# nv-tlabs/LION

Hardware: AMD Instinct MI355X
Metric: shapes/sec @1000-step DDIM, Bx2048pts (higher is better)
Workload: dtype f32 (operands of the 3x3x3 voxel convolutions and of the long 1x1 convolutions cut into fp16 hi/lo pairs on the 16-bi...

## Files before the change

include/lion_hip.h:

```cpp
#ifndef LION_HIP_H_
#define LION_HIP_H_

#include <stddef.h>
#include <stdint.h>

#ifdef __cplusplus
extern "C" {
#endif

typedef void *lionStream_t;

#define LION_OK 0
#define LION_EINVAL (-1)
#define LION_EUNSUPPORTED (-2)
#define LION_EWORKSPACE (-3)

int lion_abi_version(void);

size_t lion_avg_voxelize_workspace_bytes(int B, int C, int N, int r);
int lion_avg_voxelize_forward(const float *feat, const int32_t *coords, int B, int C, int N,
                              int r, float *out, int32_t *ind, int32_t *cnt, void *ws,
                              size_t ws_bytes, lionStream_t stream);

int lion_voxelize_points_forward(const float *feat, const float *coords, int B, int C, int N,
// ... 48 lines not shown
int lion_three_nn_interpolate_cat_forward(const float *points, const float *centers, const float *cfeat, const float *temb,
                                          int ld_t, const float *skip, int B, int C1, int C2, int C3, int N, int M,
                                          float *out, int32_t *idx, float *wgt, lionStream_t stream);
int lion_three_nn_interpolate_backward(const float *gy, const int32_t *idx, const float *wgt,
                                       int B, int C, int N, int M, float *gx,
                                       lionStream_t stream);

int lion_chamfer_forward(const float *xyz1, const float *xyz2, int B, int N, int M,
                         float *dist1, float *dist2, int32_t *idx1, int32_t *idx2,
                         lionStream_t stream);
int lion_chamfer_backward(const float *xyz1, const float *xyz2, const float *gdist1,
                          const float *gdist2, const int32_t *idx1, const int32_t *idx2, int B,
                          int N, int M, float *gxyz1, float *gxyz2, lionStream_t stream);
int lion_chamfer_loss_reduce(const float *dist1, const float *dist2, int B, int N, int M, float s1,
                             float s2, float *loss, lionStream_t stream);
int lion_chamfer_loss_backward(const float *xyz1, const float *xyz2, const int32_t *idx1,
                               const int32_t *idx2, const float *gloss, int B, int N, int M, float s1,
                               float s2, float *gxyz1, float *gxyz2, lionStream_t stream);

size_t lion_emd_workspace_bytes(int B, int N, int M);
int lion_emd_approxmatch(const float *xyz1, const float *xyz2, int B, int N, int M,
                         float *match, void *ws, size_t ws_bytes, lionStream_t stream);
int lion_emd_cost(const float *xyz1, const float *xyz2, int B, int N, int M, float *cost, void *ws,
                  size_t ws_bytes, lionStream_t stream);
int lion_emd_matchcost(const float *xyz1, const float *xyz2, const float *match, int B, int N,
                       int M, float *cost, void *ws, size_t ws_bytes, lionStream_t stream);
int lion_emd_matchcost_backward(const float *grad_cost, const float *xyz1, const float *xyz2,
                                const float *match, int B, int N, int M, float *grad1,
                                float *grad2, lionStream_t stream);
int lion_emd_loss_forward(const float *xyz1, const float *xyz2, int B, int N, int M, float *loss,
                          float *g1u, float *g2u, void *ws, size_t ws_bytes, lionStream_t stream);
int lion_emd_loss_backward(const float *gloss, const float *g1u, const float *g2u, int B, int N, int M,
                           float *gxyz1, float *gxyz2, lionStream_t stream);

int lion_ddim_update(const float *x, const float *eps, const float *z, size_t numel, float s,
                     float c, float sigma, float *out, lionStream_t stream);
int lion_ddpm_update(const float *x, const float *eps, const float *z, size_t numel,
                     int t_is_zero, float k_outer, float k_a, float k_b, float scale,
                     float temp, float *out, lionStream_t stream);
int lion_chain_begin_step(const float *table, int n_steps, int32_t *counter, float *t_out, int B, float *cur,
                          lionStream_t stream);
int lion_chain_update_noise(int mode, const float *x, const float *eps, size_t numel, const float *cur,
                            const uint32_t *seed , uint32_t stream_id, float *out,
                            float *z_out, lionStream_t stream);
int lion_chain_begin_step_temb(const float *table, int n_steps, int32_t *counter, float *t_out, int B, float *cur,
                               const float *temb_table, int temb_width, float *temb_out, lionStream_t stream);
int lion_chain_update_noise_cm(int mode, const float *x, const float *eps_cm, int B, int N, const float *cur,
                               const uint32_t *seed, uint32_t stream_id, float *out, float *z_out, lionStream_t stream);
int lion_dpmpp_update(const float *x, const float *eps, const float *hist, size_t numel, float a0, float a1, float a2,
                      float a3, float a4, float a5, float *out, float *hist_out, lionStream_t stream);
int lion_chain_update_multistep(const float *x, const float *eps, const float *hist, size_t numel, const float *cur,
                                float *out, float *hist_out, lionStream_t stream);
int lion_chain_update_multistep_cm(const float *x, const float *eps_cm, const float *hist, int B, int N, const float *cur,
                                   float *out, float *hist_out, lionStream_t stream);
int lion_sde_dpmpp_update(const float *x, const float *eps, const float *hist, const float *z_in, size_t numel, float a0,
                          float a1, float a2, float a3, float a4, float a5, float a6,
                          const uint32_t *seed , uint32_t step_word, uint32_t stream_id, float *out,
                          float *hist_out, float *z_out, lionStream_t stream);
int lion_chain_update_multistep_noise(const float *x, const float *eps, const float *hist, size_t numel, const float *cur,
                                      const float *table, const uint32_t *seed, uint32_t stream_id, float *out,
                                      float *hist_out, float *z_out, lionStream_t stream);
int lion_chain_update_multistep_noise_cm(const float *x, const float *eps_cm, const float *hist, int B, int N, const float *cur,
                                         const float *table, const uint32_t *seed, uint32_t stream_id, float *out,
                                         float *hist_out, float *z_out, lionStream_t stream);
int lion_ddim_encode_update(const float *base, const float *eps, size_t numel, float a0, float a1, float a2, float *out,
                            float *base_out, lionStream_t stream);
int lion_chain_update_encode(const float *base, const float *eps, size_t numel, const float *cur, float *out, float *base_out,
                             lionStream_t stream);
int lion_chain_update_encode_cm(const float *base, const float *eps_cm, int B, int N, const float *cur, float *out,
                                float *base_out, lionStream_t stream);
#define LION_DIFFUSE_STEP_WORD 0xFFFFFFFFu
int lion_chain_diffuse(const float *x0, const float *z_in, size_t numel, float m, float s,
                       const uint32_t *seed , uint32_t stream_id,
                       float *out, float *z_out, lionStream_t stream);
#define LION_START_STEP_WORD 0xFFFFFFFEu
int lion_philox_normal_keyed(const uint32_t *keys , int B, int n, uint32_t step_word, uint32_t stream_id,
                             float *out, lionStream_t stream);
int lion_chain_update_noise_keyed(int mode, const float *x, const float *eps, int B, int n, const float *cur,
                                  const uint32_t *keys, uint32_t stream_id, float *out, float *z_out, lionStream_t stream);
int lion_chain_update_noise_cm_keyed(int mode, const float *x, const float *eps_cm, int B, int N, const float *cur,
                                     const uint32_t *keys, uint32_t stream_id, float *out, float *z_out, lionStream_t stream);
int lion_chain_update_multistep_noise_keyed(const float *x, const float *eps, const float *hist, int B, int n, const float *cur,
                                            const float *table, const uint32_t *keys, uint32_t stream_id, float *out,
                                            float *hist_out, float *z_out, lionStream_t stream);
int lion_chain_update_multistep_noise_cm_keyed(const float *x, const float *eps_cm, const float *hist, int B, int N,
                                               const float *cur, const float *table, const uint32_t *keys, uint32_t stream_id,
                                               float *out, float *hist_out, float *z_out, lionStream_t stream);
int lion_chain_diffuse_keyed(const float *x0, int B, int n, float m, float s, const uint32_t *keys, uint32_t stream_id,
                             float *out, float *z_out, lionStream_t stream);
int lion_chain_update_noise_keyed_from(int mode, const float *x, const float *eps, int B, int n, const float *cur,
                                       const int32_t *first_row , const uint32_t *keys, uint32_t stream_id,
                                       float *out, float *z_out, lionStream_t stream);
int lion_chain_update_noise_cm_keyed_from(int mode, const float *x, const float *eps_cm, int B, int N, const float *cur,
                                          const int32_t *first_row, const uint32_t *keys, uint32_t stream_id, float *out,
                                          float *z_out, lionStream_t stream);
int lion_chain_diffuse_keyed_at(const float *x0, int B, int n, const float *ms , const uint32_t *keys,
                                uint32_t stream_id, float *out, float *z_out, lionStream_t stream);
int lion_chain_update_noise_keyed_known(int mode, const float *x, const float *eps, int B, int n, const float *cur,
                                        const int32_t *first_row , const uint32_t *keys,
                                        uint32_t stream_id, const float *known_x0, const uint8_t *keep ,
                                        const float *known_ms , uint32_t known_stream_id, float *out,
                                        float *z_out, lionStream_t stream);
int lion_chain_update_noise_cm_keyed_known(int mode, const float *x, const float *eps_cm, int B, int N, const float *cur,
                                           const int32_t *first_row, const uint32_t *keys, uint32_t stream_id,
                                           const float *known_x0, const uint8_t *keep, const float *known_ms,
                                           uint32_t known_stream_id, float *out, float *z_out, lionStream_t stream);
#define LION_VOXEL_STEP_WORD 0xFFFFFFFDu
#define LION_PERTURB_STEP_WORD 0xFFFFFFFCu
size_t lion_voxel_surface_workspace_bytes(int B, int N, int r, int K);
int lion_voxel_surface_points_keyed(const float *x, int B, int N, int r, const uint32_t *keys ,
                                    uint32_t stream_id, int K, float *out, int32_t *faces_out ,
                                    void *ws, size_t ws_bytes, lionStream_t stream);
int lion_perturb_points_keyed(int mode, const float *x, int B, int N, float p0, const uint32_t *keys, uint32_t stream_id,
                              float *out, lionStream_t stream);
int lion_voxel_occupancy(const float *x, int B, int N, int r, const float *frame_in ,
                         uint8_t *grid, float *frame_out , int32_t *clamped_out ,
                         lionStream_t stream);
int lion_voxel_surface_points_grid_keyed(const uint8_t *grid, const float *frame, int B, int r, const uint32_t *keys,
                                         uint32_t stream_id, int K, float *out, int32_t *faces_out ,
                                         lionStream_t stream);
int lion_voxel_iou(const uint8_t *a, const uint8_t *b, int B, int r, int32_t *counts ,
                   float *iou , lionStream_t stream);
int lion_latent_unpack(const float *x, int B, int N, int D, float *all, float *coords, float *rest, lionStream_t stream);
int lion_concat_broadcast(const float *a, const float *t, int B, int Ca, int Ct, int N, int ld_t, float *out,
                          lionStream_t stream);

size_t lion_conv3d_packed_floats(int Cout, int Cin);
int lion_conv3d_pack_weights(const float *w, int Cout, int Cin, float *wp, lionStream_t stream);
int lion_conv3d_k3_forward(const float *x, const float *wp, const float *bias, int B, int Cin,
                           int Cout, int r, float *y, lionStream_t stream);
size_t lion_conv3d_wgrad_workspace_floats(int B, int Cin, int Cout, int r);
int lion_conv3d_k3_wgrad(const float *x, const float *gy, int B, int Cin, int Cout, int r, float *gw, float *ws,
                         size_t ws_floats, lionStream_t stream);
int lion_conv3d_k3_wgrad_split(const float *x, const float *gy, int B, int Cin, int Cout, int r, float *gw, float *ws,
                               size_t ws_floats, lionStream_t stream);
size_t lion_conv3d_wgrad_sparse_workspace_floats(int B, int Cin, int Cout, int r);
int lion_conv3d_k3_wgrad_split_sparse(const float *x, const float *gy, const int32_t *cnt, int B, int Cin, int Cout, int r,
                                      float *gw, float *ws, size_t ws_floats, lionStream_t stream);

int lion_conv3d_stat_tiles(int r, int Cout, int B, int sparse);
int lion_conv3d_k3_fused_forward(const float *x, const float *wp, const float *bias, int B, int Cin,
                                 int Cout, int r, const float *pro_a, const float *pro_b, const float *pro_bias,
                                 const float *tconst, float *y, float *stats, int32_t *occ, lionStream_t stream);
size_t lion_conv3d_occupancy_ints(int r, int Cout, int B);
int lion_conv3d_const_response(const float *wsum, const float *bias2, const float *bias1, const float *pro_a,
                               const float *pro_b, int B, int Cin, int Cout, float *tconst, lionStream_t stream);
int lion_conv3d_tile_occupancy(const int32_t *cnt, int B, int r, int Cout, int32_t *occ_m1, int32_t *occ_m2,
                               lionStream_t stream);
int lion_conv3d_tile_occupancy_aware(const int32_t *cnt, int B, int r, int Cout, int32_t *occ_m1, int32_t *occ_m2,
                                     int consumer_aware, lionStream_t stream);
int lion_groupnorm_fold(const float *stats, int B, int C, int T, int G, int voxels, const float *gamma,
                        const float *beta, const float *fac, const float *gbias, int ld_fg, float eps,
                        float *A, float *Bs, float *chmean, lionStream_t stream);
size_t lion_conv3d_split_packed_halfs(int Cout, int Cin);
int lion_conv3d_split_pack_weights(const float *w, int Cout, int Cin, uint16_t *wp, lionStream_t stream);
int lion_conv3d_split_stat_tiles(int r, int Cout);
int lion_conv3d_k3_split_forward(const float *x, const uint16_t *wp, const float *bias, int B, int Cin, int Cout,
                                 int r, const float *pro_a, const float *pro_b, const float *pro_bias,
                                 const float *tconst, float *y, float *stats, int32_t *occ, lionStream_t stream);
int lion_conv3d_k3_half_forward(const float *x, const uint16_t *wp, const float *bias, int B, int Cin, int Cout,
                                int r, const float *pro_a, const float *pro_b, const float *pro_bias,
                                const float *tconst, float *y, float *stats, int32_t *occ, lionStream_t stream);
size_t lion_skinny_packed_floats(int Cout, int Cin);
int lion_skinny_pack_weights(const float *w, int Cout, int Cin, float *wp, lionStream_t stream);
int lion_skinny_splits(int Cin, int Cout);
int lion_skinny_gemm(const float *pin, int ks_in, const float *bias_in, int act_in, const float *addT,
                     const float *wp, int nb, int Cin, int Cout, float *pout, lionStream_t stream);
int lion_skinny_finish(const float *A, int ks_a, const float *bias_a, const float *Bp, int ks_b, const float *resid,
                       int nb, int C, int mode, float *y, lionStream_t stream);
int lion_skinny_gemm_se_finish(const float *pin, int ks_in, const float *bias_in, int act_in, const float *wp, int nb, int Cin,
                               int Cout, const float *A, int ks_a, const float *bias_a, const float *resid, float *y,
                               lionStream_t stream);
int lion_internal_skinny_gemm_plain(const float *pin, int ks_in, const float *bias_in, int act_in, const float *addT,
                                    const float *wp, int nb, int Cin, int Cout, float *pout, lionStream_t stream);
int lion_internal_skinny_gemm_se_finish_plain(const float *pin, int ks_in, const float *bias_in, int act_in, const float *wp,
                                              int nb, int Cin, int Cout, const float *A, int ks_a, const float *bias_a,
                                              const float *resid, float *y, lionStream_t stream);
int lion_to_channel_major(const float *a, int lda, int Ca, float *oa, const float *b, int ldb, int Cb, float *ob, int B,
                          lionStream_t stream);
int lion_from_channel_major(const float *x, int B, int C, float *y, lionStream_t stream);
int lion_groupnorm_fold_se(const float *stats, int B, int C, int T, int G, int voxels, const float *gamma,
                           const float *beta, const float *fac, const float *gbias, int ld_fg, float eps, const float *w1,
                           const float *w2, int H, float *A, float *Bs, lionStream_t stream);
int lion_internal_groupnorm_fold_se_plain(const float *stats, int B, int C, int T, int G, int voxels, const float *gamma,
                                          const float *beta, const float *fac, const float *gbias, int ld_fg, float eps,
                                          const float *w1, const float *w2, int H, float *A, float *Bs, lionStream_t stream);
int lion_se_gate(const float *chmean, const float *w1, const float *w2, int B, int C, int H, float *A,
                 float *Bs, lionStream_t stream);
int lion_trilinear_devoxelize_affine_forward(const float *coords, const float *feat, const float *scale,
                                             const float *shift, int B, int C, int N, int r, float *out,
                                             lionStream_t stream);
size_t lion_devoxelize_plan_bytes(int B, int N, int r);
int lion_trilinear_devoxelize_plan(const float *coords, int B, int N, int r, void *plan, size_t plan_bytes,
                                   lionStream_t stream);
int lion_trilinear_devoxelize_planned_forward(const void *plan, size_t plan_bytes, const float *coords, const float *feat,
                                              const float *scale, const float *shift, int B, int C, int N, int r,
                                              float *out, lionStream_t stream);

int lion_row_stats(const float *x, int rows, int L, float *stats, lionStream_t stream);
size_t lion_pwconv_packed_floats(int Cout, int Cin);
int lion_pwconv_pack_weights(const float *w, int Cout, int Cin, float *wp, lionStream_t stream);
int lion_pwconv_stat_tiles(int Cout, int Cin, int L);
int lion_pwconv_forward(const float *x, const float *wp, const float *bias, int B, int Cin, int Cout, int L,
                        const float *pro_a, const float *pro_b, float *y, float *stats, lionStream_t stream);
int lion_pwconv_forward_max(const float *x, const float *wp, const float *bias, int B, int Cin, int Cout, int L,
                            const float *pro_a, const float *pro_b, const float *out_a, const float *out_b,
                            float *stats, float *ymax, lionStream_t stream);
size_t lion_pwconv_split_packed_halfs(int Cout, int Cin);
int lion_pwconv_split_pack_weights(const float *w, int Cout, int Cin, uint16_t *wp, lionStream_t stream);
int lion_pwconv_split_pack_weights_t(const float *w, int Cout, int Cin, const uint16_t *wp, uint16_t *wpt, lionStream_t stream);
int lion_pwconv_split_stat_tiles(int Cout, int Cin, int L);
int lion_pwconv_split_forward(const float *x, const uint16_t *wp, const float *bias, int B, int Cin, int Cout, int L,
                              const float *pro_a, const float *pro_b, float *y, float *stats, lionStream_t stream);
int lion_pwconv_grouped_forward(const float *coords, const float *centers, const float *feat, const int32_t *idx,
                                const float *wp, const float *bias, int B, int C, int N, int M, int U, int Cout, float *y,
                                float *stats, lionStream_t stream);
int lion_pwconv_split_grouped_forward(const float *coords, const float *centers, const float *feat, const int32_t *idx,
                                      const uint16_t *wp, const float *bias, int B, int C, int N, int M, int U, int Cout,
                                      float *y, float *stats, lionStream_t stream);
int lion_internal_pwconv_walk(const float *x, const float *wp, const float *bias, int B, int Cin, int Cout, int L,
                              const float *pro_a, const float *pro_b, const float *out_a, const float *out_b,
                              const float *coords, const float *centers, const float *feat, const int32_t *idx, int N, int U,
                              float *y, float *stats, int max_wg, int lds_weights, lionStream_t stream);
int lion_internal_pwconv_small_plain(const float *x, const float *wp, const float *bias, int B, int Cin, int Cout, int L,
                                     const float *pro_a, const float *pro_b, const float *coords, const float *centers,
                                     const float *feat, const int32_t *idx, int N, int U, float *y, float *stats,
                                     lionStream_t stream);
int lion_linear_attention_core(const float *qkv, int B, int H, int D, int N, float *out, lionStream_t stream);
int lion_internal_linear_attention_path(int N, int aligned);
int lion_internal_linear_attention_core_plain(const float *qkv, int B, int H, int D, int N, float *out, lionStream_t stream);
int lion_linear_attention_core_backward(const float *qkv, const float *gout, int B, int H, int D, int N, float *gqkv,
                                        lionStream_t stream);
int lion_linear_forward(const float *x, const float *wp, const float *bias, int B, int K, int O, int act, float slope,
                        float *y, lionStream_t stream);
int lion_affine_swish(const float *x, const float *A, const float *Bs, int rows, int L, float *y,
                      lionStream_t stream);
int lion_affine_swish_max(const float *x, const float *A, const float *Bs, int rows, int M, int U,
                          float *y, lionStream_t stream);
int lion_timestep_embedding(const float *t, const float *row, float scale, int B, int half, int D, float *emb,
                            lionStream_t stream);
int lion_affine_swish_add(const float *x, const float *A, const float *Bs, const float *addend, int rows, int L, float *y,
                          lionStream_t stream);

size_t lion_scatter_csr_workspace_bytes(int B, int E, int bins);
int lion_scatter_csr(const float *gy, const int32_t *idx, const float *w, int B, int C, int S, int E, int bins, void *ws,
                     size_t ws_bytes, float *gx, lionStream_t stream);

size_t lion_pwconv_wgrad_workspace_bytes(int B, int Cin, int Cout, int L);
int lion_pwconv_wgrad(const float *x, const float *gy, int B, int Cin, int Cout, int L, void *ws, size_t ws_bytes,
                      float *gw, float *gb, lionStream_t stream);

int lion_gn_train_fold(const float *stats, const float *gw, const float *gb, const float *fac, int fac_stride,
                       const float *bias, int bias_stride, int B, int C, int G, int L, float eps, float *A, float *Bs,
                       float *mean, float *rstd, lionStream_t stream);
int lion_row_stats64(const float *x, int rows, int L, double *stats, lionStream_t stream);
int lion_gn_train_fold64(const double *stats, const float *gw, const float *gb, const float *fac, int fac_stride,
                         const float *bias, int bias_stride, int B, int C, int G, int L, float eps, float *A,
                         float *Bs, float *mean, float *rstd, lionStream_t stream);
int lion_gn_train_bwd_fold(const float *S, const float *mean, const float *rstd, const float *gw, const float *gb,
                           const float *fac, int fac_stride, int B, int C, int G, int L, float *Q, float *R, float *dfac,
                           float *dbias, int d_stride, float *pw, const float *A, const double *xstats, const float *gate,
                           const float *qse, float *Aout, lionStream_t stream);
int lion_gn_train_param_grads(const float *pw, int B, int C, float *dgw, float *dgb, float *dxs, lionStream_t stream);
int lion_se_gate_fwd(const float *stats, const float *w1, const float *w2, int B, int C, int Cr, int L, float *mean, float *h,
                     float *g, float *zero, lionStream_t stream);
int lion_se_gate_bwd(const float *S, const float *g, const float *h, const float *mean, const float *w1, const float *w2, int B,
                     int C, int Cr, int L, float *dpre2, float *dpre1, float *Q, float *dw1, float *dw2, lionStream_t stream);
int lion_rows_dot2(const float *g, const float *v, const float *ws, int B, int C, int N, float *S, lionStream_t stream);
int lion_trilinear_devoxelize_backward_affine(const float *gy, const int32_t *inds, const float *wgts, const float *x,
                                              const float *Ap, const float *Q, const float *R, int B, int C, int N, int r3,
                                              float *dx, lionStream_t stream);
int lion_gn_se_gate_fwd(const double *xstats, const float *A, const float *Bs, const float *w1, const float *w2, int B, int C, int Cr,
                        int L, float *mean, float *h, float *g, float *A2, float *B2, lionStream_t stream);
int lion_gn_se_gate_bwd(const float *S, const double *xstats, const float *A, const float *Bs, const float *g, const float *h,
                        const float *mean, const float *w1, const float *w2, int B, int C, int Cr, int L, float *Sp, float *dpre2,
                        float *dpre1, float *Qse, float *dw1, float *dw2, lionStream_t stream);
int lion_affine_act(const float *x, const float *A, const float *Bs, int rows, int L, int act, float *y,
                    lionStream_t stream);
int lion_affine_act_bwd_stats(const float *x, const float *gy, const float *A, const float *Bs, int rows, int L, int act,
                              float *S, lionStream_t stream);
int lion_affine_act_bwd_apply(const float *x, const float *gy, const float *A, const float *Bs, const float *Q,
                              const float *R, int rows, int L, int act, float *dx, lionStream_t stream);
int lion_affine_act_dropout(const float *x, const float *A, const float *Bs, int rows, int L, int act, const uint64_t *seed,
                            float keep, float *y, lionStream_t stream);
int lion_affine_act_dropout_bwd_stats(const float *x, const float *gy, const float *A, const float *Bs, int rows, int L, int act,
                                      const uint64_t *seed, float keep, float *S, lionStream_t stream);
int lion_affine_act_dropout_bwd_apply(const float *x, const float *gy, const float *A, const float *Bs, const float *Q,
                                      const float *R, int rows, int L, int act, const uint64_t *seed, float keep, float *dx,
                                      lionStream_t stream);
int lion_affine_act_max(const float *x, const float *A, const float *Bs, int rows, int M, int U, int act, float *y,
                        lionStream_t stream);
int lion_affine_act_max_bwd_stats(const float *x, const float *gy, const float *A, const float *Bs, int rows, int M, int U,
                                  int act, float *S, lionStream_t stream);
int lion_affine_act_max_bwd_apply(const float *x, const float *gy, const float *A, const float *Bs, const float *Q,
                                  const float *R, int rows, int M, int U, int act, float *dx, lionStream_t stream);

int lion_adam_chunk(void);
int lion_adam_row(void);
int lion_adam_step(const uint64_t *table, const int32_t *numel, const int32_t *blockmap, int blocks, int tensors, const float *lr,
                   float beta1, float beta2, float eps, float weight_decay, float ema_decay, lionStream_t stream);

int lion_grad_sqnorm_partials(const uint64_t *table, const int32_t *numel, const int32_t *blockmap, int blocks, float *partials,
                              lionStream_t stream);
int lion_grad_clip_coef(const float *partials, int n, float max_norm, float *out2, lionStream_t stream);
int lion_adam_step_scaled(const uint64_t *table, const int32_t *numel, const int32_t *blockmap, int blocks, int tensors,
                          const float *lr, float beta1, float beta2, float eps, float weight_decay, float ema_decay,
                          const float *grad_scale, lionStream_t stream);

#define LION_ODE_RUNNING 0
#define LION_ODE_FINISHED 1
#define LION_ODE_TOO_SMALL_STEP (-1)
typedef struct lion_ode_ctrl {
  double t, h_abs, t_bound, direction, rtol, atol;
  double h, t_new, err_norm, h0, d1, sign;
  int32_t stage, cur, status, step_rejected;
  int32_t yslot, fslot, nfe, n_accepted;
  int32_t n_rejected, accepted, pad0, pad1;
} lion_ode_ctrl;
size_t lion_ode_partials_bytes(size_t n);
int lion_ode_stage(double *Y, const double *K, size_t n, lion_ode_ctrl *ctrl, float *x32, float *t_model, int B,
                   lionStream_t stream);
int lion_ode_drift(const float *eps, int cm_points, const float *x32, size_t n, const float *t_model, float beta_start,
                   float beta_delta, float neg_beta_start, float half_beta_delta, float one_minus_sigma2_0,
                   const float *mix_a, const float *mix_b, int mix_len, double *K, lion_ode_ctrl *ctrl,
                   lionStream_t stream);
int lion_ode_error_partials(const double *Y, const double *K, size_t n, const lion_ode_ctrl *ctrl, double *partials,
                            lionStream_t stream);
int lion_ode_control(const double *partials, size_t n, lion_ode_ctrl *ctrl, lionStream_t stream);

#ifdef __cplusplus
}
#endif
#endif
```

lion_amd/_lib.py:

```python
from __future__ import annotations

import ctypes as C
import os

_HERE = os.path.dirname(os.path.abspath(__file__))
SO_PATH = os.environ.get("LION_HIP_SO") or os.path.join(_HERE, "csrc", "liblion_hip.so")

_vp, _i, _f, _sz = C.c_void_p, C.c_int, C.c_float, C.c_size_t

SIGNATURES = {
    "lion_abi_version": (_i, []),
    "lion_avg_voxelize_workspace_bytes": (_sz, [_i, _i, _i, _i]),
    "lion_avg_voxelize_forward": (_i, [_vp, _vp, _i, _i, _i, _i, _vp, _vp, _vp, _vp, _sz, _vp]),
    "lion_voxelize_points_forward": (_i, [_vp, _vp, _i, _i, _i, _i, _i, _f, _vp, _vp, _vp, _vp,
                                          _vp, _sz, _vp]),
    "lion_voxel_plan_bytes": (_sz, [_i, _i, _i]),
    "lion_voxel_index": (_i, [_vp, _i, _i, _i, _i, _f, _vp, _vp, _vp, _vp, _sz, _vp]),
    "lion_voxel_scatter": (_i, [_vp, _vp, _sz, _i, _i, _i, _i, _vp, _vp]),
    "lion_voxel_scatter_read": (_i, [_vp, _vp, _sz, _i, _i, _i, _i, _vp, _vp, _vp]),
    "lion_internal_voxelize_plan": (_i, [_i, _i, _i, _i, _i, _vp, _vp]),
    "lion_internal_devoxelize_path": (_i, [_i, _i, _i, _i, _i, _vp, _vp]),
    "lion_avg_voxelize_backward": (_i, [_vp, _vp, _vp, _i, _i, _i, _i, _vp, _vp]),
    "lion_trilinear_devoxelize_forward": (_i, [_vp, _vp, _i, _i, _i, _i, _i, _vp, _vp, _vp, _vp]),
    "lion_trilinear_devoxelize_backward": (_i, [_vp, _vp, _vp, _i, _i, _i, _i, _vp, _vp]),
    "lion_ball_query": (_i, [_vp, _vp, _i, _i, _i, _f, _i, _vp, _vp]),
    "lion_grouping_forward": (_i, [_vp, _vp, _i, _i, _i, _i, _i, _vp, _vp]),
    "lion_group_points_forward": (_i, [_vp, _vp, _vp, _vp, _i, _i, _i, _i, _i, _vp, _vp]),
    "lion_grouping_backward": (_i, [_vp, _vp, _i, _i, _i, _i, _i, _vp, _vp]),
    "lion_furthest_point_sampling": (_i, [_vp, _i, _i, _i, _vp, _vp]),
    "lion_gather_features_forward": (_i, [_vp, _vp, _i, _i, _i, _i, _vp, _vp]),
    "lion_gather_features_backward": (_i, [_vp, _vp, _i, _i, _i, _i, _vp, _vp]),
    "lion_three_nn_interpolate_forward": (_i, [_vp, _vp, _vp, _i, _i, _i, _i, _vp, _vp, _vp, _vp]),
    "lion_three_nn_interpolate_backward": (_i, [_vp, _vp, _vp, _i, _i, _i, _i, _vp, _vp]),
    "lion_chamfer_forward": (_i, [_vp, _vp, _i, _i, _i, _vp, _vp, _vp, _vp, _vp]),
    "lion_chamfer_backward": (_i, [_vp, _vp, _vp, _vp, _vp, _vp, _i, _i, _i, _vp, _vp, _vp]),
    "lion_chamfer_loss_reduce": (_i, [_vp, _vp, _i, _i, _i, _f, _f, _vp, _vp]),
    "lion_chamfer_loss_backward": (_i, [_vp, _vp, _vp, _vp, _vp, _i, _i, _i, _f, _f, _vp, _vp, _vp]),
    "lion_emd_workspace_bytes": (_sz, [_i, _i, _i]),
    "lion_emd_approxmatch": (_i, [_vp, _vp, _i, _i, _i, _vp, _vp, _sz, _vp]),
    "lion_emd_cost": (_i, [_vp, _vp, _i, _i, _i, _vp, _vp, _sz, _vp]),
    "lion_emd_matchcost": (_i, [_vp, _vp, _vp, _i, _i, _i, _vp, _vp, _sz, _vp]),
    "lion_emd_matchcost_backward": (_i, [_vp, _vp, _vp, _vp, _i, _i, _i, _vp, _vp, _vp]),
    "lion_emd_loss_forward": (_i, [_vp, _vp, _i, _i, _i, _vp, _vp, _vp, _vp, _sz, _vp]),
    "lion_emd_loss_backward": (_i, [_vp, _vp, _vp, _i, _i, _i, _vp, _vp, _vp]),
    "lion_conv3d_packed_floats": (_sz, [_i, _i]),
    "lion_conv3d_pack_weights": (_i, [_vp, _i, _i, _vp, _vp]),
    "lion_conv3d_k3_forward": (_i, [_vp, _vp, _vp, _i, _i, _i, _i, _vp, _vp]),
    "lion_conv3d_wgrad_workspace_floats": (_sz, [_i, _i, _i, _i]),
    "lion_conv3d_k3_wgrad": (_i, [_vp, _vp, _i, _i, _i, _i, _vp, _vp, _sz, _vp]),
    "lion_conv3d_k3_wgrad_split": (_i, [_vp, _vp, _i, _i, _i, _i, _vp, _vp, _sz, _vp]),
    "lion_conv3d_wgrad_sparse_workspace_floats": (_sz, [_i, _i, _i, _i]),
    "lion_conv3d_k3_wgrad_split_sparse": (_i, [_vp, _vp, _vp, _i, _i, _i, _i, _vp, _vp, _sz, _vp]),
    "lion_conv3d_stat_tiles": (_i, [_i, _i, _i, _i]),
    "lion_conv3d_k3_fused_forward": (_i, [_vp, _vp, _vp, _i, _i, _i, _i, _vp, _vp, _vp, _vp, _vp, _vp, _vp, _vp]),
    "lion_conv3d_const_response": (_i, [_vp, _vp, _vp, _vp, _vp, _i, _i, _i, _vp, _vp]),
    "lion_conv3d_occupancy_ints": (_sz, [_i, _i, _i]),
    "lion_conv3d_tile_occupancy": (_i, [_vp, _i, _i, _i, _vp, _vp, _vp]),
    "lion_conv3d_tile_occupancy_aware": (_i, [_vp, _i, _i, _i, _vp, _vp, _i, _vp]),
    "lion_conv3d_split_packed_halfs": (_sz, [_i, _i]),
    "lion_conv3d_split_pack_weights": (_i, [_vp, _i, _i, _vp, _vp]),
    "lion_conv3d_split_stat_tiles": (_i, [_i, _i]),
    "lion_conv3d_k3_split_forward": (_i, [_vp, _vp, _vp, _i, _i, _i, _i, _vp, _vp, _vp, _vp, _vp, _vp, _vp, _vp]),
    "lion_conv3d_k3_half_forward": (_i, [_vp, _vp, _vp, _i, _i, _i, _i, _vp, _vp, _vp, _vp, _vp, _vp, _vp, _vp]),
    "lion_groupnorm_fold": (_i, [_vp, _i, _i, _i, _i, _i, _vp, _vp, _vp, _vp, _i, _f, _vp, _vp, _vp, _vp]),
    "lion_groupnorm_fold_se": (_i, [_vp, _i, _i, _i, _i, _i, _vp, _vp, _vp, _vp, _i, _f, _vp, _vp, _i, _vp, _vp, _vp]),
    "lion_internal_groupnorm_fold_se_plain": (_i, [_vp, _i, _i, _i, _i, _i, _vp, _vp, _vp, _vp, _i, _f, _vp, _vp, _i, _vp, _vp, _vp]),
    "lion_skinny_packed_floats": (_sz, [_i, _i]),
    "lion_skinny_pack_weights": (_i, [_vp, _i, _i, _vp, _vp]),
    "lion_skinny_splits": (_i, [_i, _i]),
    "lion_skinny_gemm": (_i, [_vp, _i, _vp, _i, _vp, _vp, _i, _i, _i, _vp, _vp]),
    "lion_skinny_gemm_se_finish": (_i, [_vp, _i, _vp, _i, _vp, _i, _i, _i, _vp, _i, _vp, _vp, _vp, _vp]),
    "lion_internal_skinny_gemm_plain": (_i, [_vp, _i, _vp, _i, _vp, _vp, _i, _i, _i, _vp, _vp]),
    "lion_internal_skinny_gemm_se_finish_plain": (_i, [_vp, _i, _vp, _i, _vp, _i, _i, _i, _vp, _i, _vp, _vp, _vp, _vp]),
    "lion_skinny_finish": (_i, [_vp, _i, _vp, _vp, _i, _vp, _i, _i, _i, _vp, _vp]),
    "lion_to_channel_major": (_i, [_vp, _i, _i, _vp, _vp, _i, _i, _vp, _i, _vp]),
    "lion_from_channel_major": (_i, [_vp, _i, _i, _vp, _vp]),
    "lion_se_gate": (_i, [_vp, _vp, _vp, _i, _i, _i, _vp, _vp, _vp]),
    "lion_trilinear_devoxelize_affine_forward": (_i, [_vp, _vp, _vp, _vp, _i, _i, _i, _i, _vp, _vp]),
    "lion_devoxelize_plan_bytes": (_sz, [_i, _i, _i]),
    "lion_trilinear_devoxelize_plan": (_i, [_vp, _i, _i, _i, _vp, _sz, _vp]),
    "lion_trilinear_devoxelize_planned_forward": (_i, [_vp, _sz, _vp, _vp, _vp, _vp, _i, _i, _i, _i, _vp, _vp]),
    "lion_row_stats": (_i, [_vp, _i, _i, _vp, _vp]),
    "lion_pwconv_packed_floats": (_sz, [_i, _i]),
    "lion_pwconv_pack_weights": (_i, [_vp, _i, _i, _vp, _vp]),
    "lion_pwconv_stat_tiles": (_i, [_i, _i, _i]),
    "lion_pwconv_forward": (_i, [_vp, _vp, _vp, _i, _i, _i, _i, _vp, _vp, _vp, _vp, _vp]),
    "lion_pwconv_forward_max": (_i, [_vp, _vp, _vp, _i, _i, _i, _i, _vp, _vp, _vp, _vp, _vp, _vp, _vp]),
    "lion_pwconv_split_packed_halfs": (_sz, [_i, _i]),
    "lion_pwconv_split_pack_weights": (_i, [_vp, _i, _i, _vp, _vp]),
    "lion_pwconv_split_pack_weights_t": (_i, [_vp, _i, _i, _vp, _vp, _vp]),
    "lion_pwconv_split_stat_tiles": (_i, [_i, _i, _i]),
    "lion_pwconv_split_forward": (_i, [_vp, _vp, _vp, _i, _i, _i, _i, _vp, _vp, _vp, _vp, _vp]),
    "lion_pwconv_grouped_forward": (_i, [_vp, _vp, _vp, _vp, _vp, _vp, _i, _i, _i, _i, _i, _i, _vp, _vp, _vp]),
    "lion_pwconv_split_grouped_forward": (_i, [_vp, _vp, _vp, _vp, _vp, _vp, _i, _i, _i, _i, _i, _i, _vp, _vp, _vp]),
    "lion_internal_pwconv_walk": (_i, [_vp, _vp, _vp, _i, _i, _i, _i, _vp, _vp, _vp, _vp, _vp, _vp, _vp, _vp, _i, _i, _vp, _vp, _i, _i, _vp]),
    "lion_internal_pwconv_small_plain": (_i, [_vp, _vp, _vp, _i, _i, _i, _i, _vp, _vp, _vp, _vp, _vp, _vp, _i, _i, _vp, _vp, _vp]),
    "lion_linear_attention_core": (_i, [_vp, _i, _i, _i, _i, _vp, _vp]),
    "lion_internal_linear_attention_path": (_i, [_i, _i]),
    "lion_internal_linear_attention_core_plain": (_i, [_vp, _i, _i, _i, _i, _vp, _vp]),
    "lion_linear_attention_core_backward": (_i, [_vp, _vp, _i, _i, _i, _i, _vp, _vp]),
    "lion_linear_forward": (_i, [_vp, _vp, _vp, _i, _i, _i, _i, _f, _vp, _vp]),
    "lion_affine_swish": (_i, [_vp, _vp, _vp, _i, _i, _vp, _vp]),
    "lion_affine_swish_max": (_i, [_vp, _vp, _vp, _i, _i, _i, _vp, _vp]),
    "lion_timestep_embedding": (_i, [_vp, _vp, _f, _i, _i, _i, _vp, _vp]),
    "lion_affine_swish_add": (_i, [_vp, _vp, _vp, _vp, _i, _i, _vp, _vp]),
    "lion_scatter_csr_workspace_bytes": (_sz, [_i, _i, _i]),
    "lion_scatter_csr": (_i, [_vp, _vp, _vp, _i, _i, _i, _i, _i, _vp, _sz, _vp, _vp]),
    "lion_pwconv_wgrad_workspace_bytes": (_sz, [_i, _i, _i, _i]),
    "lion_pwconv_wgrad": (_i, [_vp, _vp, _i, _i, _i, _i, _vp, _sz, _vp, _vp, _vp]),
    "lion_gn_train_fold": (_i, [_vp, _vp, _vp, _vp, _i, _vp, _i, _i, _i, _i, _i, _f, _vp, _vp, _vp, _vp, _vp]),
    "lion_row_stats64": (_i, [_vp, _i, _i, _vp, _vp]),
    "lion_gn_train_fold64": (_i, [_vp, _vp, _vp, _vp, _i, _vp, _i, _i, _i, _i, _i, _f, _vp, _vp, _vp, _vp, _vp]),
    "lion_gn_train_bwd_fold": (_i, [_vp, _vp, _vp, _vp, _vp, _vp, _i, _i, _i, _i, _i, _vp, _vp, _vp, _vp, _i, _vp, _vp, _vp, _vp, _vp,
                                    _vp, _vp]),
    "lion_gn_train_param_grads": (_i, [_vp, _i, _i, _vp, _vp, _vp, _vp]),
    "lion_adam_chunk": (_i, []),
    "lion_adam_row": (_i, []),
    "lion_adam_step": (_i, [_vp, _vp, _vp, _i, _i, _vp, _f, _f, _f, _f, _f, _vp]),
    "lion_grad_sqnorm_partials": (_i, [_vp, _vp, _vp, _i, _vp, _vp]),
    "lion_grad_clip_coef": (_i, [_vp, _i, _f, _vp, _vp]),
    "lion_adam_step_scaled": (_i, [_vp, _vp, _vp, _i, _i, _vp, _f, _f, _f, _f, _f, _vp, _vp]),
    "lion_se_gate_fwd": (_i, [_vp, _vp, _vp, _i, _i, _i, _i, _vp, _vp, _vp, _vp, _vp]),
    "lion_se_gate_bwd": (_i, [_vp, _vp, _vp, _vp, _vp, _vp, _i, _i, _i, _i, _vp, _vp, _vp, _vp, _vp, _vp]),
    "lion_rows_dot2": (_i, [_vp, _vp, _vp, _i, _i, _i, _vp, _vp]),
    "lion_trilinear_devoxelize_backward_affine": (_i, [_vp, _vp, _vp, _vp, _vp, _vp, _vp, _i, _i, _i, _i, _vp, _vp]),
    "lion_gn_se_gate_fwd": (_i, [_vp, _vp, _vp, _vp, _vp, _i, _i, _i, _i, _vp, _vp, _vp, _vp, _vp, _vp]),
    "lion_gn_se_gate_bwd": (_i, [_vp, _vp, _vp, _vp, _vp, _vp, _vp, _vp, _vp, _i, _i, _i, _i, _vp, _vp, _vp, _vp, _vp, _vp, _vp]),
    "lion_affine_act": (_i, [_vp, _vp, _vp, _i, _i, _i, _vp, _vp]),
    "lion_affine_act_bwd_stats": (_i, [_vp, _vp, _vp, _vp, _i, _i, _i, _vp, _vp]),
    "lion_affine_act_bwd_apply": (_i, [_vp, _vp, _vp, _vp, _vp, _vp, _i, _i, _i, _vp, _vp]),
    "lion_affine_act_dropout": (_i, [_vp, _vp, _vp, _i, _i, _i, _vp, _f, _vp, _vp]),
    "lion_affine_act_dropout_bwd_stats": (_i, [_vp, _vp, _vp, _vp, _i, _i, _i, _vp, _f, _vp, _vp]),
    "lion_affine_act_dropout_bwd_apply": (_i, [_vp, _vp, _vp, _vp, _vp, _vp, _i, _i, _i, _vp, _f, _vp, _vp]),
    "lion_affine_act_max": (_i, [_vp, _vp, _vp, _i, _i, _i, _i, _vp, _vp]),
    "lion_affine_act_max_bwd_stats": (_i, [_vp, _vp, _vp, _vp, _i, _i, _i, _i, _vp, _vp]),
    "lion_affine_act_max_bwd_apply": (_i, [_vp, _vp, _vp, _vp, _vp, _vp, _i, _i, _i, _i, _vp, _vp]),
    "lion_ddim_update": (_i, [_vp, _vp, _vp, _sz, _f, _f, _f, _vp, _vp]),
    "lion_ddpm_update": (_i, [_vp, _vp, _vp, _sz, _i, _f, _f, _f, _f, _f, _vp, _vp]),
    "lion_chain_begin_step": (_i, [_vp, _i, _vp, _vp, _i, _vp, _vp]),
    "lion_chain_update_noise": (_i, [_i, _vp, _vp, _sz, _vp, _vp, C.c_uint32, _vp, _vp, _vp]),
    "lion_chain_begin_step_temb": (_i, [_vp, _i, _vp, _vp, _i, _vp, _vp, _i, _vp, _vp]),
    "lion_chain_update_noise_cm": (_i, [_i, _vp, _vp, _i, _i, _vp, _vp, C.c_uint32, _vp, _vp, _vp]),
    "lion_chain_diffuse": (_i, [_vp, _vp, _sz, _f, _f, _vp, C.c_uint32, _vp, _vp, _vp]),
    "lion_dpmpp_update": (_i, [_vp, _vp, _vp, _sz, _f, _f, _f, _f, _f, _f, _vp, _vp, _vp]),
    "lion_chain_update_multistep": (_i, [_vp, _vp, _vp, _sz, _vp, _vp, _vp, _vp]),
    "lion_chain_update_multistep_cm": (_i, [_vp, _vp, _vp, _i, _i, _vp, _vp, _vp, _vp]),
    "lion_sde_dpmpp_update": (_i, [_vp, _vp, _vp, _vp, _sz, _f, _f, _f, _f, _f, _f, _f, _vp, C.c_uint32, C.c_uint32, _vp, _vp,
                                   _vp, _vp]),
    "lion_chain_update_multistep_noise": (_i, [_vp, _vp, _vp, _sz, _vp, _vp, _vp, C.c_uint32, _vp, _vp, _vp, _vp]),
    "lion_chain_update_multistep_noise_cm": (_i, [_vp, _vp, _vp, _i, _i, _vp, _vp, _vp, C.c_uint32, _vp, _vp, _vp, _vp]),
    "lion_ddim_encode_update": (_i, [_vp, _vp, _sz, _f, _f, _f, _vp, _vp, _vp]),
    "lion_chain_update_encode": (_i, [_vp, _vp, _sz, _vp, _vp, _vp, _vp]),
    "lion_chain_update_encode_cm": (_i, [_vp, _vp, _i, _i, _vp, _vp, _vp, _vp]),
    "lion_philox_normal_keyed": (_i, [_vp, _i, _i, C.c_uint32, C.c_uint32, _vp, _vp]),
    "lion_chain_update_noise_keyed": (_i, [_i, _vp, _vp, _i, _i, _vp, _vp, C.c_uint32, _vp, _vp, _vp]),
    "lion_chain_update_noise_cm_keyed": (_i, [_i, _vp, _vp, _i, _i, _vp, _vp, C.c_uint32, _vp, _vp, _vp]),
    "lion_chain_update_multistep_noise_keyed": (_i, [_vp, _vp, _vp, _i, _i, _vp, _vp, _vp, C.c_uint32, _vp, _vp, _vp, _vp]),
    "lion_chain_update_multistep_noise_cm_keyed": (_i, [_vp, _vp, _vp, _i, _i, _vp, _vp, _vp, C.c_uint32, _vp, _vp, _vp, _vp]),
    "lion_chain_diffuse_keyed": (_i, [_vp, _i, _i, _f, _f, _vp, C.c_uint32, _vp, _vp, _vp]),
    "lion_chain_update_noise_keyed_from": (_i, [_i, _vp, _vp, _i, _i, _vp, _vp, _vp, C.c_uint32, _vp, _vp, _vp]),
    "lion_chain_update_noise_cm_keyed_from": (_i, [_i, _vp, _vp, _i, _i, _vp, _vp, _vp, C.c_uint32, _vp, _vp, _vp]),
    "lion_chain_update_noise_keyed_known": (_i, [_i, _vp, _vp, _i, _i, _vp, _vp, _vp, C.c_uint32, _vp, _vp, _vp, C.c_uint32, _vp,
                                                 _vp, _vp]),
    "lion_chain_update_noise_cm_keyed_known": (_i, [_i, _vp, _vp, _i, _i, _vp, _vp, _vp, C.c_uint32, _vp, _vp, _vp, C.c_uint32,
                                                    _vp, _vp, _vp]),
    "lion_chain_diffuse_keyed_at": (_i, [_vp, _i, _i, _vp, _vp, C.c_uint32, _vp, _vp, _vp]),
    "lion_voxel_surface_workspace_bytes": (_sz, [_i, _i, _i, _i]),
    "lion_voxel_surface_points_keyed": (_i, [_vp, _i, _i, _i, _vp, C.c_uint32, _i, _vp, _vp, _vp, _sz, _vp]),
    "lion_perturb_points_keyed": (_i, [_i, _vp, _i, _i, _f, _vp, C.c_uint32, _vp, _vp]),
    "lion_voxel_occupancy": (_i, [_vp, _i, _i, _i, _vp, _vp, _vp, _vp, _vp]),
    "lion_voxel_surface_points_grid_keyed": (_i, [_vp, _vp, _i, _i, _vp, C.c_uint32, _i, _vp, _vp, _vp]),
    "lion_voxel_iou": (_i, [_vp, _vp, _i, _i, _vp, _vp, _vp]),
    "lion_latent_unpack": (_i, [_vp, _i, _i, _i, _vp, _vp, _vp, _vp]),
    "lion_concat_broadcast": (_i, [_vp, _vp, _i, _i, _i, _i, _i, _vp, _vp]),
    "lion_three_nn_interpolate_cat_forward": (_i, [_vp, _vp, _vp, _vp, _i, _vp, _i, _i, _i, _i, _i, _i, _vp, _vp, _vp, _vp]),
    "lion_ode_partials_bytes": (_sz, [_sz]),
    "lion_ode_stage": (_i, [_vp, _vp, _sz, _vp, _vp, _vp, _i, _vp]),
    "lion_ode_drift": (_i, [_vp, _i, _vp, _sz, _vp, _f, _f, _f, _f, _f, _vp, _vp, _i, _vp, _vp, _vp]),
    "lion_ode_error_partials": (_i, [_vp, _vp, _sz, _vp, _vp, _vp]),
    "lion_ode_control": (_i, [_vp, _sz, _vp, _vp]),
}



_ERR = {-1: "LION_EINVAL (bad shape / null pointer)",
        -2: "LION_EUNSUPPORTED (shape outside what the kernels implement)",
        -3: "LION_EWORKSPACE (workspace too small)"}

_lib = None


def load() -> C.CDLL:
    global _lib
    if _lib is not None:
        return _lib
    if not os.path.exists(SO_PATH):
        raise RuntimeError(
            f"lion_amd: HIP extension not built: {SO_PATH} is missing. Run "
            f"`python -c 'import __graft_entry__ as g; g.build()'` or lion_amd/csrc/build.sh. "
            f"There is no CPU fallback.")
    lib = C.CDLL(SO_PATH)
    for name, (res, args) in SIGNATURES.items():
        try:
            fn = getattr(lib, name)
        except AttributeError as e:
            raise RuntimeError(f"lion_amd: {SO_PATH} does not export {name}") from e
        fn.restype = res
        fn.argtypes = args
    _lib = lib
    return lib


def check(code: int, what: str) -> None:
    if code != 0:
        msg = _ERR.get(code, f"hipError {code}" if code > 0 else f"error {code}")
        raise RuntimeError(f"lion_amd: {what} failed: {msg}")


def call(name: str, *args, unsupported_ok: bool = False) -> bool:
    import torch
    if len(args) + 1 != len(SIGNATURES[name][1]):
        raise TypeError(f"lion_amd: {name} takes {len(SIGNATURES[name][1]) - 1} arguments before the stream, got {len(args)}")
    dev, argv = None, list(args)
    for i, a in enumerate(args):
        if isinstance(a, torch.Tensor):
            d = a.get_device()
            if d != dev:
                if d < 0:
                    raise RuntimeError("lion_amd: expected a CUDA(HIP) tensor; there is no CPU path")
                if dev is not None:
                    raise RuntimeError(f"lion_amd: {name}: operands on different devices (cuda:{dev} and cuda:{d})")
# ... 27 lines not shown
```

lion_amd/chain.py:

```python
from __future__ import annotations

from collections import OrderedDict

import numpy as np
import torch

from . import _lib, _wcache

DDIM, DDPM, DPMPP, SDE_DPMPP, ENCODE = range(5)
UPDATE = {
    DDIM: ("lion_chain_update_noise", (DDIM, "x", "eps", "size", "cur", "seed", 0, "x", "z")),
    DDPM: ("lion_chain_update_noise", (DDPM, "x", "eps", "size", "cur", "seed", 0, "x", "z")),
    DPMPP: ("lion_chain_update_multistep", ("x", "eps", "hist", "size", "cur", "x", "hist")),
    SDE_DPMPP: ("lion_chain_update_multistep_noise", ("x", "eps", "hist", "size", "cur", "table", "seed", 0, "x", "hist", "z")),
    ENCODE: ("lion_chain_update_encode", ("base", "eps", "size", "cur", "x", "base")),
}
KEYED_MODES = (DDIM, DDPM, SDE_DPMPP)
FROM_ROWS_MODES = (DDPM,)
KNOWN_STREAM = 2
START_STEP_WORD, DIFFUSE_STEP_WORD = 0xFFFFFFFE, 0xFFFFFFFF
_MASK64 = 0xFFFFFFFFFFFFFFFF


def split_seed(seed: int, n: int):
    out, state = [], seed & _MASK64
    for _ in range(n):
        state = (state + 0x9E3779B97F4A7C15) & _MASK64
        z = state
        z = ((z ^ (z >> 30)) * 0xBF58476D1CE4E5B9) & _MASK64
        z = ((z ^ (z >> 27)) * 0x94D049BB133111EB) & _MASK64
        out.append(z ^ (z >> 31))
    return out


def sample_keys(seeds, num_samples, who="seeds") -> list:
    if isinstance(seeds, torch.Tensor):
        seeds = seeds.detach().cpu().reshape(-1).tolist()
    elif isinstance(seeds, np.ndarray):
        seeds = seeds.reshape(-1).tolist()
    try:
        keys = [int(s) & _MASK64 for s in seeds]
    except TypeError as e:
        raise ValueError(f"{who}: a sequence or tensor of {num_samples} ints, got {seeds!r}") from e
    if len(keys) != int(num_samples):
        raise ValueError(f"{who}: {len(keys)} seeds for {num_samples} samples")
    return keys


def first_rows(first_row, num_samples) -> list:
    rows = [int(r) for r in first_row]
    if len(rows) != int(num_samples) or any(not 0 <= r < 2 ** 31 for r in rows):
        raise ValueError(f"GraphedChain: first_row = {rows!r}: {num_samples} ints in [0, 2^31)")
    return rows


def key_words(keys, device=None):
    k = np.array([[s & 0xFFFFFFFF, (s >> 32) & 0xFFFFFFFF] for s in keys], dtype=np.uint32).view(np.int32)
    t = torch.from_numpy(k)
    return t if device is None else t.to(device)


RECORD = None
TEMB_TABLE = __import__("os").environ.get("LION_TEMB_TABLE", "1") != "0"
CHANNEL_MAJOR_EPS = __import__("os").environ.get("LION_CHAIN_CM_EPS", "1") != "0"

def policy_key() -> tuple:
    from . import conv_ops, fused_ops, geometry
    from .models import pvcnn2_ada
    return (pvcnn2_ada.SPARSE_CONV1, pvcnn2_ada.FUSE_INFERENCE, pvcnn2_ada.OVERLAP_POINT_BRANCH, geometry.ENABLED,
            geometry.SPLIT_GRAPH, conv_ops.SPLIT, fused_ops.PW_SPLIT, pvcnn2_ada.VOX_PLAN, TEMB_TABLE, fused_ops.MAX_RECOMPUTE,
            pvcnn2_ada.SKIP_UNREAD, pvcnn2_ada.SKIP_UNREAD_LEVEL2, CHANNEL_MAJOR_EPS, pvcnn2_ada.SA_GATHER, conv_ops.PRECISION)


def channel_major(model, shape) -> bool:
    n_pts, n_cls = getattr(model, "num_points", 0), getattr(model, "num_classes", 0)
    return CHANNEL_MAJOR_EPS and hasattr(model, "geometry_source") and n_cls == 4 and int(np.prod(shape)) == n_pts * n_cls


def same_conditioning(owner, condition_input, clip_feat) -> bool:
    same = lambda buf, new: (buf is None) == (new is None) and (buf is None or buf.shape == new.shape)
    return same(owner.cond, condition_input) and same(owner.clip, clip_feat)


class LRU:

    def __init__(self, capacity=4):
        self._entries, self._capacity = OrderedDict(), capacity

    def lookup(self, key, usable, build):
        hit = self._entries.get(key)
        if hit is not None and usable(hit):
            self._entries.move_to_end(key)
            return hit
        self._entries.pop(key, None)
        hit = self._entries[key] = build()
        while len(self._entries) > self._capacity:
            self._entries.popitem(last=False)
        return hit

    def clear(self):
        self._entries.clear()


class CapturedStep:

    def __init__(self, model, step, x, *, warmup=2, split=None):
        self.model, self.x = model, x
        self.fingerprint, self.policy = _wcache.fingerprint(model), policy_key()
        self.pinned = []
        dev = x.device
        from . import geometry
        src = getattr(model, "geometry_source", None)
        self.geo_graphs = self.graph_b = self.graphs = self.waits = self.geo_plan = None
        if split is None:
            split = geometry.SPLIT_GRAPH and src is not None and not geometry.ENABLED
        main = torch.cuda.current_stream(dev)
        side = torch.cuda.Stream(device=dev)
        side.wait_stream(main)
        with _wcache.pinning(self.pinned):
            with torch.no_grad(), torch.cuda.stream(side):
                for _ in range(warmup):
                    step()
            main.wait_stream(side)
            if split:
                self.geo_stream = torch.cuda.Stream(device=dev)
                self.ev_step = torch.cuda.Event()

                def geo(boundary=None):
                    mods, coords = src(x)
                    return geometry.compute_chain(mods, coords, boundary=boundary)
                self.geo_stream.wait_stream(main)
                with torch.no_grad(), torch.cuda.stream(self.geo_stream):
                    geo()
                main.wait_stream(self.geo_stream)
                torch.cuda.synchronize(dev)
                self.geo_graphs = [torch.cuda.CUDAGraph()]
                gs = torch.cuda.Stream(device=dev)
                gs.wait_stream(main)

                def geo_cut(i):
                    if i == 1:
                        self.geo_graphs[-1].capture_end()
                        self.geo_graphs.append(torch.cuda.CUDAGraph())
                        self.geo_graphs[-1].capture_begin(pool=self.geo_graphs[0].pool())
                with torch.no_grad(), torch.cuda.stream(gs):
                    self.geo_graphs[0].capture_begin()
                    try:
                        self.geo_plan = geo(geo_cut)
                    finally:
                        self.geo_graphs[-1].capture_end()
                main.wait_stream(gs)
                torch.cuda.synchronize(dev)
                self.geo_stage_of_graph = [0, self.geo_plan["stages"] - 1][:len(self.geo_graphs)]
                self.ev_geo = [torch.cuda.Event() for _ in self.geo_graphs]
                graphs, waits = [torch.cuda.CUDAGraph()], []

                def on_use(first, last):
                    need = [g for g, st_ in enumerate(self.geo_stage_of_graph)
                            if st_ >= first and (g == 0 or self.geo_stage_of_graph[g - 1] < last)]
                    need = [g for g in need if not any(g in w for w in waits)]
                    if not need:
                        return
                    graphs[-1].capture_end()
                    waits.append(need)
                    graphs.append(torch.cuda.CUDAGraph())
                    graphs[-1].capture_begin(pool=graphs[0].pool())
                cap = torch.cuda.Stream(device=dev)
                cap.wait_stream(main)
                with torch.no_grad(), torch.cuda.stream(cap), geometry.external(self.geo_plan, on_use):
                    graphs[0].capture_begin()
                    try:
                        step()
                    finally:
                        graphs[-1].capture_end()
                main.wait_stream(cap)
                self.graph = graphs[0]
                if waits:
                    self.graphs, self.waits = graphs, waits
                    self.graph_b = graphs[1]
                else:
                    self.geo_graphs = self.geo_plan = None
            else:
                self.graph = torch.cuda.CUDAGraph()
                with torch.no_grad(), torch.cuda.graph(self.graph):
                    step()
        self.pinned = list({id(v): v for v in self.pinned}.values())

    def replay(self):
        if self.graph_b is None:
            self.graph.replay()
            return
        main = torch.cuda.current_stream(self.x.device)
        self.ev_step.record(main)
        self.geo_stream.wait_event(self.ev_step)
        with torch.cuda.stream(self.geo_stream):
            for g, ev in zip(self.geo_graphs, self.ev_geo):
                g.replay()
                ev.record(self.geo_stream)
        self.graphs[0].replay()
        for k, need in enumerate(self.waits):
            for g in need:
                main.wait_event(self.ev_geo[g])
            self.graphs[k + 1].replay()

    def valid(self):
        return self.fingerprint == _wcache.fingerprint(self.model) and self.policy == policy_key()


class GraphedChain:
    def __init__(self, model, num_samples, shape, condition_input, clip_feat, device, mode, capacity, warmup=2,
                 record_noise=False, keyed=False, from_rows=False, known=False):
        self.model, self.mode, self.capacity, self.keyed = model, mode, int(capacity), bool(keyed)
        self.from_rows, self.known = bool(from_rows), bool(known)
        dev = torch.device(device)
        size = [num_samples] + list(shape)
        per_sample = int(np.prod(shape))
        if self.from_rows and not (keyed and mode in FROM_ROWS_MODES):
            raise ValueError(f"GraphedChain: from_rows needs a keyed DDPM chain, got mode {mode}, keyed={bool(keyed)}")
        if self.known and not (keyed and self.from_rows):
            raise ValueError(f"GraphedChain: known needs keyed=True and from_rows=True, got keyed={bool(keyed)}, "
                             f"from_rows={self.from_rows}")
        if keyed and mode not in KEYED_MODES:
            raise ValueError(f"GraphedChain: mode {mode} draws nothing and has no keyed form")
        if keyed and per_sample % 4 != 0:
# ... 153 lines not shown
```

lion_amd/csrc/common.h:

```cpp
#pragma once
#include <hip/hip_runtime.h>
#include <stdint.h>
#include <stddef.h>
#include <type_traits>

#include "lion_hip.h"

#define LION_WAVE 64

#define LION_LAUNCH_CHECK()                         \
  do {                                              \
    hipError_t e__ = hipGetLastError();             \
    if (e__ != hipSuccess) return (int)e__;         \
  } while (0)

static inline int lion_cdiv(int a, int b) { return (a + b - 1) / b; }

#define LION_MAX_DEVICES 32
struct LionLdsLimit {
  size_t bytes[LION_MAX_DEVICES];
};
static inline int lion_current_device(int *dev) {
  if (hipGetDevice(dev) != hipSuccess || *dev < 0 || *dev >= LION_MAX_DEVICES) return LION_EINVAL;
  return 0;
}
static inline int lion_cu_count(int *n) {
  static int cu_count[LION_MAX_DEVICES] = {0};
  int dev = 0;
  if (int e = lion_current_device(&dev)) return e;
  if (!cu_count[dev]) {
    hipDeviceProp_t prop;
    if (hipGetDeviceProperties(&prop, dev) != hipSuccess) return LION_EINVAL;
    cu_count[dev] = prop.multiProcessorCount;
  }
  *n = cu_count[dev];
  return 0;
}
template <typename K>
static inline int lion_dynamic_lds(K kernel, size_t bytes, LionLdsLimit &limit) {
  int dev = 0;
  if (int e = lion_current_device(&dev)) return e;
  if (bytes > limit.bytes[dev]) {
    hipError_t e = hipFuncSetAttribute(reinterpret_cast<const void *>(kernel),
                                       hipFuncAttributeMaxDynamicSharedMemorySize, (int)bytes);
    if (e != hipSuccess) return (int)e;
    limit.bytes[dev] = bytes;
  }
  return 0;
}

template <auto Kernel> struct LionLaunch;
template <typename... P, void (*Kernel)(P...)> struct LionLaunch<Kernel> {
  int operator()(dim3 grid, dim3 block, size_t lds, hipStream_t st, P... args) const {
    if (lds > 0) {
      static LionLdsLimit limit = {};
      if (int e = lion_dynamic_lds(Kernel, lds, limit)) return e;
    }
    Kernel<<<grid, block, lds, st>>>(args...);
    return (int)hipGetLastError();
  }
};
template <auto Kernel> static constexpr LionLaunch<Kernel> lion_launch{};

template <bool V> using BoolC = std::bool_constant<V>;
template <int V> using IntC = std::integral_constant<int, V>;
template <typename F> static inline int lion_with_flags(bool a, F f) { return a ? f(BoolC<true>{}) : f(BoolC<false>{}); }
template <typename F> static inline int lion_with_flags(bool a, bool b, F f) {
  return lion_with_flags(a, [&](auto A) { return lion_with_flags(b, [&](auto B) { return f(A, B); }); });
}

struct PwGather {
  const float *coords, *centers, *feat;
  const int32_t *idx;
  int C, N, U;
};

__device__ __forceinline__ float mul_rn(float a, float b) { return __fmul_rn(a, b); }
__device__ __forceinline__ float add_rn(float a, float b) { return __fadd_rn(a, b); }
__device__ __forceinline__ float sub_rn(float a, float b) { return __fsub_rn(a, b); }
__device__ __forceinline__ float div_rn(float a, float b) { return __fdiv_rn(a, b); }
__device__ __forceinline__ float sqrt_rn(float a) { return sqrtf(a); }
__device__ __forceinline__ void philox4x32_10(uint32_t c0, uint32_t c1, uint32_t c2, uint32_t c3, uint32_t k0,
                                              uint32_t k1, uint32_t out[4]) {
#pragma unroll
  for (int r = 0; r < 10; ++r) {
    const uint64_t p0 = (uint64_t)0xD2511F53u * c0, p1 = (uint64_t)0xCD9E8D57u * c2;
    const uint32_t n0 = (uint32_t)(p1 >> 32) ^ c1 ^ k0, n2 = (uint32_t)(p0 >> 32) ^ c3 ^ k1;
    c1 = (uint32_t)p1; c3 = (uint32_t)p0; c0 = n0; c2 = n2;
    k0 += 0x9E3779B9u; k1 += 0xBB67AE85u;
  }
  out[0] = c0; out[1] = c1; out[2] = c2; out[3] = c3;
}

__device__ __forceinline__ float swish_fast(float t) { return t * __builtin_amdgcn_rcpf(1.0f + __expf(-t)); }

__device__ __forceinline__ float sqdist3(float ax, float ay, float az, float bx, float by,
                                         float bz) {
  const float dx = sub_rn(ax, bx), dy = sub_rn(ay, by), dz = sub_rn(az, bz);
  return add_rn(add_rn(mul_rn(dx, dx), mul_rn(dy, dy)), mul_rn(dz, dz));
}

#define LION_DPP_F32(v, ctrl) __builtin_bit_cast(float, __builtin_amdgcn_update_dpp(0, __builtin_bit_cast(int, (v)), (ctrl), 0xf, 0xf, true))
__device__ __forceinline__ float row16_sum_rn(float v) {
  v = __fadd_rn(v, LION_DPP_F32(v, 0xB1));
  v = __fadd_rn(v, LION_DPP_F32(v, 0x4E));
  v = __fadd_rn(v, LION_DPP_F32(v, 0x141));
  v = __fadd_rn(v, LION_DPP_F32(v, 0x140));
  return v;
}
__device__ __forceinline__ unsigned wave_max_u32_lane63(unsigned v) {
#define LION_DPP_U32(x, ctrl, rmask) ((unsigned)__builtin_amdgcn_update_dpp(0, (int)(x), (ctrl), (rmask), 0xf, true))
  unsigned o;
  o = LION_DPP_U32(v, 0xB1, 0xf); v = o > v ? o : v;
  o = LION_DPP_U32(v, 0x4E, 0xf); v = o > v ? o : v;
  o = LION_DPP_U32(v, 0x141, 0xf); v = o > v ? o : v;
  o = LION_DPP_U32(v, 0x140, 0xf); v = o > v ? o : v;
  o = LION_DPP_U32(v, 0x142, 0xa); v = o > v ? o : v;
  o = LION_DPP_U32(v, 0x143, 0xc); v = o > v ? o : v;
#undef LION_DPP_U32
  return v;
}
__device__ __forceinline__ float row_pair_sum_odd_rows(float v) {
  return __fadd_rn(v, __builtin_bit_cast(float, __builtin_amdgcn_update_dpp(0, __builtin_bit_cast(int, v), 0x142, 0xa, 0xf, true)));
}
#define LION_DPP_F32_ROWS(x, ctrl, rmask) \
  __builtin_bit_cast(float, __builtin_amdgcn_update_dpp(0, __builtin_bit_cast(int, (x)), (ctrl), (rmask), 0xf, true))
__device__ __forceinline__ float row16_max(float v) {
  float o;
  o = LION_DPP_F32(v, 0xB1); v = o > v ? o : v;
  o = LION_DPP_F32(v, 0x4E); v = o > v ? o : v;
  o = LION_DPP_F32(v, 0x141); v = o > v ? o : v;
  o = LION_DPP_F32(v, 0x140); v = o > v ? o : v;
  return v;
}

__device__ __forceinline__ int wave_incl_scan(int v, int lane) {
#pragma unroll
  for (int d = 1; d < LION_WAVE; d <<= 1) {
    const int t = __shfl_up(v, d, LION_WAVE);
    if (lane >= d) v += t;
  }
  return v;
}
```

lion_amd/csrc/conv3d.hip:

```cpp
#include "conv3d_tiles.h"

namespace {

typedef float f32x16 __attribute__((ext_vector_type(16)));
#ifndef LION_CONV_KC
#define LION_CONV_KC 4
#endif
#ifndef LION_CONV_WAVES
#define LION_CONV_WAVES 2
#endif
constexpr int KC = LION_CONV_KC;

__device__ __forceinline__ float pro_act(float v, float pa, float pb) {
  const float t = v * pa + pb;
  return swish_fast(t);
}

template <int TD, int TH, int TW, int COT, int VB, bool PRO, bool STATS>
__global__ __launch_bounds__(256, LION_CONV_WAVES) void conv3d_k3_kernel(const float *__restrict__ x,
                                                                const float *__restrict__ wp,
                                                                const float *__restrict__ bias,
                                                                float *__restrict__ y, int Cin,
                                                                int Cout, int r,
                                                                const float *__restrict__ pro_a,
// ... 341 lines not shown
    const int4 v = c4[i];
    if (v.x | v.y | v.z | v.w) {
      const unsigned m4 = (v.x ? 1u : 0u) | (v.y ? 2u : 0u) | (v.z ? 4u : 0u) | (v.w ? 8u : 0u);
      atomicOr(&col[(i << 2) / r], m4 << ((i << 2) % r));
    }
  }
  __syncthreads();
  const int RW = 64 / r;
  for (int e = tid; e < 2 * ntiles; e += 1024) {
    const int t = e % ntiles, margin = 1 + e / ntiles;
    const int dt = (t / nth) * TD, ht = (t % nth) * TH;
    int mask = 0;
    for (int w = 0; w < 4; ++w) {
      const int dl = dt + (w * RW) / TH, hl = ht + (w * RW) % TH;
      unsigned any = 0u;
      for (int d = max(dl - margin, 0); d <= min(dl + margin, r - 1); ++d)
        for (int h = max(hl - margin, 0); h <= min(hl + RW - 1 + margin, r - 1); ++h) any |= col[d * r + h];
      mask |= (any ? 1 : 0) << w;
    }
    flag[margin - 1][t] = mask;
  }
  __syncthreads();
  __shared__ unsigned long long bal[2][4];
  const int m = tid >> 8, t = tid & 255, lane = tid & 63, w = (tid >> 6) & 3;
  const bool live = tid < 512 && t < ntiles;
  const int f = live ? flag[m][t] : 0;
  const unsigned long long bl = __ballot(f != 0);
  if (tid < 512 && lane == 0) bal[m][w] = bl;
  __syncthreads();
  if (live) {
    int32_t *occ = m == 0 ? occ1 : occ2;
    if (occ) {
      int before = __popcll(bal[m][w] & ((1ull << lane) - 1ull)), occupied = 0;
      for (int ww = 0; ww < 4; ++ww) {
        const int c = __popcll(bal[m][ww]);
        if (ww < w) before += c;
        occupied += c;
      }
      int32_t *fl = occ + (size_t)b * ntiles, *list = occ + total + (size_t)b * ntiles;
      int need = flag[1][t] != 0;
      if (m == 0) {
        if (aware == 2) {
          need = 0;
        } else {
          const int td = t / nth, th = t % nth;
          for (int dd = max(td - 1, 0); dd <= min(td + 1, r / TD - 1); ++dd)
            for (int hh = max(th - 1, 0); hh <= min(th + 1, nth - 1); ++hh) need |= flag[1][dd * nth + hh] != 0;
        }
      }
      fl[t] = f | (need << 8) | ((m == 1 && flag[0][t] != 0) ? (1 << 9) : 0);
      list[f ? before : occupied + (t - before)] = t;
      if (b == 0 && t == 0) { occ[2 * total] = 0; occ[2 * total + 1] = 0; occ[2 * total + 2] = aware; }
    }
  }
}

__global__ __launch_bounds__(256) void conv_tconst_kernel(const float *__restrict__ wsum, const float *__restrict__ bias2,
                                                          const float *__restrict__ bias1, const float *__restrict__ pro_a,
                                                          const float *__restrict__ pro_b, int Cin, int Cout,
                                                          float *__restrict__ tconst) {
  __shared__ float sc[256];
  const int cfg = blockIdx.x, b = blockIdx.y, tid = threadIdx.x;
  for (int c = tid; c < Cin; c += 256)
    sc[c] = pro_act(bias1 ? bias1[c] : 0.f, pro_a[(size_t)b * Cin + c], pro_b[(size_t)b * Cin + c]);
  __syncthreads();
  for (int co = tid; co < Cout; co += 256) {
    double acc = bias2 ? (double)bias2[co] : 0.0;
    const float *w = wsum + (size_t)cfg * Cin * Cout + co;
    for (int c = 0; c < Cin; ++c) acc += (double)w[(size_t)c * Cout] * (double)sc[c];
    tconst[((size_t)b * 27 + cfg) * Cout + co] = (float)acc;
  }
}

template <int HV, int CC>
__global__ __launch_bounds__(256) void gn_fold_se_ahead_kernel(const float *__restrict__ stats, int C, int T, int G, float count,
                                                               const float *__restrict__ gamma, const float *__restrict__ beta,
                                                               const float *__restrict__ fac, const float *__restrict__ gbias,
                                                               int ld_fg, float eps, const float *__restrict__ w1,
                                                               const float *__restrict__ w2, float *__restrict__ A,
                                                               float *__restrict__ Bs) {
  constexpr int H = 4 * HV;
  __shared__ double cs[256][2];
  __shared__ float sA[256], sB[256], sm[256], sh[128];
  const int b = blockIdx.x, tid = threadIdx.x, lane = tid & 63, wave = tid >> 6, cpg = C / G;
  const int tc = min(tid, C - 1);
  const float p_f = fac[(size_t)b * ld_fg + tc], p_gb = gbias[(size_t)b * ld_fg + tc], p_gam = gamma[tc], p_bet = beta[tc];
  float w1r[HV][CC];
  float4 w2r[HV];
#pragma unroll
  for (int jj = 0; jj < HV; ++jj)
#pragma unroll
    for (int q = 0; q < CC; ++q) w1r[jj][q] = w1[(size_t)(wave + 4 * jj) * C + min(lane + 64 * q, C - 1)];
#pragma unroll
  for (int j = 0; j < HV; ++j) w2r[j] = reinterpret_cast<const float4 *>(w2 + (size_t)tc * H)[j];
  int cp2 = 1;
  while (cp2 < C) cp2 <<= 1;
  const int LPC = 256 / cp2, ch = tid / LPC, sub = tid % LPC;
  double s1 = 0.0, s2 = 0.0;
  if (ch < C) {
    const float2 *p = reinterpret_cast<const float2 *>(stats + (((size_t)b * C + ch) * T) * 2);
    for (int t0 = sub; t0 < T; t0 += 8 * LPC) {
      float2 v[8];
#pragma unroll
      for (int u = 0; u < 8; ++u) v[u] = p[min(t0 + u * LPC, T - 1)];
#pragma unroll
      for (int u = 0; u < 8; ++u)
        if (t0 + u * LPC < T) { s1 += (double)v[u].x; s2 += (double)v[u].y; }
    }
  }
  for (int m = 1; m < LPC; m <<= 1) { s1 += __shfl_xor(s1, m, 64); s2 += __shfl_xor(s2, m, 64); }
  if (ch < C && sub == 0) { cs[ch][0] = s1; cs[ch][1] = s2; }
  __syncthreads();
  if (tid < C) {
    const int g0 = (tid / cpg) * cpg;
    double g1 = 0.0, g2 = 0.0;
    for (int k = 0; k < cpg; ++k) { g1 += cs[g0 + k][0]; g2 += cs[g0 + k][1]; }
    const double n = (double)count * cpg, mean = g1 / n;
    double var = g2 / n - mean * mean;
    var = var > 0.0 ? var : 0.0;
    const float rstd = (float)(1.0 / sqrt(var + (double)eps));
    const float a0 = rstd * p_gam;
    const float a = a0 * p_f, bb = (p_bet - (float)mean * a0) * p_f + p_gb;
    sA[tid] = a;
    sB[tid] = bb;
    sm[tid] = a * (float)(cs[tid][0] / count) + bb;
  }
  __syncthreads();
#pragma unroll
  for (int jj = 0; jj < HV; ++jj) {
    float acc = 0.f;
#pragma unroll
    for (int q = 0; q < CC; ++q)
      if (lane + 64 * q < C) acc += w1r[jj][q] * sm[lane + 64 * q];
#pragma unroll
    for (int m = 32; m >= 1; m >>= 1) acc += __shfl_xor(acc, m, 64);
    if (lane == 0) sh[wave + 4 * jj] = acc > 0.f ? acc : 0.f;
  }
  __syncthreads();
  if (tid < C) {
    float acc = 0.f;
#pragma unroll
    for (int j = 0; j < HV; ++j) {
      acc += w2r[j].x * sh[4 * j];
      acc += w2r[j].y * sh[4 * j + 1];
      acc += w2r[j].z * sh[4 * j + 2];
      acc += w2r[j].w * sh[4 * j + 3];
    }
    const float g = 1.0f / (1.0f + expf(-acc));
    A[(size_t)b * C + tid] = sA[tid] * g;
    Bs[(size_t)b * C + tid] = sB[tid] * g;
  }
}

__global__ void conv3d_pack_kernel(const float *__restrict__ w, int Cout, int Cin, int Cin_pad,
                                   float *__restrict__ wp) {
  const int i = blockIdx.x * blockDim.x + threadIdx.x;
  const int total = Cin_pad * 27 * Cout;
  if (i >= total) return;
  const int co = i % Cout, t = (i / Cout) % 27, ci = i / (Cout * 27);
  wp[i] = ci < Cin ? w[((size_t)co * Cin + ci) * 27 + t] : 0.f;
}

template <int COT, int TD, int TH, int TW>
static int launch_conv(IntC<TD>, IntC<TH>, IntC<TW>, const float *x, const float *wp, const float *bias, float *y, int B,
                       int Cin, int Cout, int r, const float *pa, const float *pb, const float *pbias, const float *tconst,
                       float *stats, int32_t *occ, hipStream_t st) {
  constexpr int VB = TD * TH * TW / 128;
  const int tiles = conv_tile_count(r, VB);
  dim3 grid;
  if (int e = conv_grid(occ != nullptr, B, tiles, Cout / COT, 2, &grid)) return e;
  constexpr int NT = 256, HALO = (TD + 2) * (TH + 2) * (TW + 2);
  constexpr int SWS = ((KC * 27 * COT + 255) / 256) * 256 + 256;
  static_assert(KC * HALO >= 27 * COT, "the response table must fit the input tile buffer");
  const size_t LDS = (size_t)(((KC * HALO + 3) & ~3) + 2 * SWS + COT + (pa ? 3 * ((Cin + 63) & ~63) : 0) +
                              (NT / 64) * COT * 2) * 4;
  return lion_with_flags(pa != nullptr, stats != nullptr, [&](auto PRO, auto ST) {
    return lion_launch<conv3d_k3_kernel<TD, TH, TW, COT, VB, decltype(PRO)::value, decltype(ST)::value>>(
        grid, NT, LDS, st, x, wp, bias, y, Cin, Cout, r, pa, pb, pbias, tconst, stats, occ, B, tiles);
  });
}

struct ConvPlan { int vb, cot, tiles; };
constexpr ConvPlan conv_plan(int r, int Cout, int B, bool sparse) {
  const int t4 = conv_tile_count(r, 4), t2 = conv_tile_count(r, 2);
  if (!sparse && Cout % 64 == 0 && r >= 16 && (long)t4 * (Cout / 64) * B >= 512) return {4, 64, t4};
  if (Cout % 64 == 0 && (long)t2 * (Cout / 64) * B >= 512) return {2, 64, t2};
  if (Cout % 32 == 0 && r >= 16) return sparse ? ConvPlan{2, 32, t2} : ConvPlan{4, 32, t4};
  if (Cout % 32 == 0) return {1, 32, conv_tile_count(r, 1)};
  return {0, 0, 0};
}
constexpr bool sparse256(int r, int B) { return conv_plan(r, 32, B, true).vb == 2 && conv_plan(r, 64, B, true).vb == 2; }
static_assert(sparse256(16, 1) && sparse256(16, 32) && sparse256(32, 1) && sparse256(32, 32), "a sparse plan left conv_tile256");

}

extern "C" {

size_t lion_conv3d_packed_floats(int Cout, int Cin) {
  return (size_t)((Cin + KC - 1) / KC * KC) * 27 * Cout;
}

int lion_conv3d_pack_weights(const float *w, int Cout, int Cin, float *wp, lionStream_t stream) {
  if (!w || !wp || Cout <= 0 || Cin <= 0) return LION_EINVAL;
  const int Cin_pad = (Cin + KC - 1) / KC * KC;
  const int total = Cin_pad * 27 * Cout;
  return lion_launch<conv3d_pack_kernel>(lion_cdiv(total, 256), 256, 0, static_cast<hipStream_t>(stream), w, Cout, Cin,
                                         Cin_pad, wp);
}

int lion_conv3d_k3_fused_forward(const float *x, const float *wp, const float *bias, int B, int Cin,
                                 int Cout, int r, const float *pro_a, const float *pro_b, const float *pro_bias,
                                 const float *tconst, float *y, float *stats, int32_t *occ, lionStream_t stream) {
  if (int e = conv_forward_args(x, wp, y, B, Cin, Cout, pro_a, pro_b, tconst, occ)) return e;
  if (Cin % KC != 0 || (pro_a && Cin > 256) || (r != 8 && r != 16 && r != 32)) return LION_EUNSUPPORTED;
  hipStream_t st = static_cast<hipStream_t>(stream);
  const ConvPlan p = conv_plan(r, Cout, B, occ != nullptr);
  return conv_tile_dispatch(r, p.vb, [&](auto TD, auto TH, auto TW) {
    auto go = [&](auto COT) {
      return launch_conv<decltype(COT)::value>(TD, TH, TW, x, wp, bias, y, B, Cin, Cout, r, pro_a, pro_b, pro_bias, tconst,
                                               stats, occ, st);
    };
    constexpr int vb = decltype(TD)::value * decltype(TH)::value * decltype(TW)::value / 128;
    if constexpr (decltype(TW)::value == 8) return p.cot == 32 * vb ? go(IntC<32 * vb>{}) : (int)LION_EUNSUPPORTED;
    else return p.cot == 64 ? go(IntC<64>{}) : go(IntC<32>{});
  });
}

int lion_conv3d_k3_forward(const float *x, const float *wp, const float *bias, int B, int Cin,
                           int Cout, int r, float *y, lionStream_t stream) {
  return lion_conv3d_k3_fused_forward(x, wp, bias, B, Cin, Cout, r, nullptr, nullptr, nullptr, nullptr, y, nullptr,
                                      nullptr, stream);
}

int lion_conv3d_const_response(const float *wsum, const float *bias2, const float *bias1, const float *pro_a,
                               const float *pro_b, int B, int Cin, int Cout, float *tconst, lionStream_t stream) {
  if (!wsum || !pro_a || !pro_b || !tconst || B <= 0 || Cin <= 0 || Cout <= 0) return LION_EINVAL;
  if (Cin > 256) return LION_EUNSUPPORTED;
  return lion_launch<conv_tconst_kernel>(dim3(27, B), 256, 0, static_cast<hipStream_t>(stream), wsum, bias2, bias1,
                                         pro_a, pro_b, Cin, Cout, tconst);
}

size_t lion_conv3d_occupancy_ints(int r, int Cout, int B) {
  if (r != 16 && r != 32) return 0;
  return (size_t)2 * B * conv_plan(r, Cout, B, true).tiles + 4;
}

int lion_conv3d_tile_occupancy(const int32_t *cnt, int B, int r, int Cout, int32_t *occ_m1, int32_t *occ_m2,
                               lionStream_t stream) {
  return lion_conv3d_tile_occupancy_aware(cnt, B, r, Cout, occ_m1, occ_m2, 0, stream);
}

int lion_conv3d_tile_occupancy_aware(const int32_t *cnt, int B, int r, int Cout, int32_t *occ_m1, int32_t *occ_m2,
                                     int consumer_aware, lionStream_t stream) {
  if (!cnt || (!occ_m1 && !occ_m2) || B <= 0 || Cout <= 0) return LION_EINVAL;
  if (r != 16 && r != 32) return LION_EUNSUPPORTED;
  const ConvPlan p = conv_plan(r, Cout, B, true);
  if (!p.vb || p.tiles > 256 || (((uintptr_t)cnt) & 15) != 0) return LION_EUNSUPPORTED;
  const ConvTileDims t = conv_tile_dims(r, p.vb);
  return lion_launch<conv_tile_occ_kernel>(B, 1024, 0, static_cast<hipStream_t>(stream), cnt, r, t.td, t.th, occ_m1, occ_m2,
                                           consumer_aware == 2 ? 2 : consumer_aware ? 1 : 0);
}

int lion_conv3d_stat_tiles(int r, int Cout, int B, int sparse) {
  if (r != 8 && r != 16 && r != 32) return 0;
  return conv_plan(r, Cout, B, sparse != 0).tiles;
}

static int gn_fold_se_args(const float *stats, int B, int C, int T, int G, const float *gamma, const float *beta,
                           const float *fac, const float *gbias, int ld_fg, const float *w1, const float *w2, int H,
                           float *A, float *Bs) {
  if (!stats || !gamma || !beta || !fac || !gbias || !w1 || !w2 || !A || !Bs) return LION_EINVAL;
  if (B <= 0 || C <= 0 || T <= 0 || G <= 0 || C % G != 0 || ld_fg < C || H <= 0) return LION_EINVAL;
  if (C > 256 || C < 4 || H > 128) return LION_EUNSUPPORTED;
  return 0;
}

int lion_groupnorm_fold_se(const float *stats, int B, int C, int T, int G, int voxels, const float *gamma,
                           const float *beta, const float *fac, const float *gbias, int ld_fg, float eps, const float *w1,
                           const float *w2, int H, float *A, float *Bs, lionStream_t stream) {
  if (int e = gn_fold_se_args(stats, B, C, T, G, gamma, beta, fac, gbias, ld_fg, w1, w2, H, A, Bs)) return e;
  hipStream_t st = static_cast<hipStream_t>(stream);
  if (H % 4 != 0 || H > 32 || (H & (H - 1)) != 0 || (((uintptr_t)w2) & 15) != 0)
    return lion_launch<gn_fold_se_kernel>(B, 256, 0, st, stats, C, T, G, (float)voxels, gamma, beta, fac, gbias, ld_fg, eps, w1, w2,
                                          H, A, Bs);
  auto go = [&](auto HV, auto CC) {
    return lion_launch<gn_fold_se_ahead_kernel<decltype(HV)::value, decltype(CC)::value>>(
        B, 256, 0, st, stats, C, T, G, (float)voxels, gamma, beta, fac, gbias, ld_fg, eps, w1, w2, A, Bs);
  };
  auto rows = [&](auto CC) {
    return H == 4 ? go(IntC<1>{}, CC) : H == 8 ? go(IntC<2>{}, CC) : H == 16 ? go(IntC<4>{}, CC) : go(IntC<8>{}, CC);
  };
  return C <= 64 ? rows(IntC<1>{}) : C <= 128 ? rows(IntC<2>{}) : rows(IntC<4>{});
}

int lion_internal_groupnorm_fold_se_plain(const float *stats, int B, int C, int T, int G, int voxels, const float *gamma,
                                          const float *beta, const float *fac, const float *gbias, int ld_fg, float eps,
                                          const float *w1, const float *w2, int H, float *A, float *Bs, lionStream_t stream) {
  if (int e = gn_fold_se_args(stats, B, C, T, G, gamma, beta, fac, gbias, ld_fg, w1, w2, H, A, Bs)) return e;
  return lion_launch<gn_fold_se_kernel>(B, 256, 0, static_cast<hipStream_t>(stream), stats, C, T, G, (float)voxels,
                                        gamma, beta, fac, gbias, ld_fg, eps, w1, w2, H, A, Bs);
}

int lion_groupnorm_fold(const float *stats, int B, int C, int T, int G, int voxels, const float *gamma,
                        const float *beta, const float *fac, const float *gbias, int ld_fg, float eps,
                        float *A, float *Bs, float *chmean, lionStream_t stream) {
  if (!stats || !gamma || !beta || !fac || !gbias || !A || !Bs || !chmean) return LION_EINVAL;
  if (B <= 0 || C <= 0 || T <= 0 || G <= 0 || C % G != 0 || C / G > 64 || ld_fg < C) return LION_EINVAL;
  return lion_launch<gn_fold_kernel>(dim3(G, B), 256, 0, static_cast<hipStream_t>(stream), stats, C, T, G,
                                     (float)voxels, gamma, beta, fac, gbias, ld_fg, eps, A, Bs, chmean);
}

}
```

lion_amd/csrc/devoxelize.hip:

```cpp
#include "common.h"

namespace {

struct Corners {
  int ix[8];
  float w[8];
};

__device__ __forceinline__ Corners corners_of(float x, float y, float z, int r, int r2) {
  Corners k;
  const float xl = floorf(x), yl = floorf(y), zl = floorf(z);
  const float xd1 = sub_rn(x, xl), yd1 = sub_rn(y, yl), zd1 = sub_rn(z, zl);
  const float xd0 = sub_rn(1.0f, xd1), yd0 = sub_rn(1.0f, yd1), zd0 = sub_rn(1.0f, zd1);
  k.w[0] = mul_rn(mul_rn(xd0, yd0), zd0);
  k.w[1] = mul_rn(mul_rn(xd0, yd0), zd1);
  k.w[2] = mul_rn(mul_rn(xd0, yd1), zd0);
  k.w[3] = mul_rn(mul_rn(xd0, yd1), zd1);
  k.w[4] = mul_rn(mul_rn(xd1, yd0), zd0);
  k.w[5] = mul_rn(mul_rn(xd1, yd0), zd1);
  k.w[6] = mul_rn(mul_rn(xd1, yd1), zd0);
  k.w[7] = mul_rn(mul_rn(xd1, yd1), zd1);
  const int xlo = (int)xl, ylo = (int)yl, zlo = (int)zl;
  const int xs = (xd1 > 0.0f) ? r2 : 0;
  const int ys = (yd1 > 0.0f) ? r : 0;
  const int zs = (zd1 > 0.0f) ? 1 : 0;
  k.ix[0] = xlo * r2 + ylo * r + zlo;
  k.ix[1] = k.ix[0] + zs;
  k.ix[2] = k.ix[0] + ys;
  k.ix[3] = k.ix[2] + zs;
  k.ix[4] = k.ix[0] + xs;
  k.ix[5] = k.ix[4] + zs;
  k.ix[6] = k.ix[4] + ys;
  k.ix[7] = k.ix[6] + zs;
  return k;
}

template <int CT, bool AFF>
__global__ __launch_bounds__(256) void devox_fwd_kernel(const float *__restrict__ coords,
                                                        const float *__restrict__ feat, int C,
                                                        int N, int r, int training,
                                                        float *__restrict__ out,
                                                        int32_t *__restrict__ inds,
                                                        float *__restrict__ wgts,
                                                        const float *__restrict__ scale,
                                                        const float *__restrict__ shift) {
  const int b = blockIdx.z, i = blockIdx.x * blockDim.x + threadIdx.x;
  if (i >= N) return;
  const int r2 = r * r, r3 = r2 * r;
  const float *co = coords + (size_t)b * 3 * N;
  Corners k = corners_of(co[i], co[i + N], co[i + 2 * N], r, r2);
  if (training && blockIdx.y == 0) {
#pragma unroll
    for (int q = 0; q < 8; ++q) {
      wgts[((size_t)b * 8 + q) * N + i] = k.w[q];
      inds[((size_t)b * 8 + q) * N + i] = k.ix[q];
    }
  }
#pragma unroll
  for (int q = 0; q < 8; ++q) k.ix[q] = min(max(k.ix[q], 0), r3 - 1);
  const int c0 = blockIdx.y * CT, c1 = min(C, c0 + CT);
  const float *f = feat + ((size_t)b * C + c0) * r3;
  float *o = out + ((size_t)b * C + c0) * N + i;
  float wsum = 0.f;
  if (AFF) {
    wsum = k.w[0];
#pragma unroll
    for (int q = 1; q < 8; ++q) wsum += k.w[q];
  }
#pragma unroll 4
  for (int c = c0; c < c1; ++c, f += r3, o += N) {
    float v[8];
#pragma unroll
    for (int q = 0; q < 8; ++q) v[q] = f[k.ix[q]];
    float acc = mul_rn(k.w[0], v[0]);
#pragma unroll
    for (int q = 1; q < 8; ++q) acc = add_rn(acc, mul_rn(k.w[q], v[q]));
    if (AFF) acc = acc * scale[(size_t)b * C + c] + shift[(size_t)b * C + c] * wsum;
    *o = acc;
  }
}


template <int LD, bool AFF, bool SPLIT, bool ONE>
__global__ __launch_bounds__(256) void devox_slab_kernel(
    const float *__restrict__ coords, const float *__restrict__ feat, int C, int N, int r, int PX,
    int XS_rt, int CT, int CI, int slab_floats, int training, float *__restrict__ out,
    int32_t *__restrict__ inds, float *__restrict__ wgts, const float *__restrict__ scale,
    const float *__restrict__ shift) {
  static_assert(!(ONE && SPLIT), "the single-slab form fetches whole grids: there is no row-end rule to apply");
  constexpr bool FILT = !ONE;
  extern __shared__ __attribute__((aligned(16))) unsigned char smem[];
  float *lds = reinterpret_cast<float *>(smem);
  constexpr int PP = 8;
  const int XS = ONE ? 1 : XS_rt;
  const int tid = threadIdx.x, b = blockIdx.y, c0 = blockIdx.x * CT;
  const int nch = min(CT, C - c0);
  const int r2 = r * r, r3 = r2 * r;
  const float *co = coords + (size_t)b * 3 * N;
  uint16_t *sorted = reinterpret_cast<uint16_t *>(lds + 2 * slab_floats);
  int *scnt = reinterpret_cast<int *>(sorted + ((N + 1) & ~1));
  unsigned *need = reinterpret_cast<unsigned *>(scnt + XS);

  const int ngrp = (nch + CI - 1) / CI;
  const int nit = ngrp * XS;
  auto slab_count4 = [&](int g, int xs) {
    return XS == 1 ? (min(CI, nch - g * CI) * r3) >> 2 : ((min(r, xs * PX + PX + 1) - xs * PX) * r2) >> 2;
  };
  typedef __attribute__((address_space(3))) float lds_float;
  const uint32_t lds_base = (uint32_t)(uintptr_t)(lds_float *)lds;
  const int wave = __builtin_amdgcn_readfirstlane(tid >> 6);
  auto issue = [&](int it) {
    const int g = it / XS, xs = it - g * XS;
    const float4 *src = reinterpret_cast<const float4 *>(feat + ((size_t)b * C + c0 + g * CI) * r3 + (size_t)xs * PX * r2);
    const int n4 = slab_count4(g, xs);
    const uint32_t dst0 = lds_base + (uint32_t)((it & 1) * slab_floats * 4 + wave * 1024);
    const int row0 = XS == 1 ? 0 : xs * PX * r;
#pragma unroll
    for (int j = 0; j < LD; ++j) {
      const int f = tid + j * 256;
      const float4 *gp = src + f;
      const uint32_t dst = __builtin_amdgcn_readfirstlane(dst0 + j * 4096);
      bool want;
      if (FILT) {
        int row = (4 * f) / r;
        if (XS == 1) row %= r2;
        else row += row0;
        want = f < n4 && ((need[row >> 5] >> (row & 31)) & 1u);
        if (SPLIT && !want && f < n4) {
          int rowh = (4 * f + 3) / r;
          if (XS == 1) rowh %= r2;
          else rowh += row0;
          want = (need[rowh >> 5] >> (rowh & 31)) & 1u;
        }
      } else {
        want = f < n4;
      }
      if (want) {
        unsigned keep;
        asm volatile("s_mov_b32 %0, m0\n\ts_mov_b32 m0, %2\n\ts_nop 0\n\tglobal_load_lds_dwordx4 %1, off\n\ts_mov_b32 m0, %0"
                     : "=&s"(keep) : "v"(gp), "s"(dst) : "memory");
      }
    }
  };
  float cx[PP], cy[PP], cz[PP];
  if constexpr (ONE) {
#pragma unroll
    for (int p = 0; p < PP; ++p) {
      const int i = tid + p * 256;
      cx[p] = cy[p] = cz[p] = 0.f;
      if (i < N) { cx[p] = co[i]; cy[p] = co[i + N]; cz[p] = co[i + 2 * N]; }
    }
    issue(0);
  } else {
    const int nwords = (r2 + 31) >> 5;
    for (int w = tid; w < nwords; w += 256) need[w] = 0u;
    __syncthreads();
    for (int i = tid; i < N; i += 256) {
      const float x = co[i], y = co[i + N];
      const float xl = floorf(x), yl = floorf(y);
      if (xl >= 0.f && yl >= 0.f && xl < (float)r && yl < (float)r) {
        const int x0 = (int)xl, y0 = (int)yl;
        const int x1 = min(x0 + (sub_rn(x, xl) > 0.0f ? 1 : 0), r - 1), y1 = min(y0 + (sub_rn(y, yl) > 0.0f ? 1 : 0), r - 1);
        const int ra = x0 * r + y0, rb = x0 * r + y1, rc = x1 * r + y0, rd = x1 * r + y1;
        atomicOr(&need[ra >> 5], 1u << (ra & 31));
        atomicOr(&need[rb >> 5], 1u << (rb & 31));
        atomicOr(&need[rc >> 5], 1u << (rc & 31));
        atomicOr(&need[rd >> 5], 1u << (rd & 31));
      }
    }
    __syncthreads();
    issue(0);

    for (int s2 = tid; s2 < XS; s2 += 256) scnt[s2] = 0;
    __syncthreads();
    int sl0[PP];
#pragma unroll
    for (int p = 0; p < PP; ++p) {
      const int i = tid + p * 256;
      sl0[p] = -1;
      if (i < N) {
        sl0[p] = min(max((int)floorf(co[i]) / PX, 0), XS - 1);
        if (XS > 1) atomicAdd(&scnt[sl0[p]], 1);
      }
    }
    __syncthreads();
    if (tid == 0) {
      int run = 0;
      for (int s2 = 0; s2 < XS; ++s2) { const int c = scnt[s2]; scnt[s2] = run; run += c; }
    }
    __syncthreads();
#pragma unroll
    for (int p = 0; p < PP; ++p) {
      const int i = tid + p * 256;
      if (i < N) sorted[XS > 1 ? atomicAdd(&scnt[sl0[p]], 1) : i] = (uint16_t)i;
    }
    __syncthreads();
  }

  int ix0[PP], xsl[PP], pid[PP];
  float xd1[PP], yd1[PP], zd1[PP];
#pragma unroll
  for (int p = 0; p < PP; ++p) {
    const int k = tid + p * 256;
    xsl[p] = -1;
    ix0[p] = 0;
    pid[p] = 0;
    xd1[p] = yd1[p] = zd1[p] = 0.f;
    if (k < N) {
      const int i = ONE ? k : (int)sorted[k];
      pid[p] = i;
      const float x = ONE ? cx[p] : co[i], y = ONE ? cy[p] : co[i + N], z = ONE ? cz[p] : co[i + 2 * N];
      const Corners kk = corners_of(x, y, z, r, r2);
      if (training && blockIdx.x == 0) {
#pragma unroll
        for (int q = 0; q < 8; ++q) {
          wgts[((size_t)b * 8 + q) * N + i] = kk.w[q];
          inds[((size_t)b * 8 + q) * N + i] = kk.ix[q];
        }
      }
      const float xl = floorf(x), yl = floorf(y), zl = floorf(z);
      xd1[p] = sub_rn(x, xl);
      yd1[p] = sub_rn(y, yl);
      zd1[p] = sub_rn(z, zl);
      ix0[p] = kk.ix[0];
      xsl[p] = min(max((int)xl / PX, 0), XS - 1);
      const int xin = (int)xl - xsl[p] * PX;
      const bool ok = xl >= 0.f && yl >= 0.f && zl >= 0.f && xl < (float)r && yl < (float)r && zl < (float)r &&
                      kk.ix[7] < r3 && xin >= 0 && xin < PX;
      if (!ok) xsl[p] = -2;
    }
  }

  for (int it = 0; it < nit; ++it) {
    const int g = it / XS, xs = it - g * XS;
    const int cg = c0 + g * CI, cin = min(CI, nch - g * CI);
    float *buf = lds + (it & 1) * slab_floats;
    asm volatile("s_waitcnt vmcnt(0)" ::: "memory");
    __syncthreads();
    if (it + 1 < nit) issue(it + 1);
    const int base = xs * PX * r2;
    float *o = out + ((size_t)b * C + cg) * N;
#pragma unroll
    for (int p = 0; p < PP; ++p) {
      if (xsl[p] == xs) {
        const float xd0 = sub_rn(1.0f, xd1[p]), yd0 = sub_rn(1.0f, yd1[p]), zd0 = sub_rn(1.0f, zd1[p]);
        const int xo = (xd1[p] > 0.0f) ? r2 : 0, yo = (yd1[p] > 0.0f) ? r : 0, zo = (zd1[p] > 0.0f) ? 1 : 0;
        const float w0 = mul_rn(mul_rn(xd0, yd0), zd0), w1 = mul_rn(mul_rn(xd0, yd0), zd1[p]);
        const float w2 = mul_rn(mul_rn(xd0, yd1[p]), zd0), w3 = mul_rn(mul_rn(xd0, yd1[p]), zd1[p]);
        const float w4 = mul_rn(mul_rn(xd1[p], yd0), zd0), w5 = mul_rn(mul_rn(xd1[p], yd0), zd1[p]);
        const float w6 = mul_rn(mul_rn(xd1[p], yd1[p]), zd0), w7 = mul_rn(mul_rn(xd1[p], yd1[p]), zd1[p]);
        float wsum = w0;
        if (AFF) { wsum += w1; wsum += w2; wsum += w3; wsum += w4; wsum += w5; wsum += w6; wsum += w7; }
        const float *f0 = buf + (ix0[p] - base);
        for (int ci = 0; ci < cin; ++ci, f0 += r3) {
          const float *f1 = f0 + xo;
          const float v0 = f0[0], v1 = f0[zo], v2 = f0[yo], v3 = f0[yo + zo];
          const float v4 = f1[0], v5 = f1[zo], v6 = f1[yo], v7 = f1[yo + zo];
          float a = mul_rn(w0, v0);
          a = add_rn(a, mul_rn(w1, v1));
          a = add_rn(a, mul_rn(w2, v2));
          a = add_rn(a, mul_rn(w3, v3));
          a = add_rn(a, mul_rn(w4, v4));
          a = add_rn(a, mul_rn(w5, v5));
          a = add_rn(a, mul_rn(w6, v6));
          a = add_rn(a, mul_rn(w7, v7));
          if (AFF) a = a * scale[(size_t)b * C + cg + ci] + shift[(size_t)b * C + cg + ci] * wsum;
          o[(size_t)ci * N + pid[p]] = a;
        }
      } else if (xsl[p] == -2 && xs == 0) {
        for (int ci = 0; ci < cin; ++ci) o[(size_t)ci * N + pid[p]] = 0.f;
      }
    }
  }
}

constexpr int DVR_R = 32, DVR_NT = 512, DVR_PP = 2048 / DVR_NT;
constexpr int DVR_RING_BYTES = 144 * 1024;
constexpr int DVR_NJ = 9;

__device__ __forceinline__ void wait_vm_uniform(int n) {
  n = __builtin_amdgcn_readfirstlane(n);
#define LION_WVM(k) case k: asm volatile("s_waitcnt vmcnt(" #k ")" ::: "memory"); break;
  switch (n < 0 ? 0 : n) {
    LION_WVM(0) LION_WVM(1) LION_WVM(2) LION_WVM(3) LION_WVM(4) LION_WVM(5) LION_WVM(6) LION_WVM(7) LION_WVM(8) LION_WVM(9)
    LION_WVM(10) LION_WVM(11) LION_WVM(12) LION_WVM(13) LION_WVM(14) LION_WVM(15) LION_WVM(16) LION_WVM(17) LION_WVM(18)
    LION_WVM(19) LION_WVM(20) LION_WVM(21) LION_WVM(22) LION_WVM(23) LION_WVM(24) LION_WVM(25) LION_WVM(26) LION_WVM(27)
    LION_WVM(28) LION_WVM(29) LION_WVM(30) LION_WVM(31) LION_WVM(32) LION_WVM(33) LION_WVM(34) LION_WVM(35) LION_WVM(36)
    LION_WVM(37) LION_WVM(38) LION_WVM(39)
  default: asm volatile("s_waitcnt vmcnt(40)" ::: "memory"); break;
  }
#undef LION_WVM
}

template <int G> constexpr int devox_plan_stride() { return 16 + (DVR_NJ * DVR_NT / (G / 4)) * 2 + 2048 * 16 + 2048; }

template <bool AFF, int G, int MODE>
__global__ __launch_bounds__(DVR_NT) void devox_ring_kernel(const float *__restrict__ coords,
                                                            const float *__restrict__ feat, int C, int N, int CT,
                                                            int training, float *__restrict__ out,
                                                            int32_t *__restrict__ inds, float *__restrict__ wgts,
                                                            const float *__restrict__ scale,
                                                            const float *__restrict__ shift, int dmax,
                                                            unsigned char *__restrict__ plan) {
  extern __shared__ __attribute__((aligned(16))) unsigned char smem[];
  constexpr int PP = DVR_PP, r = DVR_R, r2 = r * r, r3 = r2 * r, NT = DVR_NT;
  constexpr int PPR = r / G, NP = r2 * PPR, nwords = NP / 32, LP = G / 4;
  constexpr int NPMAX = DVR_NJ * NT / LP;
  static_assert(nwords <= 128, "two bitmap words per lane of the ranking wave");
  float *lds = reinterpret_cast<float *>(smem);
  const int tid = threadIdx.x, b = blockIdx.y, c0 = blockIdx.x * CT;
  const int nch = min(CT, C - c0);
  unsigned *need = reinterpret_cast<unsigned *>(smem + DVR_RING_BYTES);
  unsigned *base = need + nwords;
  uint16_t *plist = reinterpret_cast<uint16_t *>(base + nwords);
  float *s_sc = reinterpret_cast<float *>(plist + NPMAX);
  int *s_np = reinterpret_cast<int *>(s_sc + 32);
  const float *co = coords + (size_t)b * 3 * N;
  unsigned char *pl_b = (MODE != 0) ? plan + (size_t)b * devox_plan_stride<G>() : nullptr;
  const uint16_t *pl_list = reinterpret_cast<const uint16_t *>(pl_b + 16);
  uint16_t *pl_off = reinterpret_cast<uint16_t *>(pl_b + 16 + NPMAX * 2);
  signed char *pl_st = reinterpret_cast<signed char *>(pl_b + 16 + NPMAX * 2 + 2048 * 16);

  if (tid < nwords) need[tid] = 0u;
  if (AFF && tid < 2 * 16) {
    const int ci = tid & 15;
    s_sc[tid] = ci < nch ? (tid < 16 ? scale : shift)[(size_t)b * C + c0 + ci] : 0.f;
  }
  __syncthreads();
  int np = 0, nj = 0, buf_bytes = 0, D = 2;
  bool fits = false;
  int goff[DVR_NJ];
  typedef __attribute__((address_space(3))) float lds_float;
  const uint32_t lds_base = (uint32_t)(uintptr_t)(lds_float *)lds;
  const int wave = __builtin_amdgcn_readfirstlane(tid >> 6);
  int ops = 0;
  int mark[4] = {0, 0, 0, 0};
  auto ring_shape = [&]() {
    nj = (np * LP + NT - 1) / NT;
    buf_bytes = nj * NT * 16;
    D = nj == 0 ? 2 : min(min(dmax, 4), DVR_RING_BYTES / (nj ? buf_bytes : 1));
    fits = nj <= DVR_NJ && D >= 2;
  };
  auto issue = [&](int ci) {
    const float *src = feat + ((size_t)b * C + c0 + ci) * r3;
    const uint32_t dst0 = lds_base + (uint32_t)((ci % D) * buf_bytes + wave * 1024);
#pragma unroll
    for (int j = 0; j < DVR_NJ; ++j) {
      if (j < nj) {
        const uint32_t dst = __builtin_amdgcn_readfirstlane(dst0 + j * (NT * 16));
        const float *gp = src + goff[j];
        unsigned keep;
        asm volatile("s_mov_b32 %0, m0\n\ts_mov_b32 m0, %2\n\ts_nop 0\n\tglobal_load_lds_dwordx4 %1, off nt\n\ts_mov_b32 m0, %0"
                     : "=&s"(keep) : "v"(gp), "s"(dst) : "memory");
      }
    }
    ops += nj;
    mark[ci % D] = ops;
  };
  if (MODE == 1) {
    const int *hdr = reinterpret_cast<const int *>(pl_b);
    unsigned pl[DVR_NJ];
#pragma unroll
    for (int j = 0; j < DVR_NJ; ++j) pl[j] = pl_list[(tid + j * NT) / LP];
    np = __builtin_amdgcn_readfirstlane(hdr[0]);
    ring_shape();
    fits = fits && hdr[1] != 0;
    const int n4 = fits ? np * LP : 0;
#pragma unroll
    for (int j = 0; j < DVR_NJ; ++j) {
      const int f = tid + j * NT;
      goff[j] = f < n4 ? (int)pl[j] * G + (f % LP) * 4 : 0;
    }
    if (fits)
      for (int k = 0; k < D - 1 && k < nch; ++k) issue(k);
  }
  float xd1[PP], yd1[PP], zd1[PP];
  int row4[PP][4], zl_[PP], st[PP];
#pragma unroll
  for (int p = 0; p < PP; ++p) {
    const int i = tid + p * NT;
    st[p] = 0;
    xd1[p] = yd1[p] = zd1[p] = 0.f;
    row4[p][0] = row4[p][1] = row4[p][2] = row4[p][3] = zl_[p] = 0;
    if (i < N) {
      const float x = co[i], y = co[i + N], z = co[i + 2 * N];
      const Corners kk = corners_of(x, y, z, r, r2);
      if (training && blockIdx.x == 0) {
#pragma unroll
        for (int q = 0; q < 8; ++q) {
          wgts[((size_t)b * 8 + q) * N + i] = kk.w[q];
          inds[((size_t)b * 8 + q) * N + i] = kk.ix[q];
        }
      }
      const float xl = floorf(x), yl = floorf(y), zl = floorf(z);
      xd1[p] = sub_rn(x, xl);
      yd1[p] = sub_rn(y, yl);
      zd1[p] = sub_rn(z, zl);
      const bool ok = xl >= 0.f && yl >= 0.f && zl >= 0.f && xl < (float)r && yl < (float)r && zl < (float)r &&
                      kk.ix[7] < r3;
      st[p] = ok ? 1 : -2;
      if (ok) {
        const int x0 = (int)xl, y0 = (int)yl;
        const int x1 = x0 + (xd1[p] > 0.0f ? 1 : 0), y1 = y0 + (yd1[p] > 0.0f ? 1 : 0);
        zl_[p] = (int)zl;
        row4[p][0] = x0 * r + y0; row4[p][1] = x0 * r + y1; row4[p][2] = x1 * r + y0; row4[p][3] = x1 * r + y1;
        if (zl_[p] == r - 1 && zd1[p] > 0.0f) st[p] = 2;
      }
      if (MODE != 1 && st[p] == 1) {
        const int zh = zl_[p] + (zd1[p] > 0.0f ? 1 : 0);
#pragma unroll
        for (int k = 0; k < 4; ++k) {
          const int pl = row4[p][k] * PPR + zl_[p] / G, ph = row4[p][k] * PPR + zh / G;
          atomicOr(&need[pl >> 5], 1u << (pl & 31));
          if (ph != pl) atomicOr(&need[ph >> 5], 1u << (ph & 31));
        }
      }
    }
  }
  auto slot_of = [&](int pc) { return (int)(base[pc >> 5] + __popc(need[pc >> 5] & ((1u << (pc & 31)) - 1u))); };
  if (MODE != 1) {
    __syncthreads();
    if (tid < 64) {
      const int w0 = 2 * tid, w1 = 2 * tid + 1;
      const int c0_ = w0 < nwords ? __popc(need[w0]) : 0, c1_ = w1 < nwords ? __popc(need[w1]) : 0;
// ... 171 lines not shown
  int ix[8];
  float w[8];
  for (int q = 0; q < 8; ++q) {
    ix[q] = min(max(inds[((size_t)b * 8 + q) * N + i], 0), r3 - 1);
    w[q] = wgts[((size_t)b * 8 + q) * N + i];
  }
  const int c0 = blockIdx.y * CT, c1 = min(C, c0 + CT);
  for (int c = c0; c < c1; ++c) {
    const float gv = gy[((size_t)b * C + c) * N + i];
    for (int q = 0; q < 8; ++q) atomicAdd(gx + ((size_t)b * C + c) * r3 + ix[q], mul_rn(w[q], gv));
  }
}

}

constexpr int DVR_G = 8;
constexpr size_t DVR_LDS = (size_t)DVR_RING_BYTES + (size_t)2 * (DVR_R * DVR_R * (DVR_R / DVR_G) / 32) * 4 +
                           (size_t)(DVR_NJ * DVR_NT / (DVR_G / 4)) * 2 + 32 * 4 + 16;
static int devox_ring_depth() {
  static const int d = getenv("LION_DEVOX_RING") ? atoi(getenv("LION_DEVOX_RING")) : 4;
  return d < 2 ? 2 : d;
}

static int devox_ring_ct(int B, int C) {
  int CT = 8;
  while (CT > 1 && (long)B * lion_cdiv(C, CT) < 256) CT >>= 1;
  return CT;
}

template <int MODE>
static int devox_ring_launch(const float *coords, const float *feat, int B, int C, int N, int training, float *out,
                             int32_t *inds, float *wgts, const float *scale, const float *shift, unsigned char *plan,
                             hipStream_t st) {
  const int CT = devox_ring_ct(B, C);
  return lion_with_flags(scale != nullptr, [&](auto AFFINE) {
    return lion_launch<devox_ring_kernel<decltype(AFFINE)::value, DVR_G, MODE>>(
        dim3(lion_cdiv(C, CT), B), DVR_NT, DVR_LDS, st, coords, feat, C, N, CT, training, out, inds, wgts, scale, shift,
        devox_ring_depth(), plan);
  });
}

enum DevoxKind { DEVOX_RING = 0, DEVOX_SLAB = 1, DEVOX_GATHER = 2 };
struct DevoxPlan {
  DevoxKind kind;
  int PX, XS, CI, ld, slab_floats;
  int ct;
  size_t lds;
  dim3 grid;
};

static DevoxPlan devox_plan(int B, int C, int N, int r, bool aligned) {
  DevoxPlan p = {DEVOX_GATHER, 0, 0, 0, 0, 0, 0, 0, dim3()};
  const int r2 = r * r;
  if (r == DVR_R && N <= 2048 && aligned) {
    p.kind = DEVOX_RING;
    p.ct = devox_ring_ct(B, C);
    p.lds = DVR_LDS;
    p.grid = dim3(lion_cdiv(C, p.ct), B);
  } else if ((r2 % 4) == 0 && N <= 2048 && r2 <= 4608 && aligned) {
    p.kind = DEVOX_SLAB;
    const int planes_max = 9216 / r2;
    p.PX = planes_max >= r ? r : planes_max - 1;
    p.XS = lion_cdiv(r, p.PX);
    p.CI = p.XS == 1 ? (9216 / (r2 * r) < 16 ? 9216 / (r2 * r) : 16) : 1;
    const int ld0 = lion_cdiv((p.XS == 1 ? p.CI * r2 * r : (p.PX + 1) * r2) / 4, 256);
    p.ld = ld0 <= 1 ? 1 : ld0 <= 2 ? 2 : ld0 <= 4 ? 4 : 9;
    p.slab_floats = p.ld * 1024;
    p.lds = (size_t)2 * p.slab_floats * 4 + (size_t)((N + 1) & ~1) * 2 + (size_t)p.XS * 4 + (size_t)((r2 + 31) / 32) * 4;
    p.ct = 4 * p.CI;
    while (p.ct > p.CI && (long)B * lion_cdiv(C, p.ct) < 512) p.ct >>= 1;
    p.grid = dim3(lion_cdiv(C, p.ct), B);
  } else {
    const int pt = lion_cdiv(N, 256);
    p.ct = 16;
    while (p.ct > 2 && (long)B * pt * lion_cdiv(C, p.ct) < 2048) p.ct >>= 1;
    p.grid = dim3(pt, lion_cdiv(C, p.ct), B);
  }
  return p;
}

template <typename F> static int devox_ld_dispatch(int ld, F f) {
  switch (ld) {
  case 1: return f(IntC<1>{});
  case 2: return f(IntC<2>{});
  case 4: return f(IntC<4>{});
  default: return f(IntC<9>{});
  }
}
template <typename F> static int devox_ct_dispatch(int ct, F f) {
  switch (ct) {
  case 16: return f(IntC<16>{});
  case 8: return f(IntC<8>{});
  case 4: return f(IntC<4>{});
  default: return f(IntC<2>{});
  }
}

extern "C" {

static int devox_launch(const float *coords, const float *feat, int B, int C, int N, int r,
                        int training, float *out, int32_t *inds, float *wgts, const float *scale,
                        const float *shift, hipStream_t st) {
  const DevoxPlan p = devox_plan(B, C, N, r, (((uintptr_t)feat) & 15) == 0);
  if (p.kind == DEVOX_RING)
    return devox_ring_launch<0>(coords, feat, B, C, N, training, out, inds, wgts, scale, shift, nullptr, st);
  if (p.kind == DEVOX_SLAB) {
    auto slab = [&](auto LD, auto SPLIT, auto ONE) {
      return lion_with_flags(scale != nullptr, [&](auto AFFINE) {
        return lion_launch<devox_slab_kernel<decltype(LD)::value, decltype(AFFINE)::value, decltype(SPLIT)::value,
                                             decltype(ONE)::value>>(
            p.grid, 256, p.lds, st, coords, feat, C, N, r, p.PX, p.XS, p.ct, p.CI, p.slab_floats, training, out, inds, wgts,
            scale, shift);
      });
    };
    if (p.XS > 1) {
      if (p.ld != 9) return LION_EUNSUPPORTED;
      return lion_with_flags((r & 3) != 0, [&](auto SPLIT) { return slab(IntC<9>{}, SPLIT, BoolC<false>{}); });
    }
    return devox_ld_dispatch(p.ld, [&](auto LD) { return slab(LD, BoolC<false>{}, BoolC<true>{}); });
  }
  return devox_ct_dispatch(p.ct, [&](auto CT) {
    return lion_with_flags(scale != nullptr, [&](auto AFFINE) {
      return lion_launch<devox_fwd_kernel<decltype(CT)::value, decltype(AFFINE)::value>>(
          p.grid, 256, 0, st, coords, feat, C, N, r, training, out, inds, wgts, scale, shift);
    });
  });
}

int lion_internal_devoxelize_path(int B, int C, int N, int r, int aligned, int32_t *out, lionStream_t) {
  if (!out || B <= 0 || C <= 0 || N <= 0 || r <= 0) return LION_EINVAL;
  const DevoxPlan p = devox_plan(B, C, N, r, aligned != 0);
  const int32_t v[8] = {p.kind, p.PX, p.XS, p.CI, p.ld, p.ct, (int32_t)p.lds, (int32_t)p.grid.x};
  for (int k = 0; k < 8; ++k) out[k] = v[k];
  return LION_OK;
}

int lion_trilinear_devoxelize_forward(const float *coords, const float *feat, int B, int C, int N,
                                      int r, int training, float *out, int32_t *inds, float *wgts,
                                      lionStream_t stream) {
  if (!coords || !feat || !out || B <= 0 || C <= 0 || N <= 0 || r <= 0) return LION_EINVAL;
  if (training && (!inds || !wgts)) return LION_EINVAL;
  return devox_launch(coords, feat, B, C, N, r, training, out, inds, wgts, nullptr, nullptr,
                      static_cast<hipStream_t>(stream));
}

int lion_trilinear_devoxelize_affine_forward(const float *coords, const float *feat, const float *scale,
                                             const float *shift, int B, int C, int N, int r, float *out,
                                             lionStream_t stream) {
  if (!coords || !feat || !out || !scale || !shift || B <= 0 || C <= 0 || N <= 0 || r <= 0) return LION_EINVAL;
  return devox_launch(coords, feat, B, C, N, r, 0, out, nullptr, nullptr, scale, shift,
                      static_cast<hipStream_t>(stream));
}

size_t lion_devoxelize_plan_bytes(int B, int N, int r) {
  if (B <= 0 || N <= 0 || N > 2048 || r != DVR_R) return 0;
  return (size_t)B * devox_plan_stride<DVR_G>();
}

int lion_trilinear_devoxelize_plan(const float *coords, int B, int N, int r, void *plan, size_t plan_bytes,
                                   lionStream_t stream) {
  if (!coords || !plan || B <= 0 || N <= 0) return LION_EINVAL;
  const size_t need = lion_devoxelize_plan_bytes(B, N, r);
  if (!need || (((uintptr_t)plan) & 15) != 0) return LION_EUNSUPPORTED;
  if (plan_bytes < need) return LION_EWORKSPACE;
  return lion_launch<devox_ring_kernel<false, DVR_G, 2>>(dim3(1, B), DVR_NT, DVR_LDS, static_cast<hipStream_t>(stream),
                                                         coords, nullptr, 1, N, 1, 0, nullptr, nullptr, nullptr,
                                                         nullptr, nullptr, devox_ring_depth(),
                                                         static_cast<unsigned char *>(plan));
}

int lion_trilinear_devoxelize_planned_forward(const void *plan, size_t plan_bytes, const float *coords, const float *feat,
                                              const float *scale, const float *shift, int B, int C, int N, int r,
                                              float *out, lionStream_t stream) {
  if (!plan || !coords || !feat || !out || B <= 0 || C <= 0 || N <= 0) return LION_EINVAL;
  if ((scale == nullptr) != (shift == nullptr)) return LION_EINVAL;
  const size_t need = lion_devoxelize_plan_bytes(B, N, r);
  if (!need || (((uintptr_t)plan) & 15) != 0 || (((uintptr_t)feat) & 15) != 0) return LION_EUNSUPPORTED;
  if (plan_bytes < need) return LION_EWORKSPACE;
  hipStream_t st = static_cast<hipStream_t>(stream);
  unsigned char *pl = const_cast<unsigned char *>(static_cast<const unsigned char *>(plan));
  return devox_ring_launch<1>(coords, feat, B, C, N, 0, out, nullptr, nullptr, scale, shift, pl, st);
}

struct DevoxBwdPlan { int parts, nt; size_t lds; };
static DevoxBwdPlan devox_bwd_plan(int r3) {
  int parts = (size_t)r3 * 4 > 64 * 1024 ? 2 : 1;
  if (r3 % (4 * parts) != 0) parts = 1;
  return {parts, r3 >= 16384 ? 1024 : 256, (size_t)(r3 / parts) * 4};
}

int lion_trilinear_devoxelize_backward(const float *gy, const int32_t *inds, const float *wgts,
                                       int B, int C, int N, int r3, float *gx,
                                       lionStream_t stream) {
  if (!gy || !inds || !wgts || !gx || B <= 0 || C <= 0 || N <= 0 || r3 <= 0) return LION_EINVAL;
  hipStream_t st = static_cast<hipStream_t>(stream);
  if ((size_t)r3 * 4 <= 128 * 1024 && (r3 % 4) == 0) {
    const DevoxBwdPlan p = devox_bwd_plan(r3);
    return lion_launch<devox_bwd_lds_kernel<false>>(dim3(C, B, p.parts), p.nt, p.lds, st, gy, inds, wgts, nullptr, nullptr,
                                                    nullptr, nullptr, C, N, r3, gx);
  }
  hipError_t e = hipMemsetAsync(gx, 0, (size_t)B * C * r3 * 4, st);
  if (e != hipSuccess) return (int)e;
  const int CT = 8;
  return lion_launch<devox_bwd_atomic_kernel>(dim3(lion_cdiv(N, 256), lion_cdiv(C, CT), B), 256, 0, st, gy, inds, wgts,
                                              C, N, r3, CT, gx);
}

int lion_trilinear_devoxelize_backward_affine(const float *gy, const int32_t *inds, const float *wgts, const float *x,
                                              const float *Ap, const float *Q, const float *R, int B, int C, int N, int r3,
                                              float *dx, lionStream_t stream) {
  if (!gy || !inds || !wgts || !x || !Ap || !Q || !R || !dx || B <= 0 || C <= 0 || N <= 0 || r3 <= 0) return LION_EINVAL;
  if ((size_t)r3 * 4 > 128 * 1024 || (r3 % 8) != 0 || (((uintptr_t)x | (uintptr_t)dx) & 15) != 0) return LION_EUNSUPPORTED;
  const DevoxBwdPlan p = devox_bwd_plan(r3);
  return lion_launch<devox_bwd_lds_kernel<true>>(dim3(C, B, p.parts), p.nt, p.lds, static_cast<hipStream_t>(stream), gy, inds,
                                                 wgts, x, Ap, Q, R, C, N, r3, dx);
}

}
```

lion_amd/csrc/pointwise.hip:

```cpp
#include "common.h"

namespace {

__device__ __forceinline__ float swishf(float t) { return swish_fast(t); }

__global__ __launch_bounds__(256) void row_stats_kernel(const float *__restrict__ x, int L,
                                                        float *__restrict__ stats) {
  __shared__ float r1[4], r2[4];
  const int row = blockIdx.x, tid = threadIdx.x, lane = tid & 63, wave = tid >> 6;
  const float *p = x + (size_t)row * L;
  float s1 = 0.f, s2 = 0.f;
  if ((L & 3) == 0) {
    for (int i = tid * 4; i < L; i += 1024) {
      const float4 v = *reinterpret_cast<const float4 *>(p + i);
      s1 += (v.x + v.y) + (v.z + v.w);
      s2 += (v.x * v.x + v.y * v.y) + (v.z * v.z + v.w * v.w);
    }
  } else {
    for (int i = tid; i < L; i += 256) { const float v = p[i]; s1 += v; s2 += v * v; }
  }
  s1 = row16_sum_rn(s1); s2 = row16_sum_rn(s2);
#pragma unroll
  for (int m = 16; m < 64; m <<= 1) { s1 += __shfl_xor(s1, m, 64); s2 += __shfl_xor(s2, m, 64); }
  if (lane == 0) { r1[wave] = s1; r2[wave] = s2; }
  __syncthreads();
  if (tid == 0) {
    stats[(size_t)row * 2] = (r1[0] + r1[1]) + (r1[2] + r1[3]);
    stats[(size_t)row * 2 + 1] = (r2[0] + r2[1]) + (r2[2] + r2[3]);
  }
}

__global__ __launch_bounds__(256) void affine_swish_kernel(const float *__restrict__ x,
                                                           const float *__restrict__ A,
                                                           const float *__restrict__ Bs, int L,
                                                           float *__restrict__ y) {
  const int row = blockIdx.y;
  const float a = A[row], b = Bs[row];
  const float *p = x + (size_t)row * L;
  float *q = y + (size_t)row * L;
  const int i = (blockIdx.x * 256 + threadIdx.x) * 4;
  if (i + 3 < L && (L & 3) == 0) {
    const float4 v = *reinterpret_cast<const float4 *>(p + i);
    *reinterpret_cast<float4 *>(q + i) =
        make_float4(swishf(v.x * a + b), swishf(v.y * a + b), swishf(v.z * a + b), swishf(v.w * a + b));
  } else {
    for (int j = i; j < L && j < i + 4; ++j) q[j] = swishf(p[j] * a + b);
  }
}

__global__ __launch_bounds__(256) void affine_swish_add_kernel(const float *__restrict__ x, const float *__restrict__ A,
                                                               const float *__restrict__ Bs,
                                                               const float *__restrict__ addend, int L,
                                                               float *__restrict__ y) {
  const int row = blockIdx.y;
  const float a = A[row], b = Bs[row];
  const float *p = x + (size_t)row * L, *ad = addend + (size_t)row * L;
  float *q = y + (size_t)row * L;
  const int i = (blockIdx.x * 256 + threadIdx.x) * 4;
  if (i + 3 < L && (L & 3) == 0) {
    const float4 v = *reinterpret_cast<const float4 *>(p + i), w = *reinterpret_cast<const float4 *>(ad + i);
    *reinterpret_cast<float4 *>(q + i) = make_float4(swishf(v.x * a + b) + w.x, swishf(v.y * a + b) + w.y,
                                                     swishf(v.z * a + b) + w.z, swishf(v.w * a + b) + w.w);
  } else {
    for (int j = i; j < L && j < i + 4; ++j) q[j] = swishf(p[j] * a + b) + ad[j];
  }
}

__global__ void timestep_embedding_kernel(const float *__restrict__ t, const float *__restrict__ row, float scale, int B,
                                          int half, int D, float *__restrict__ emb) {
  const int e = blockIdx.x * blockDim.x + threadIdx.x;
  if (e >= B * D) return;
  const int b = e / D, i = e - b * D;
  float v = 0.f;
  if (i < 2 * half) {
    const float ang = mul_rn(mul_rn(t[b], scale), row[i < half ? i : i - half]);
    v = i < half ? sinf(ang) : cosf(ang);
  }
  emb[e] = v;
}

__global__ __launch_bounds__(256) void affine_swish_max_kernel(const float *__restrict__ x,
                                                               const float *__restrict__ A,
                                                               const float *__restrict__ Bs, int M,
                                                               int U, float *__restrict__ y) {
  const int row = blockIdx.y, m = blockIdx.x * 256 + threadIdx.x;
  if (m >= M) return;
  const float a = A[row], b = Bs[row];
  const float *p = x + ((size_t)row * M + m) * U;
  float best = -INFINITY;
  if ((U & 3) == 0) {
    for (int u = 0; u < U; u += 4) {
      const float4 v = *reinterpret_cast<const float4 *>(p + u);
      best = fmaxf(best, fmaxf(fmaxf(swishf(v.x * a + b), swishf(v.y * a + b)),
                               fmaxf(swishf(v.z * a + b), swishf(v.w * a + b))));
    }
  } else {
    for (int u = 0; u < U; ++u) best = fmaxf(best, swishf(p[u] * a + b));
  }
  y[(size_t)row * M + m] = best;
}

template <int LPM>
__global__ __launch_bounds__(256) void affine_swish_max_coop_kernel(const float *__restrict__ x,
                                                                    const float *__restrict__ A,
                                                                    const float *__restrict__ Bs, int M,
                                                                    float *__restrict__ y) {
  constexpr int MPW = 64 / LPM;
  constexpr int IT = 8;
  const int row = blockIdx.y, lane = threadIdx.x & 63, wave = threadIdx.x >> 6;
  const float a = A[row], b = Bs[row];
  const int m0 = (blockIdx.x * 4 + wave) * MPW * IT;
  const float4 *p = reinterpret_cast<const float4 *>(x + (size_t)row * M * (LPM * 4));
  float4 v[IT];
#pragma unroll
  for (int i = 0; i < IT; ++i) {
    const int m = min(m0 + i * MPW + lane / LPM, M - 1);
    v[i] = p[(size_t)m * LPM + (lane % LPM)];
  }
#pragma unroll
  for (int i = 0; i < IT; ++i) {
    float best = fmaxf(fmaxf(swishf(v[i].x * a + b), swishf(v[i].y * a + b)),
                       fmaxf(swishf(v[i].z * a + b), swishf(v[i].w * a + b)));
    if (LPM >= 2) best = fmaxf(best, LION_DPP_F32(best, 0xB1));
    if (LPM >= 4) best = fmaxf(best, LION_DPP_F32(best, 0x4E));
    if (LPM >= 8) best = fmaxf(best, LION_DPP_F32(best, 0x141));
    if (LPM >= 16) best = fmaxf(best, LION_DPP_F32(best, 0x140));
    const int m = m0 + i * MPW + lane / LPM;
    if ((lane % LPM) == 0 && m < M) y[(size_t)row * M + m] = best;
  }
}

__global__ __launch_bounds__(256) void se_gate_kernel(const float *__restrict__ chmean,
                                                      const float *__restrict__ w1,
                                                      const float *__restrict__ w2, int C, int H,
                                                      float *__restrict__ A, float *__restrict__ Bs) {
  __shared__ float sm[1024], sh[128];
  const int b = blockIdx.x, tid = threadIdx.x, lane = tid & 63, wave = tid >> 6;
  for (int c = tid; c < C; c += 256) sm[c] = A[(size_t)b * C + c] * chmean[(size_t)b * C + c] + Bs[(size_t)b * C + c];
  __syncthreads();
  for (int j = wave; j < H; j += 4) {
    float acc = 0.f;
    for (int c = lane; c < C; c += 64) acc += w1[(size_t)j * C + c] * sm[c];
#pragma unroll
    for (int m = 32; m >= 1; m >>= 1) acc += __shfl_xor(acc, m, 64);
    if (lane == 0) sh[j] = acc > 0.f ? acc : 0.f;
  }
  __syncthreads();
  for (int c = tid; c < C; c += 256) {
    float acc = 0.f;
    for (int j = 0; j < H; ++j) acc += w2[(size_t)c * H + j] * sh[j];
    const float g = 1.0f / (1.0f + expf(-acc));
    A[(size_t)b * C + c] *= g;
    Bs[(size_t)b * C + c] *= g;
  }
}


__global__ __launch_bounds__(256) void latent_unpack_kernel(const float *__restrict__ x, int N, int D,
                                                            float *__restrict__ all, float *__restrict__ coords,
                                                            float *__restrict__ rest) {
  __shared__ float tile[256 * 9];
  const int b = blockIdx.y, n0 = blockIdx.x * 256, tid = threadIdx.x;
  const int np = min(256, N - n0);
  const float *src = x + ((size_t)b * N + n0) * D;
  for (int i = tid; i < np * D; i += 256) tile[(i / D) * (D + 1) + i % D] = src[i];
  __syncthreads();
  if (tid >= np) return;
  for (int d = 0; d < D; ++d) {
    const float v = tile[tid * (D + 1) + d];
    if (all) all[((size_t)b * D + d) * N + n0 + tid] = v;
    if (coords && d < 3) coords[((size_t)b * 3 + d) * N + n0 + tid] = v;
    if (rest && d >= 3) rest[((size_t)b * (D - 3) + d - 3) * N + n0 + tid] = v;
  }
}

__global__ __launch_bounds__(256) void concat_broadcast_kernel(const float *__restrict__ a, const float *__restrict__ t,
                                                               int Ca, int Ct, int N4, int ld_t, float4 *__restrict__ out) {
  const int row = blockIdx.y, C = Ca + Ct, b = row / C, c = row % C;
  float4 *o = out + (size_t)row * N4;
  if (c < Ca) {
    const float4 *s = reinterpret_cast<const float4 *>(a) + ((size_t)b * Ca + c) * N4;
    for (int i = blockIdx.x * 256 + threadIdx.x; i < N4; i += gridDim.x * 256) o[i] = s[i];
  } else {
    const float v = t[(size_t)b * ld_t + c - Ca];
    for (int i = blockIdx.x * 256 + threadIdx.x; i < N4; i += gridDim.x * 256) o[i] = make_float4(v, v, v, v);
  }
}

}

constexpr int kMaxGridY = 65535;

extern "C" {

int lion_row_stats(const float *x, int rows, int L, float *stats, lionStream_t stream) {
  if (!x || !stats || rows <= 0 || L <= 0) return LION_EINVAL;
  return lion_launch<row_stats_kernel>(rows, 256, 0, static_cast<hipStream_t>(stream), x, L, stats);
}

int lion_affine_swish(const float *x, const float *A, const float *Bs, int rows, int L, float *y,
                      lionStream_t stream) {
  if (!x || !A || !Bs || !y || rows <= 0 || L <= 0) return LION_EINVAL;
  for (int r0 = 0; r0 < rows; r0 += kMaxGridY) {
    const int nr = rows - r0 < kMaxGridY ? rows - r0 : kMaxGridY;
    const size_t off = (size_t)r0 * L;
    if (int e = lion_launch<affine_swish_kernel>(dim3(lion_cdiv(lion_cdiv(L, 4), 256), nr), 256, 0,
                                                 static_cast<hipStream_t>(stream), x + off, A + r0, Bs + r0, L,
                                                 y + off))
      return e;
  }
  return 0;
}

int lion_timestep_embedding(const float *t, const float *row, float scale, int B, int half, int D, float *emb,
                            lionStream_t stream) {
  if (!t || !row || !emb || B <= 0 || half <= 0 || D < 2 * half) return LION_EINVAL;
  return lion_launch<timestep_embedding_kernel>(lion_cdiv(B * D, 256), 256, 0, static_cast<hipStream_t>(stream), t, row,
// ... 68 lines not shown
```

lion_amd/fused_ops.py:

```python
import collections
import os

import torch

from . import _lib
from ._wcache import WeightCache
from . import conv_ops
from .conv_ops import supported


def _border_sums(weight):
    m = torch.tensor([[0., 1., 1.], [1., 1., 1.], [1., 1., 0.]], dtype=torch.float64, device=weight.device)
    ws = torch.einsum("oidhw,ad,bh,cw->abcio", weight.detach().double(), m, m, m)
    return ws.reshape(27, weight.shape[1], weight.shape[0]).float().contiguous()


_WSUM_CACHE = WeightCache(_border_sums)


def border_weight_sums(weight):
    return _WSUM_CACHE.get(weight)


def conv3d_occupancy(counts, r, cout, b, consumer_aware=False):
    lib = _lib.load()
    n = lib.lion_conv3d_occupancy_ints(r, cout, b)
    buf = torch.empty((2, n), device=counts.device, dtype=torch.int32)
    _lib.call("lion_conv3d_tile_occupancy_aware", counts.contiguous(), b, r, cout, buf[0], buf[1], int(consumer_aware))
    return buf[0], buf[1]


class FoldSpec:

    def __init__(self, gn: torch.nn.GroupNorm, fac, gbias, count, se=None):
        self.gn, self.fac, self.gbias, self.count, self.se = gn, fac, gbias, int(count), se

    def apply(self, stats):
        if self.se is not None:
            merged = groupnorm_fold_se(stats, self.gn, self.fac, self.gbias, self.count, self.se)
            if merged is not None:
                return merged
            a, b_, m = groupnorm_fold(stats, self.gn, self.fac, self.gbias, self.count)
            return se_gate_(a, b_, m, self.se)
        a, b_, _ = groupnorm_fold(stats, self.gn, self.fac, self.gbias, self.count)
        return a, b_


def _pro_pair(pro):
    return (None, None) if pro is None else (pro[0].contiguous(), pro[1].contiguous())


def _bias(bias):
    return None if bias is None else bias.detach().contiguous()


def conv3d_fused(x, conv, pro=None, want_stats=True, occ=None, prev_conv=None, split=None, fold=None):
    lib = _lib.load()
    b, cin, r = x.shape[0], x.shape[1], x.shape[2]
    cout = conv.out_channels
    route = conv_ops.conv_route(cin, cout, r, split, x)
    assert pro is None or cin % 4 == 0
    x = conv_ops.pad_cin4(x)
    cin = x.shape[1]
    wp = route.packed(conv.weight)
    y = torch.empty((b, cout, r, r, r), device=x.device, dtype=torch.float32)
    pbias = tconst = None
    pa, pb = _pro_pair(pro)
    bias = _bias(conv.bias)
    sparse = occ is not None and r >= 16
    if sparse and pro is not None:
        if prev_conv is None or cin > 256:
            sparse = False
        else:
            ws = border_weight_sums(conv.weight)
            pbias = _bias(prev_conv.bias)
            tconst = torch.empty((b, 27, cout), device=x.device, dtype=torch.float32)
            _lib.call("lion_conv3d_const_response", ws, bias, pbias, pa, pb, b, cin, cout, tconst)
    stats = None
    if want_stats:
        query = getattr(lib, route.stat_tiles)
        tiles = query(r, cout, b, int(sparse)) if route.kind == "f32" else query(r, cout)
        stats = torch.empty((b, cout, tiles, 2), device=x.device, dtype=torch.float32)
    if not sparse:
        occ = None
    _lib.call(route.forward, x, wp, bias, b, cin, cout, r, pa, pb, pbias, tconst, y, stats, occ)
    if fold is not None:
        return y, fold.apply(stats)
    return y, stats


def groupnorm_fold(stats, gn: torch.nn.GroupNorm, fac, gbias, voxels):
    b, c, t, _ = stats.shape
    A = torch.empty((b, c), device=stats.device, dtype=torch.float32)
    Bs = torch.empty_like(A)
    cm = torch.empty_like(A)
    if not (fac.stride(1) == 1 and gbias.stride(1) == 1 and fac.stride(0) == gbias.stride(0) and fac.stride(0) >= c):
        fac, gbias = fac.contiguous(), gbias.contiguous()
    _lib.call("lion_groupnorm_fold", stats, b, c, t, gn.num_groups, int(voxels), gn.weight, gn.bias, fac, gbias,
              int(fac.stride(0)), float(gn.eps), A, Bs, cm)
    return A, Bs, cm


def groupnorm_fold_se(stats, gn: torch.nn.GroupNorm, fac, gbias, voxels, se):
    b, c, t, _ = stats.shape
    w1, w2 = se.fc[0].weight.detach(), se.fc[2].weight.detach()
    h = w1.shape[0]
    if c > 256 or c < 4 or h > 128 or not (w1.is_contiguous() and w2.is_contiguous()):
        return None
    A = torch.empty((b, c), device=stats.device, dtype=torch.float32)
    Bs = torch.empty_like(A)
    if not (fac.stride(1) == 1 and gbias.stride(1) == 1 and fac.stride(0) == gbias.stride(0) and fac.stride(0) >= c):
        fac, gbias = fac.contiguous(), gbias.contiguous()
    _lib.call("lion_groupnorm_fold_se", stats, b, c, t, gn.num_groups, int(voxels), gn.weight, gn.bias, fac, gbias,
              int(fac.stride(0)), float(gn.eps), w1, w2, h, A, Bs)
    return A, Bs


def se_gate_(A, Bs, chmean, se):
    w1, w2 = se.fc[0].weight.detach(), se.fc[2].weight.detach()
    h, c = w1.shape
    if c > 1024 or h > 128 or not (w1.is_contiguous() and w2.is_contiguous()):
        gate = se.fc(A * chmean + Bs)
        return A * gate, Bs * gate
    _lib.call("lion_se_gate", chmean, w1, w2, A.shape[0], c, h, A, Bs)
    return A, Bs


def devoxelize_plan(coords, r):
    lib = _lib.load()
    b, _, n = coords.shape
    nbytes = lib.lion_devoxelize_plan_bytes(b, n, int(r))
    if nbytes == 0 or not coords.is_contiguous() or coords.dtype != torch.float32:
        return None
    buf = torch.empty((nbytes,), device=coords.device, dtype=torch.uint8)
    _lib.call("lion_trilinear_devoxelize_plan", coords, b, n, int(r), buf, nbytes)
    return {"buf": buf, "coords": coords, "shape": (b, n, int(r))}


def devoxelize_affine(grid, coords, r, scale, shift, plan=None):
    b, c = grid.shape[:2]
    n = coords.shape[2]
    out = torch.empty((b, c, n), device=grid.device, dtype=torch.float32)
    co_c, gr_c, sc_c, sh_c = coords.contiguous(), grid.contiguous(), scale.contiguous(), shift.contiguous()
    if plan is not None and plan["shape"] == (b, n, int(r)) and plan["coords"].data_ptr() == co_c.data_ptr():
        buf = plan["buf"]
        _lib.call("lion_trilinear_devoxelize_planned_forward", buf, buf.numel(), co_c, gr_c, sc_c, sh_c, b, c, n, int(r), out)
        return out
    _lib.call("lion_trilinear_devoxelize_affine_forward", co_c, gr_c, sc_c, sh_c, b, c, n, int(r), out)
    return out


def fusable(conv1, conv2, r, x):
    return (x.is_cuda and x.dtype == torch.float32 and not torch.is_autocast_enabled()
            and supported(conv1.in_channels, conv1.out_channels, r)
            and supported(conv2.in_channels, conv2.out_channels, r)
            and conv2.in_channels % 4 == 0 and conv2.in_channels <= 256)


def _pw_pack(weight):
    return conv_ops.pack_with(weight, "lion_pwconv_packed_floats", "lion_pwconv_pack_weights", torch.float32, as_matrix=True)


_PW_CACHE = WeightCache(_pw_pack)
PW_ALL = os.environ.get("LION_PW_ALL", "1") != "0"


def pw_packed_weight(weight):
    return _PW_CACHE.get(weight)


def _pw_split_pack(weight):
    return conv_ops.pack_with(weight, "lion_pwconv_split_packed_halfs", "lion_pwconv_split_pack_weights", torch.int16,
                              as_matrix=True)


_PW_SPLIT_CACHE = WeightCache(_pw_split_pack)
PW_SPLIT = os.environ.get("LION_PW_SPLIT", "1") != "0"


def pw_use_split(split, b, cin, cout, L):
    can = cin * L < (1 << 29) and cin <= 4096
    if split is None:
        return PW_SPLIT and can and b * L >= 8192 and (L <= 4096 or cin * cout >= 8192)
    return bool(split) and can


PwRoute = collections.namedtuple("PwRoute", "split forward grouped stat_tiles cache pack")
_PW_ROUTES = {
    False: PwRoute(False, "lion_pwconv_forward", "lion_pwconv_grouped_forward", "lion_pwconv_stat_tiles", _PW_CACHE, _pw_pack),
    True: PwRoute(True, "lion_pwconv_split_forward", "lion_pwconv_split_grouped_forward", "lion_pwconv_split_stat_tiles",
                  _PW_SPLIT_CACHE, _pw_split_pack)}


def pw_route(b, cin, cout, L, split=None):
    return _PW_ROUTES[pw_use_split(split, b, cin, cout, L)]


def _pw_stats(route, b, cin, cout, L, like):
    tiles = getattr(_lib.load(), route.stat_tiles)(cout, cin, L)
    return torch.empty((b, cout, tiles, 2), device=like.device, dtype=torch.float32)


def is_plain_1x1(conv):
    return (conv.groups == 1 and all(k == 1 for k in conv.kernel_size) and all(s == 1 for s in conv.stride)
            and all(p == 0 for p in conv.padding))


def pw_supported(conv, x):
    if not PW_ALL:
        L = x[0, 0].numel()
        if not (conv.out_channels in (32, 64, 128, 256) and L >= 1024 and x.shape[0] * L * conv.out_channels >= (1 << 22)):
            return False
    return (is_plain_1x1(conv) and x.is_cuda and x.dtype == torch.float32 and x[0, 0].numel() > 0
            and _lib.load().lion_pwconv_stat_tiles(conv.out_channels, conv.in_channels, x[0, 0].numel()) > 0)


def pwconv_fused(x, conv, pro=None, want_stats=True, split=None):
    x = x.contiguous()
    b, cin = x.shape[:2]
    L = x[0, 0].numel()
    cout = conv.out_channels
    route = pw_route(b, cin, cout, L, split)
    y = torch.empty((b, cout) + tuple(x.shape[2:]), device=x.device, dtype=torch.float32)
    stats = _pw_stats(route, b, cin, cout, L, x) if want_stats else None
    pa, pb = _pro_pair(pro)
    _lib.call(route.forward, x, route.cache.get(conv.weight), _bias(conv.bias), b, cin, cout, L, pa, pb, y, stats)
    return y, stats


MAX_RECOMPUTE = os.environ.get("LION_PW_MAX_RECOMPUTE", "0") != "0"


def pwconv_max_recompute(x, conv, gn, style, pro):
    lib = _lib.load()
    x = x.contiguous()
    b, cin, m, u = x.shape
    L = m * u
    cout = conv.out_channels
    wp = pw_packed_weight(conv.weight)
    tiles = lib.lion_pwconv_stat_tiles(cout, cin, L)
    if tiles <= 0:
        return None
    stats = torch.empty((b, cout, tiles, 2), device=x.device, dtype=torch.float32)
    pa, pb = _pro_pair(pro)
    bias = _bias(conv.bias)
    if not _lib.call("lion_pwconv_forward_max", x, wp, bias, b, cin, cout, L, pa, pb, None, None, stats, None,
                     unsupported_ok=True):
        return None
    f, g = gn.affine(style)
    A, Bs, _ = groupnorm_fold(stats, gn.norm, f, g, L)
    y = torch.empty((b, cout, m), device=x.device, dtype=torch.float32)
    _lib.call("lion_pwconv_forward_max", x, wp, bias, b, cin, cout, L, pa, pb, A, Bs, None, y)
    return y


def pwconv_raw(x, w2d, bias=None, cached_param=None, transposed=False):
    lib = _lib.load()
    x = x.contiguous()
    b, cin = x.shape[:2]
    cout = w2d.shape[1] if transposed else w2d.shape[0]
    L = x[0, 0].numel()
    if not (x.is_cuda and x.dtype == torch.float32 and L > 0 and lib.lion_pwconv_stat_tiles(cout, cin, L) > 0):
        return None
    route = pw_route(b, cin, cout, L)
    if transposed and route.split and cached_param is not None:
        wf = route.cache.get(cached_param)
        wp = torch.empty((lib.lion_pwconv_split_packed_halfs(cout, cin),), device=x.device, dtype=torch.int16)
        _lib.call("lion_pwconv_split_pack_weights_t", w2d.detach().contiguous(), cin, cout, wf, wp)
    elif transposed:
        wp = route.pack(w2d.detach().t().contiguous())
    elif cached_param is not None:
        wp = route.cache.get(cached_param)
    else:
        wp = route.pack(w2d)
    y = torch.empty((b, cout) + tuple(x.shape[2:]), device=x.device, dtype=torch.float32)
    _lib.call(route.forward, x, wp, _bias(bias), b, cin, cout, L, None, None, y, None)
    return y


def pwconv_wgrad(x, gy, want_bias=False):
    lib = _lib.load()
    x, gy = x.contiguous(), gy.contiguous()
    b, cin = x.shape[:2]
    cout = gy.shape[1]
    L = x[0, 0].numel()
    wsb = lib.lion_pwconv_wgrad_workspace_bytes(b, cin, cout, L)
    ws = torch.empty((wsb,), device=x.device, dtype=torch.uint8)
    gw = torch.empty((cout, cin), device=x.device, dtype=torch.float32)
    gb = torch.empty((cout,), device=x.device, dtype=torch.float32) if want_bias else None
    _lib.call("lion_pwconv_wgrad", x, gy, b, cin, cout, L, ws, wsb, gw, gb)
    return (gw, gb) if want_bias else gw


def group_points(coords, centers, feat, idx):
    b, _, n = coords.shape
    m, u = idx.shape[1], idx.shape[2]
    c = 0 if feat is None else feat.shape[1]
    out = torch.empty((b, 3 + c, m, u), device=coords.device, dtype=torch.float32)
    _lib.call("lion_group_points_forward", coords.contiguous(), centers.contiguous(), None if feat is None else feat.contiguous(),
              idx.contiguous(), b, c, n, m, u, out)
    return out

# ... 250 lines not shown
```

lion_amd/models/pvcnn2_ada.py:

```python
import contextlib
import functools
import os

import torch
import torch.nn as nn
from einops import rearrange

from .. import functional as F
from ..functional import backend
from ..conv_ops import conv3d_module
from .. import fused_ops

FUSE_INFERENCE = True
SPARSE_CONV1 = True
OVERLAP_POINT_BRANCH = os.environ.get("LION_OVERLAP_POINT_BRANCH", "0") != "0"
_POINT_STREAMS = {}


_VOX_PLANS = None
VOX_PLAN = os.environ.get("LION_VOX_PLAN", "1") != "0"
OCC_PLAN = os.environ.get("LION_OCC_PLAN", "1") != "0"
SKIP_UNREAD = os.environ.get("LION_CONV_SKIP_UNREAD", "1") != "0"
SKIP_UNREAD_LEVEL2 = os.environ.get("LION_CONV_SKIP_UNREAD_LEVEL2", "1") != "0"
OCC_CLONE = os.environ.get("LION_OCC_CLONE", "0") != "0"
DEVOX_PLAN = os.environ.get("LION_DEVOX_PLAN", "1") != "0"
SA_GATHER = os.environ.get("LION_SA_GATHER", "1") != "0"


@contextlib.contextmanager
def voxel_plans():
    global _VOX_PLANS
    prev, _VOX_PLANS = _VOX_PLANS, ({} if VOX_PLAN else None)
    try:
        yield
    finally:
        _VOX_PLANS = prev


class VoxelGeometry:

    def __init__(self, coords, r, normalize, eps, plan, scoped):
        self.coords, self.r, self.normalize, self.eps, self.plan, self.scoped = coords, r, normalize, eps, plan, scoped
        self.norm, self.cnt = (plan["norm"], plan["cnt"]) if plan is not None else (None, None)
        self._occ, self._devox = {}, False

    def scatter(self, features, reader_level=0):
        b, c = features.shape[:2]
        if self.plan is None:
            out, self.norm, _, self.cnt = backend._backend.voxelize_points_forward(
                features.float().contiguous(), self.coords, self.r, self.normalize, self.eps)
        else:
            aware = reader_level and SKIP_UNREAD and SPARSE_CONV1 and self.r in (16, 32)
            occ_m1 = self.occupancy(reader_level, 64)[0] if aware else None
            out = backend._backend.voxel_scatter(features.float().contiguous(), self.plan, occ_m1)
        return out.view(b, c, self.r, self.r, self.r)

    def occupancy(self, level, cout):
        keep = self.scoped and OCC_PLAN
        occ = self._occ.get(level) if keep else None
        if occ is None:
            occ = fused_ops.conv3d_occupancy(self.cnt, self.r, cout, self.cnt.shape[0], consumer_aware=level)
            if keep:
                self._occ[level] = occ
        if keep and OCC_CLONE:
            return occ[0].clone(), occ[1].clone()
        return occ

    def devox_plan(self):
        if not (self.scoped and DEVOX_PLAN) or self.r != 32 or self.norm.shape[2] > 2048 or not self.norm.is_contiguous():
            return None
        if self._devox is False:
            self._devox = fused_ops.devoxelize_plan(self.norm, self.r)
        return self._devox


def _point_stream(device):
    key = (device.type, device.index)
    if key not in _POINT_STREAMS:
        _POINT_STREAMS[key] = torch.cuda.Stream(device=device)
    return _POINT_STREAMS[key]
from .adagn import AdaGN


class SE3d(nn.Module):

    def __init__(self, channel, reduction=8):
        super().__init__()
        self.fc = nn.Sequential(
            nn.Linear(channel, channel // reduction, bias=False),
            nn.ReLU(inplace=True),
            nn.Linear(channel // reduction, channel, bias=False),
            nn.Sigmoid())
        self.channel = channel

    def __repr__(self):
        return f"SE({self.channel}, {self.channel})"

    def gate(self, inputs):
        return self.fc(inputs.mean(-1).mean(-1).mean(-1))

    def forward(self, inputs):
        return inputs * self.gate(inputs).view(inputs.shape[0], inputs.shape[1], 1, 1, 1)


class LinearAttention(nn.Module):

    def __init__(self, dim, heads=4, dim_head=32, verbose=True):
        super().__init__()
        self.heads = heads
        hidden_dim = dim_head * heads
        self.to_qkv = nn.Conv2d(dim, hidden_dim * 3, 1, bias=False)
        self.to_out = nn.Conv2d(hidden_dim, dim, 1)

    def forward(self, x):
        if own_kernels(x) and self.to_qkv.out_channels == 3 * self.heads * 32 and fused_ops.pw_supported(self.to_qkv, x):
            qkv = fused_ops.pwconv_fused(x, self.to_qkv, None, want_stats=False)[0]
            core = fused_ops.linear_attention_core(qkv, self.heads, 32)
            return fused_ops.pwconv_fused(core, self.to_out, None, want_stats=False)[0]
        x = x.unsqueeze(-1)
        b, c, h, w = x.shape
        qkv = self.to_qkv(x)
        from .. import train_ops
        if w == 1 and self.to_qkv.out_channels == 3 * self.heads * 32 and train_ops.attention_trainable(qkv.squeeze(-1), self.heads, 32):
            out = train_ops.linear_attention_core(qkv.squeeze(-1), self.heads)
            return self.to_out(out.unsqueeze(-1)).squeeze(-1)
        q, k, v = rearrange(qkv, 'b (qkv heads c) h w -> qkv b heads c (h w)', heads=self.heads, qkv=3)
        k = k.softmax(dim=-1)
        context = torch.einsum('bhdn,bhen->bhde', k, v)
        out = torch.einsum('bhde,bhdn->bhen', context, q)
        out = rearrange(out, 'b heads c (h w) -> b (heads c) h w', heads=self.heads, h=h, w=w)
        return self.to_out(out).squeeze(-1)


def swish(input):
    return input * torch.sigmoid(input)


class Swish(nn.Module):
    def forward(self, input):
        return swish(input)


class BallQuery(nn.Module):

    def __init__(self, radius, num_neighbors, include_coordinates=True):
        super().__init__()
        self.radius = radius
        self.num_neighbors = num_neighbors
        self.include_coordinates = include_coordinates

    def forward(self, points_coords, centers_coords, points_features=None, grouped_view=False):
        with torch.autocast("cuda", enabled=False):
            points_coords = points_coords.float().contiguous()
            centers_coords = centers_coords.float().contiguous()
            neighbor_indices = F.ball_query(centers_coords, points_coords, self.radius, self.num_neighbors)
            if own_kernels(points_coords) and self.include_coordinates and points_coords.shape[1] == 3 \
                    and (points_features is None or points_features.dtype == torch.float32):
                if grouped_view and SA_GATHER:
                    return fused_ops.GroupedPoints(points_coords, centers_coords, points_features, neighbor_indices)
                return fused_ops.group_points(points_coords, centers_coords, points_features, neighbor_indices)
            neighbor_coordinates = F.grouping(points_coords, neighbor_indices)
            neighbor_coordinates = neighbor_coordinates - centers_coords.unsqueeze(-1)
            if points_features is None:
                assert self.include_coordinates, 'No Features For Grouping'
                return neighbor_coordinates
            neighbor_features = F.grouping(points_features.float(), neighbor_indices)
            if self.include_coordinates:
                neighbor_features = torch.cat([neighbor_coordinates, neighbor_features], dim=1)
# ... 56 lines not shown
    i, n = 0, len(layers)
    while i < n:
        layer = layers[i]
        norm = _group_norm(layer, adaptive)
        if norm is not None and train_ops.usable(x, need_grad):
            fused_act = i + 1 < n and isinstance(layers[i + 1], Swish)
            factor, bias = layer.affine(style) if adaptive else (None, None)
            if (not fused_act and i + 1 < n and isinstance(layers[i + 1], SE3d) and x.dim() == 5
                    and train_ops.se3d_trainable(layers[i + 1], x, need_grad)):
                x = train_ops.adagn_se(x, norm, factor, bias, layers[i + 1])
                i += 2
                continue
            if reduce_max and i + (2 if fused_act else 1) == n and train_ops.adagn_act_max_usable(x, need_grad):
                return train_ops.adagn_act_max(x, norm, factor, bias, act=fused_act)
            i += 2 if fused_act else 1
            drop_p, used = train_ops.fusable_dropout(layers, i) if fused_act else (0.0, 0)
            x = train_ops.adagn_act(x, norm, factor, bias, act=fused_act, dropout_p=drop_p)
            i += used
            continue
        if adaptive and isinstance(layer, AdaGN):
            x = layer(x, style)
        elif isinstance(layer, convs):
            x = conv(layer, x)
        elif isinstance(layer, SE3d) and train_ops.se3d_trainable(layer, x, need_grad):
            x = train_ops.se3d(layer, x)
        else:
            x = layer(x)
        i += 1
    return x.max(dim=-1).values if reduce_max else x


def run_layers(layers, x, style, conv, reduce_max=False):
    return walk(layers, x, style, conv, reduce_max, adaptive=True)


def voxel_tail(layers, grid, style, voxel_coords, resolution, training, adaptive):
    from .. import train_ops
    norm = _group_norm(layers[-2], adaptive) if training and len(layers) >= 2 and isinstance(layers[-1], SE3d) else None
    if norm is not None and train_ops.usable(grid) and train_ops.adagn_se_devox_usable(grid, layers[-1]):
        grid = walk(layers[:-2], grid, style, conv3d_module, False, adaptive)
        factor, bias = layers[-2].affine(style) if adaptive else (None, None)
        return train_ops.adagn_se_devox(grid, norm, factor, bias, layers[-1], voxel_coords, resolution), None
    grid = walk(layers, grid, style, conv3d_module, False, adaptive)
    return F.trilinear_devoxelize(grid, voxel_coords, resolution, training), grid


class SharedMLP(nn.Module):

    def __init__(self, in_channels, out_channels, dim=1, cfg={}):
        assert len(cfg) > 0, cfg
        super().__init__()
        conv = nn.Conv1d if dim == 1 else nn.Conv2d
        if not isinstance(out_channels, (list, tuple)):
            out_channels = [out_channels]
        layers = []
        for oc in out_channels:
            layers += [conv(in_channels, oc, 1), AdaGN(dim, cfg, oc), Swish()]
            in_channels = oc
        self.layers = nn.ModuleList(layers)

    def _fusable(self, x):
        return own_kernels(x) and not self.training

    def _run(self, x, style, reduce_max=False, add=None):
        if isinstance(x, fused_ops.GroupedPoints) and not self._fusable(x.coords):
            x = x.materialize()
        if self._fusable(x if torch.is_tensor(x) else x.coords):
            n = len(self.layers) // 3
            convs, gns = [self.layers[3 * i] for i in range(n)], [self.layers[3 * i + 1] for i in range(n)]
            return fused_ops.shared_mlp(x, convs, gns, style, reduce_max, add=add)
        x = run_layers(list(self.layers), x, style, conv1x1, reduce_max=reduce_max)
        return x if add is None else x + add

    def forward_max(self, x, style):
        return self._run(x, style, reduce_max=True)

    def forward(self, *inputs):
        if len(inputs) == 1 and len(inputs[0]) == 4:
            inputs = inputs[0]
        if len(inputs) == 4:
            x, _, _, style = inputs
            return (self._run(x, style), *inputs[1:])
        if len(inputs) == 2:
            return self._run(*inputs)
        raise NotImplementedError


class Voxelization(nn.Module):

    def __init__(self, resolution, normalize=True, eps=0):
        super().__init__()
        self.r = int(resolution)
        self.normalize = normalize
        self.eps = eps

    def geometry(self, coords):
        co = coords.detach()[:, :3].float().contiguous()
        if _VOX_PLANS is None:
            return VoxelGeometry(co, self.r, self.normalize, self.eps, None, False)
        key = (co.data_ptr(), tuple(co.shape), self.r, bool(self.normalize), float(self.eps))
        geo = _VOX_PLANS.get(key)
        if geo is None:
            geo = VoxelGeometry(co, self.r, self.normalize, self.eps, backend._backend.voxel_index(co, self.r, self.normalize, self.eps), True)
            if geo.plan is not None:
                _VOX_PLANS[key] = geo
        return geo

    def forward(self, features, coords):
        coords = coords.detach()
        if features is None:
            _, norm_coords, _, _ = backend._backend.voxelize_points_forward(
                None, coords[:, :3].float().contiguous(), self.r, self.normalize, self.eps)
            return features, norm_coords
        return F.voxelize_points(features, coords, self.r, self.normalize, self.eps)

    def extra_repr(self):
        return 'resolution={}{}'.format(
            self.r, ', normalized eps = {}'.format(self.eps) if self.normalize else '')


class PVConv(nn.Module):

    def __init__(self, in_channels, out_channels, kernel_size, resolution, normalize=1, eps=0,
                 with_se=False, add_point_feat=True, attention=False, dropout=0.1, verbose=True,
                 cfg={}):
        super().__init__()
        assert len(cfg) > 0, cfg
        self.resolution = resolution
        self.voxelization = Voxelization(resolution, normalize=normalize, eps=eps)
        norm = functools.partial(AdaGN, 3, cfg)
        voxel_layers = [
            nn.Conv3d(in_channels, out_channels, kernel_size, stride=1, padding=kernel_size // 2),
            norm(out_channels),
            Swish(),
            nn.Dropout(dropout),
            nn.Conv3d(out_channels, out_channels, kernel_size, stride=1, padding=kernel_size // 2),
            norm(out_channels),
        ]
        if with_se:
            voxel_layers.append(SE3d(out_channels))
        self.voxel_layers = nn.ModuleList(voxel_layers)
        self.attn = LinearAttention(out_channels, verbose=verbose) if attention else None
        if add_point_feat:
            self.point_features = SharedMLP(in_channels, out_channels, cfg=cfg)
        self.add_point_feat = add_point_feat

    def _aware_level(self):
        if not SKIP_UNREAD:
            return 0
        from .. import conv_ops
        conv2 = self.voxel_layers[4]
        return 2 if (SKIP_UNREAD_LEVEL2 and conv_ops.use_split(None, conv2.in_channels, conv2.out_channels, self.resolution)) else 1

    def _fused_voxel_branch(self, grid, geo, style, level):
        conv1, gn1, conv2, gn2 = self.voxel_layers[0], self.voxel_layers[1], self.voxel_layers[4], self.voxel_layers[5]
        se = self.voxel_layers[6] if len(self.voxel_layers) > 6 else None
        r = self.resolution
        occ1 = occ2 = None
        if SPARSE_CONV1 and r >= 16:
            occ1, occ2 = geo.occupancy(level, conv1.out_channels)
        f1, g1 = gn1.affine(style)
        y1, (a1, b1) = fused_ops.conv3d_fused(grid, conv1, None, True, occ1,
                                              fold=fused_ops.FoldSpec(gn1.norm, f1, g1, r ** 3))
        f2, g2 = gn2.affine(style)
        y2, (a2, b2) = fused_ops.conv3d_fused(y1, conv2, (a1, b1), True, occ2, prev_conv=conv1,
                                              fold=fused_ops.FoldSpec(gn2.norm, f2, g2, r ** 3, se))
        return fused_ops.devoxelize_affine(y2, geo.norm, r, a2, b2, plan=geo.devox_plan())

    def forward(self, inputs):
        features, coords_input, time_emb, style = inputs
        coords = coords_input[:, :3] if coords_input.shape[1] > 3 else coords_input
        assert features.shape[0] == coords.shape[0] and features.shape[2] == coords.shape[2], \
            f'get feat: {features.shape} and {coords.shape}'
        assert coords.shape[1] == 3, f'expect coords: B,3,Npoint, get: {coords.shape}'
        infer = (FUSE_INFERENCE and not self.training and not torch.is_grad_enabled() and features.is_cuda
                 and not torch.is_autocast_enabled())
        will_fuse = infer and fused_ops.fusable(self.voxel_layers[0], self.voxel_layers[4], self.resolution, features.float())
        if infer:
            level = self._aware_level() if will_fuse else 0
            geo = self.voxelization.geometry(coords)
            grid, voxel_coords = geo.scatter(features, level), geo.norm
        else:
            grid, voxel_coords = self.voxelization(features, coords)
        if will_fuse:
            pf = None
            if self.add_point_feat and OVERLAP_POINT_BRANCH:
                main, side = torch.cuda.current_stream(features.device), _point_stream(features.device)
                side.wait_stream(main)
                with torch.cuda.stream(side):
                    pf = self.point_features(features, style)
            fused = self._fused_voxel_branch(grid, geo, style, level)
            if pf is not None:
                main.wait_stream(side)
                pf.record_stream(main)
                fused = fused + pf
            elif self.add_point_feat:
                fused = self.point_features._run(features, style, add=fused)
            if self.attn is not None:
                fused = self.attn(fused)
            return fused, coords_input, time_emb, style
        fused, grid = voxel_tail(list(self.voxel_layers), grid, style, voxel_coords, self.resolution, self.training, adaptive=True)
        if self.add_point_feat:
            fused = fused + self.point_features(features, style)
        if self.attn is not None:
            fused = self.attn(fused)
        return fused, coords_input, time_emb, style


class PointNetAModule(nn.Module):

    def __init__(self, in_channels, out_channels, include_coordinates=True, cfg={}):
        super().__init__()
        if not isinstance(out_channels, (list, tuple)):
            out_channels = [[out_channels]]
        elif not isinstance(out_channels[0], (list, tuple)):
            out_channels = [out_channels]
        mlps, total = [], 0
        for oc in out_channels:
            mlps.append(SharedMLP(in_channels + (3 if include_coordinates else 0), oc, dim=1, cfg=cfg))
            total += oc[-1]
        self.include_coordinates = include_coordinates
        self.out_channels = total
        self.mlps = nn.ModuleList(mlps)

    def forward(self, inputs):
        features, coords, time_emb, style = inputs
        if self.include_coordinates:
            features = torch.cat([features, coords], dim=1)
        coords = torch.zeros((coords.size(0), 3, 1), device=coords.device)
        pooled = [mlp(features, style).max(dim=-1, keepdim=True).values for mlp in self.mlps]
        return (torch.cat(pooled, dim=1) if len(pooled) > 1 else pooled[0]), coords, time_emb

    def extra_repr(self):
        return f'out_channels={self.out_channels}, include_coordinates={self.include_coordinates}'


class PointNetSAModule(nn.Module):

    def __init__(self, num_centers, radius, num_neighbors, in_channels, out_channels,
                 include_coordinates=True, cfg={}):
        super().__init__()
        if not isinstance(radius, (list, tuple)):
            radius = [radius]
        if not isinstance(num_neighbors, (list, tuple)):
            num_neighbors = [num_neighbors] * len(radius)
        assert len(radius) == len(num_neighbors)
        if not isinstance(out_channels, (list, tuple)):
            out_channels = [[out_channels]] * len(radius)
        elif not isinstance(out_channels[0], (list, tuple)):
            out_channels = [out_channels] * len(radius)
        assert len(radius) == len(out_channels)
        groupers, mlps, total = [], [], 0
        for rad, oc, nn_ in zip(radius, out_channels, num_neighbors):
            groupers.append(BallQuery(radius=rad, num_neighbors=nn_, include_coordinates=include_coordinates))
            mlps.append(SharedMLP(in_channels + (3 if include_coordinates else 0), oc, dim=2, cfg=cfg))
            total += oc[-1]
        self.num_centers = num_centers
        self.out_channels = total
        self.groupers = nn.ModuleList(groupers)
        self.mlps = nn.ModuleList(mlps)

    def forward(self, inputs):
        features, coords, time_emb, style = inputs[0], inputs[1], inputs[2], inputs[3]
        if coords.shape[1] > 3:
            coords = coords[:, :3]
        centers_coords = F.furthest_point_sample(coords, self.num_centers)
        S = centers_coords.shape[-1]
        if time_emb is not None and type(time_emb) is not dict:
            time_emb = time_emb[:, :, :S]
        pooled = [mlp.forward_max(grouper(coords, centers_coords, features, grouped_view=True), style)
                  for grouper, mlp in zip(self.groupers, self.mlps)]
        out = torch.cat(pooled, dim=1) if len(pooled) > 1 else pooled[0]
        return out, centers_coords, time_emb, style

    def extra_repr(self):
        return f'num_centers={self.num_centers}, out_channels={self.out_channels}'


class PointNetFPModule(nn.Module):

    def __init__(self, in_channels, out_channels, cfg={}):
        super().__init__()
        self.mlp = SharedMLP(in_channels=in_channels, out_channels=out_channels, dim=1, cfg=cfg)

    def forward(self, inputs):
        if len(inputs) == 5:
            points_coords, centers_coords, centers_features, time_emb, style = inputs
            points_features = None
        elif len(inputs) == 6:
            points_coords, centers_coords, centers_features, points_features, time_emb, style = inputs
        else:
            raise NotImplementedError
        interpolated = None
        if isinstance(centers_features, tuple):
            cfeat, ctemb = centers_features
            interpolated = fused_ops.three_nn_interpolate_cat(points_coords, centers_coords, cfeat, ctemb, points_features)
            if interpolated is None:
                centers_features = torch.cat([cfeat, ctemb], dim=1)
        if interpolated is None:
            interpolated = F.nearest_neighbor_interpolate(points_coords, centers_coords, centers_features)
            if points_features is not None:
                interpolated = torch.cat([interpolated, points_features], dim=1)
        if time_emb is not None:
            time_emb = time_emb[:, :, 0:1].expand(-1, -1, points_coords.shape[-1])
        return self.mlp(interpolated, style), points_coords, time_emb, style


def _linear_gn_relu(in_channels, out_channels):
    return nn.Sequential(nn.Linear(in_channels, out_channels), nn.GroupNorm(8, out_channels), Swish())


def create_mlp_components(in_channels, out_channels, classifier=False, dim=2, width_multiplier=1, cfg={}):
    r = width_multiplier
    block = _linear_gn_relu if dim == 1 else SharedMLP
    if not isinstance(out_channels, (list, tuple)):
        out_channels = [out_channels]
    if len(out_channels) == 0 or (len(out_channels) == 1 and out_channels[0] is None):
        return nn.Sequential(), in_channels, in_channels
    layers = []
    for oc in out_channels[:-1]:
        if oc < 1:
            layers.append(nn.Dropout(oc))
        else:
            oc = int(r * oc)
            layers.append(block(in_channels, oc, cfg=cfg))
            in_channels = oc
    if dim == 1:
        layers.append(nn.Linear(in_channels, out_channels[-1]) if classifier
                      else _linear_gn_relu(in_channels, int(r * out_channels[-1])))
    else:
        layers.append(nn.Conv1d(in_channels, out_channels[-1], 1) if classifier
                      else SharedMLP(in_channels, int(r * out_channels[-1])))
    return layers, out_channels[-1] if classifier else int(r * out_channels[-1])


def create_pointnet2_sa_components(sa_blocks, extra_feature_channels, input_dim=3, embed_dim=64,
                                   use_att=False, force_att=0, dropout=0.1, with_se=False,
                                   normalize=True, eps=0, has_temb=1, width_multiplier=1,
                                   voxel_resolution_multiplier=1, verbose=True, cfg={}):
    assert len(cfg) > 0, cfg
    r, vr = width_multiplier, voxel_resolution_multiplier
    in_channels = extra_feature_channels + input_dim
    sa_layers, sa_in_channels = [], []
    num_centers = None
    for c, (conv_configs, sa_configs) in enumerate(sa_blocks):
# ... 69 lines not shown
```

Before: 5.915.

## Fuse point-branch GroupNorm fold with voxel fold and apply it after devoxelize

In the PVConv inference path, the point-branch 1x1 conv now runs before the voxel branch. Its GroupNorm statistics are folded in the same launch as the first voxel conv's fold, using a new paired fold kernel. The point branch's affine+swish+add is then applied either inside the devoxelize kernel (behind LION_DEVOX_TAIL, off by default) or in a separate affine_swish pass over the devoxelized output. This removes a separate fold launch and the point-MLP finish, but adds a large templated tail path to the devoxelize kernel with register-held prefetch and select trees.

```diff
diff --git a/include/lion_hip.h b/include/lion_hip.h
--- a/include/lion_hip.h
+++ b/include/lion_hip.h
@@ -224,6 +224,12 @@
 int lion_groupnorm_fold(const float *stats, int B, int C, int T, int G, int voxels, const float *gamma,
                         const float *beta, const float *fac, const float *gbias, int ld_fg, float eps,
                         float *A, float *Bs, float *chmean, lionStream_t stream);
+int lion_groupnorm_fold_pair(int B, const float *stats0, int C0, int T0, int G0, int voxels0, const float *gamma0,
+                             const float *beta0, const float *fac0, const float *gbias0, int ld_fg0, float eps0,
+                             float *A0, float *Bs0, float *chmean0, const float *stats1, int C1, int T1, int G1,
+                             int voxels1, const float *gamma1, const float *beta1, const float *fac1,
+                             const float *gbias1, int ld_fg1, float eps1, float *A1, float *Bs1, float *chmean1,
+                             lionStream_t stream);
 size_t lion_conv3d_split_packed_halfs(int Cout, int Cin);
 int lion_conv3d_split_pack_weights(const float *w, int Cout, int Cin, uint16_t *wp, lionStream_t stream);
 int lion_conv3d_split_stat_tiles(int r, int Cout);
@@ -262,6 +268,10 @@
 int lion_trilinear_devoxelize_affine_forward(const float *coords, const float *feat, const float *scale,
                                              const float *shift, int B, int C, int N, int r, float *out,
                                              lionStream_t stream);
+int lion_trilinear_devoxelize_affine_tail_forward(const float *coords, const float *feat, const float *scale,
+                                                  const float *shift, const float *pw, const float *pw_a,
+                                                  const float *pw_b, int B, int C, int N, int r, float *out,
+                                                  lionStream_t stream);
 size_t lion_devoxelize_plan_bytes(int B, int N, int r);
 int lion_trilinear_devoxelize_plan(const float *coords, int B, int N, int r, void *plan, size_t plan_bytes,
                                    lionStream_t stream);
diff --git a/lion_amd/_lib.py b/lion_amd/_lib.py
--- a/lion_amd/_lib.py
+++ b/lion_amd/_lib.py
@@ -63,6 +63,7 @@
     "lion_conv3d_k3_split_forward": (_i, [_vp, _vp, _vp, _i, _i, _i, _i, _vp, _vp, _vp, _vp, _vp, _vp, _vp, _vp]),
     "lion_conv3d_k3_half_forward": (_i, [_vp, _vp, _vp, _i, _i, _i, _i, _vp, _vp, _vp, _vp, _vp, _vp, _vp, _vp]),
     "lion_groupnorm_fold": (_i, [_vp, _i, _i, _i, _i, _i, _vp, _vp, _vp, _vp, _i, _f, _vp, _vp, _vp, _vp]),
+    "lion_groupnorm_fold_pair": (_i, [_i] + 2 * [_vp, _i, _i, _i, _i, _vp, _vp, _vp, _vp, _i, _f, _vp, _vp, _vp] + [_vp]),
     "lion_groupnorm_fold_se": (_i, [_vp, _i, _i, _i, _i, _i, _vp, _vp, _vp, _vp, _i, _f, _vp, _vp, _i, _vp, _vp, _vp]),
     "lion_internal_groupnorm_fold_se_plain": (_i, [_vp, _i, _i, _i, _i, _i, _vp, _vp, _vp, _vp, _i, _f, _vp, _vp, _i, _vp, _vp, _vp]),
     "lion_skinny_packed_floats": (_sz, [_i, _i]),
@@ -77,6 +78,7 @@
     "lion_from_channel_major": (_i, [_vp, _i, _i, _vp, _vp]),
     "lion_se_gate": (_i, [_vp, _vp, _vp, _i, _i, _i, _vp, _vp, _vp]),
     "lion_trilinear_devoxelize_affine_forward": (_i, [_vp, _vp, _vp, _vp, _i, _i, _i, _i, _vp, _vp]),
+    "lion_trilinear_devoxelize_affine_tail_forward": (_i, [_vp, _vp, _vp, _vp, _vp, _vp, _vp, _i, _i, _i, _i, _vp, _vp]),
     "lion_devoxelize_plan_bytes": (_sz, [_i, _i, _i]),
     "lion_trilinear_devoxelize_plan": (_i, [_vp, _i, _i, _i, _vp, _sz, _vp]),
     "lion_trilinear_devoxelize_planned_forward": (_i, [_vp, _sz, _vp, _vp, _vp, _vp, _i, _i, _i, _i, _vp, _vp]),
diff --git a/lion_amd/chain.py b/lion_amd/chain.py
--- a/lion_amd/chain.py
+++ b/lion_amd/chain.py
@@ -69,7 +69,8 @@
     from .models import pvcnn2_ada
     return (pvcnn2_ada.SPARSE_CONV1, pvcnn2_ada.FUSE_INFERENCE, pvcnn2_ada.OVERLAP_POINT_BRANCH, geometry.ENABLED,
             geometry.SPLIT_GRAPH, conv_ops.SPLIT, fused_ops.PW_SPLIT, pvcnn2_ada.VOX_PLAN, TEMB_TABLE, fused_ops.MAX_RECOMPUTE,
-            pvcnn2_ada.SKIP_UNREAD, pvcnn2_ada.SKIP_UNREAD_LEVEL2, CHANNEL_MAJOR_EPS, pvcnn2_ada.SA_GATHER, conv_ops.PRECISION)
+            pvcnn2_ada.SKIP_UNREAD, pvcnn2_ada.SKIP_UNREAD_LEVEL2, CHANNEL_MAJOR_EPS, pvcnn2_ada.SA_GATHER, conv_ops.PRECISION,
+            pvcnn2_ada.PVCONV_TAIL, fused_ops.DEVOX_TAIL)
 
 
 def channel_major(model, shape) -> bool:
diff --git a/lion_amd/csrc/common.h b/lion_amd/csrc/common.h
--- a/lion_amd/csrc/common.h
+++ b/lion_amd/csrc/common.h
@@ -93,6 +93,7 @@
 }
 
 __device__ __forceinline__ float swish_fast(float t) { return t * __builtin_amdgcn_rcpf(1.0f + __expf(-t)); }
+__device__ __forceinline__ float swish_affine_add(float x, float a, float b, float w) { return swish_fast(x * a + b) + w; }
 
 __device__ __forceinline__ float sqdist3(float ax, float ay, float az, float bx, float by,
                                          float bz) {
diff --git a/lion_amd/csrc/conv3d.hip b/lion_amd/csrc/conv3d.hip
--- a/lion_amd/csrc/conv3d.hip
+++ b/lion_amd/csrc/conv3d.hip
@@ -517,6 +517,80 @@
   }
 }
 
+struct GnFoldArgs {
+  const float *stats;
+  int C, T, G;
+  float count;
+  const float *gamma, *beta, *fac, *gbias;
+  int ld_fg;
+  float eps;
+  float *A, *Bs, *chmean;
+};
+
+__device__ __forceinline__ void gn_fold_ahead_body(const GnFoldArgs &a, int b, int g) {
+  __shared__ double cs[64][2];
+  __shared__ double gs[2];
+  __shared__ double ws[4][2];
+  const int C = a.C, T = a.T, cpg = C / a.G, tid = threadIdx.x;
+  const float count = a.count;
+  const int tc = g * cpg + min(tid, cpg - 1);
+  const float p_f = a.fac[(size_t)b * a.ld_fg + tc], p_gb = a.gbias[(size_t)b * a.ld_fg + tc];
+  const float p_gam = a.gamma[tc], p_bet = a.beta[tc];
+  int cp2 = 1;
+  while (cp2 < cpg) cp2 <<= 1;
+  const int LPC = 256 / cp2, ch = tid / LPC, sub = tid % LPC;
+  double s1 = 0.0, s2 = 0.0;
+  if (ch < cpg) {
+    const float2 *p = reinterpret_cast<const float2 *>(a.stats + (((size_t)b * C + g * cpg + ch) * T) * 2);
+    for (int t0 = sub; t0 < T; t0 += 8 * LPC) {
+      float2 v[8];
+#pragma unroll
+      for (int u = 0; u < 8; ++u) v[u] = p[min(t0 + u * LPC, T - 1)];
+#pragma unroll
+      for (int u = 0; u < 8; ++u)
+        if (t0 + u * LPC < T) { s1 += (double)v[u].x; s2 += (double)v[u].y; }
+    }
+  }
+  for (int m = 1; m < LPC && m < 64; m <<= 1) { s1 += __shfl_xor(s1, m, 64); s2 += __shfl_xor(s2, m, 64); }
+  if (LPC > 64) {
+    if ((tid & 63) == 0) { ws[tid >> 6][0] = s1; ws[tid >> 6][1] = s2; }
+    __syncthreads();
+    if (sub == 0) {
+      s1 = 0.0; s2 = 0.0;
+      for (int w = 0; w < LPC / 64; ++w) { s1 += ws[(tid >> 6) + w][0]; s2 += ws[(tid >> 6) + w][1]; }
+    }
+  }
+  if (ch < cpg && sub == 0) {
+    cs[ch][0] = s1;
+    cs[ch][1] = s2;
+    a.chmean[(size_t)b * C + g * cpg + ch] = (float)(s1 / count);
+  }
+  __syncthreads();
+  if (tid == 0) {
+    double g1 = 0.0, g2 = 0.0;
+    for (int c = 0; c < cpg; ++c) { g1 += cs[c][0]; g2 += cs[c][1]; }
+    gs[0] = g1;
+    gs[1] = g2;
+  }
+  __syncthreads();
+  if (tid < cpg) {
+    const double n = (double)count * cpg;
+    const double mean = gs[0] / n;
+    double var = gs[1] / n - mean * mean;
+    var = var > 0.0 ? var : 0.0;
+    const float rstd = (float)(1.0 / sqrt(var + (double)a.eps));
+    const int c = g * cpg + tid;
+    const float a0 = rstd * p_gam;
+    a.A[(size_t)b * C + c] = a0 * p_f;
+    a.Bs[(size_t)b * C + c] = (p_bet - (float)mean * a0) * p_f + p_gb;
+  }
+}
+
+__global__ __launch_bounds__(256) void gn_fold_pair_kernel(GnFoldArgs a0, GnFoldArgs a1) {
+  const bool second = (int)blockIdx.x >= a0.G;
+  gn_fold_ahead_body(second ? a1 : a0, blockIdx.y, second ? (int)blockIdx.x - a0.G : (int)blockIdx.x);
+}
+
 __global__ void conv3d_pack_kernel(const float *__restrict__ w, int Cout, int Cin, int Cin_pad,
                                    float *__restrict__ wp) {
   const int i = blockIdx.x * blockDim.x + threadIdx.x;
@@ -666,13 +740,36 @@
                                         gamma, beta, fac, gbias, ld_fg, eps, w1, w2, H, A, Bs);
 }
 
+static int gn_fold_args(const float *stats, int B, int C, int T, int G, int voxels, const float *gamma, const float *beta,
+                        const float *fac, const float *gbias, int ld_fg, float eps, float *A, float *Bs, float *chmean,
+                        GnFoldArgs *out) {
+  if (!stats || !gamma || !beta || !fac || !gbias || !A || !Bs || !chmean) return LION_EINVAL;
+  if (B <= 0 || C <= 0 || T <= 0 || G <= 0 || C % G != 0 || C / G > 64 || ld_fg < C) return LION_EINVAL;
+  *out = {stats, C, T, G, (float)voxels, gamma, beta, fac, gbias, ld_fg, eps, A, Bs, chmean};
+  return 0;
+}
+
 int lion_groupnorm_fold(const float *stats, int B, int C, int T, int G, int voxels, const float *gamma,
                         const float *beta, const float *fac, const float *gbias, int ld_fg, float eps,
                         float *A, float *Bs, float *chmean, lionStream_t stream) {
-  if (!stats || !gamma || !beta || !fac || !gbias || !A || !Bs || !chmean) return LION_EINVAL;
-  if (B <= 0 || C <= 0 || T <= 0 || G <= 0 || C % G != 0 || C / G > 64 || ld_fg < C) return LION_EINVAL;
+  GnFoldArgs a;
+  if (int e = gn_fold_args(stats, B, C, T, G, voxels, gamma, beta, fac, gbias, ld_fg, eps, A, Bs, chmean, &a)) return e;
   return lion_launch<gn_fold_kernel>(dim3(G, B), 256, 0, static_cast<hipStream_t>(stream), stats, C, T, G,
                                      (float)voxels, gamma, beta, fac, gbias, ld_fg, eps, A, Bs, chmean);
 }
 
-}
+int lion_groupnorm_fold_pair(int B, const float *stats0, int C0, int T0, int G0, int voxels0, const float *gamma0,
+                             const float *beta0, const float *fac0, const float *gbias0, int ld_fg0, float eps0,
+                             float *A0, float *Bs0, float *chmean0, const float *stats1, int C1, int T1, int G1,
+                             int voxels1, const float *gamma1, const float *beta1, const float *fac1,
+                             const float *gbias1, int ld_fg1, float eps1, float *A1, float *Bs1, float *chmean1,
+                             lionStream_t stream) {
+  GnFoldArgs a0, a1;
+  if (int e = gn_fold_args(stats0, B, C0, T0, G0, voxels0, gamma0, beta0, fac0, gbias0, ld_fg0, eps0, A0, Bs0, chmean0, &a0))
+    return e;
+  if (int e = gn_fold_args(stats1, B, C1, T1, G1, voxels1, gamma1, beta1, fac1, gbias1, ld_fg1, eps1, A1, Bs1, chmean1, &a1))
+    return e;
+  return lion_launch<gn_fold_pair_kernel>(dim3(G0 + G1, B), 256, 0, static_cast<hipStream_t>(stream), a0, a1);
+}
+
+}
diff --git a/lion_amd/csrc/devoxelize.hip b/lion_amd/csrc/devoxelize.hip
--- a/lion_amd/csrc/devoxelize.hip
+++ b/lion_amd/csrc/devoxelize.hip
@@ -81,13 +81,22 @@
 }
 
 
-template <int LD, bool AFF, bool SPLIT, bool ONE>
+using DevoxTailPtr = const float *__restrict__;
+struct DevoxTail { const float *pw, *pw_a, *pw_b; };
+__device__ __forceinline__ DevoxTail devox_tail() { return {nullptr, nullptr, nullptr}; }
+__device__ __forceinline__ DevoxTail devox_tail(DevoxTailPtr pw, DevoxTailPtr pw_a, DevoxTailPtr pw_b) { return {pw, pw_a, pw_b}; }
+
+template <int LD, bool AFF, bool SPLIT, bool ONE, typename... TailT>
 __global__ __launch_bounds__(256) void devox_slab_kernel(
     const float *__restrict__ coords, const float *__restrict__ feat, int C, int N, int r, int PX,
     int XS_rt, int CT, int CI, int slab_floats, int training, float *__restrict__ out,
     int32_t *__restrict__ inds, float *__restrict__ wgts, const float *__restrict__ scale,
-    const float *__restrict__ shift) {
+    const float *__restrict__ shift, TailT... tail_pack) {
+  constexpr bool TAIL = sizeof...(TailT) == 3;
+  static_assert(sizeof...(TailT) == 0 || sizeof...(TailT) == 3, "no tail, or pw, pw_a, pw_b");
+  const DevoxTail tail = devox_tail(tail_pack...);
   static_assert(!(ONE && SPLIT), "the single-slab form fetches whole grids: there is no row-end rule to apply");
+  static_assert(!TAIL || (ONE && AFF), "the tail exists for the single-slab affine form");
   constexpr bool FILT = !ONE;
   extern __shared__ __attribute__((aligned(16))) unsigned char smem[];
   float *lds = reinterpret_cast<float *>(smem);
@@ -142,6 +151,18 @@
       }
     }
   };
+  constexpr int TQ = TAIL ? 16 : 1;
+  const int tsh = N <= 256 ? 4 : N <= 512 ? 3 : N <= 1024 ? 2 : 1;
+  float tw[TQ];
+  auto tail_request = [&](int g) {
+    const int cin = min(CI, nch - g * CI);
+    if constexpr (TAIL) {
+      const float *__restrict__ src = tail.pw + ((size_t)b * C + c0 + g * CI) * N;
+#pragma unroll
+      for (int k = 0; k < TQ; ++k)
+        tw[k] = src[(unsigned)(min(k & ((1 << tsh) - 1), cin - 1) * N + min(tid + (k >> tsh) * 256, N - 1))];
+    }
+  };
   float cx[PP], cy[PP], cz[PP];
   if constexpr (ONE) {
 #pragma unroll
@@ -150,6 +171,7 @@
       cx[p] = cy[p] = cz[p] = 0.f;
       if (i < N) { cx[p] = co[i]; cy[p] = co[i + N]; cz[p] = co[i + 2 * N]; }
     }
+    if constexpr (TAIL) tail_request(0);
     issue(0);
   } else {
     const int nwords = (r2 + 31) >> 5;
@@ -237,9 +259,37 @@
     float *buf = lds + (it & 1) * slab_floats;
     asm volatile("s_waitcnt vmcnt(0)" ::: "memory");
     __syncthreads();
+    if constexpr (TAIL) {
+#pragma unroll
+      for (int k = 0; k < TQ; ++k) asm volatile("" : "+v"(tw[k]));
+    }
     if (it + 1 < nit) issue(it + 1);
     const int base = xs * PX * r2;
     float *o = out + ((size_t)b * C + cg) * N;
+    auto with_tail = [&](float a, int p, int ci, bool beyond_c) {
+      float t = a;
+      if constexpr (TAIL) {
+      const float *__restrict__ pw = tail.pw, *__restrict__ pw_a = tail.pw_a, *__restrict__ pw_b = tail.pw_b;
+      if (!beyond_c || ci < (1 << tsh)) {
+        const int idx = (p << tsh) + ci;
+        const bool b0 = idx & 1, b1 = idx & 2, b2 = idx & 4, b3 = idx & 8;
+        const float a0 = b0 ? tw[1] : tw[0], a1 = b0 ? tw[3] : tw[2], a2 = b0 ? tw[5] : tw[4], a3 = b0 ? tw[7] : tw[6];
+        const float a4 = b0 ? tw[9] : tw[8], a5 = b0 ? tw[11] : tw[10], a6 = b0 ? tw[13] : tw[12], a7 = b0 ? tw[15] : tw[14];
+        const float e0 = b1 ? a1 : a0, e1 = b1 ? a3 : a2, e2 = b1 ? a5 : a4, e3 = b1 ? a7 : a6;
+        const float d0 = b2 ? e1 : e0, d1 = b2 ? e3 : e2;
+        t = b3 ? d1 : d0;
+      } else {
+        t = (pw + ((size_t)b * C + cg) * N)[(unsigned)(ci * N + pid[p])];
+      }
+      t = swish_affine_add(t, pw_a[(size_t)b * C + cg + ci], pw_b[(size_t)b * C + cg + ci], a);
+      }
+      return t;
+    };
+    const bool beyond = TAIL && cin > (1 << tsh);
+#pragma unroll
+    for (int copy = 0; copy < (TAIL ? 2 : 1); ++copy) {
+    const bool beyond_c = copy == 1;
+    if (TAIL && beyond_c != beyond) continue;
 #pragma unroll
     for (int p = 0; p < PP; ++p) {
       if (xsl[p] == xs) {
@@ -265,11 +315,20 @@
           a = add_rn(a, mul_rn(w6, v6));
           a = add_rn(a, mul_rn(w7, v7));
           if (AFF) a = a * scale[(size_t)b * C + cg + ci] + shift[(size_t)b * C + cg + ci] * wsum;
+          if constexpr (TAIL) a = with_tail(a, p, ci, beyond_c);
           o[(size_t)ci * N + pid[p]] = a;
         }
       } else if (xsl[p] == -2 && xs == 0) {
-        for (int ci = 0; ci < cin; ++ci) o[(size_t)ci * N + pid[p]] = 0.f;
-      }
+        if constexpr (TAIL) {
+          for (int ci = 0; ci < cin; ++ci) o[(size_t)ci * N + pid[p]] = with_tail(0.f, p, ci, beyond_c);
+        } else {
+          for (int ci = 0; ci < cin; ++ci) o[(size_t)ci * N + pid[p]] = 0.f;
+        }
+      }
+    }
+    }
+    if constexpr (TAIL) {
+      if (it + 1 < nit) tail_request(it + 1);
     }
   }
 }
@@ -747,6 +806,21 @@
                       static_cast<hipStream_t>(stream));
 }
 
+int lion_trilinear_devoxelize_affine_tail_forward(const float *coords, const float *feat, const float *scale,
+                                                  const float *shift, const float *pw, const float *pw_a,
+                                                  const float *pw_b, int B, int C, int N, int r, float *out,
+                                                  lionStream_t stream) {
+  if (!coords || !feat || !out || !scale || !shift || !pw || !pw_a || !pw_b || B <= 0 || C <= 0 || N <= 0 || r <= 0)
+    return LION_EINVAL;
+  const DevoxPlan p = devox_plan(B, C, N, r, (((uintptr_t)feat) & 15) == 0);
+  if (p.kind != DEVOX_SLAB || p.XS != 1) return LION_EUNSUPPORTED;
+  return devox_ld_dispatch(p.ld, [&](auto LD) {
+    return lion_launch<devox_slab_kernel<decltype(LD)::value, true, false, true, DevoxTailPtr, DevoxTailPtr, DevoxTailPtr>>(
+        p.grid, 256, p.lds, static_cast<hipStream_t>(stream), coords, feat, C, N, r, p.PX, p.XS, p.ct, p.CI, p.slab_floats, 0,
+        out, nullptr, nullptr, scale, shift, pw, pw_a, pw_b);
+  });
+}
+
 size_t lion_devoxelize_plan_bytes(int B, int N, int r) {
   if (B <= 0 || N <= 0 || N > 2048 || r != DVR_R) return 0;
   return (size_t)B * devox_plan_stride<DVR_G>();
diff --git a/lion_amd/csrc/pointwise.hip b/lion_amd/csrc/pointwise.hip
--- a/lion_amd/csrc/pointwise.hip
+++ b/lion_amd/csrc/pointwise.hip
@@ -59,10 +59,10 @@
   const int i = (blockIdx.x * 256 + threadIdx.x) * 4;
   if (i + 3 < L && (L & 3) == 0) {
     const float4 v = *reinterpret_cast<const float4 *>(p + i), w = *reinterpret_cast<const float4 *>(ad + i);
-    *reinterpret_cast<float4 *>(q + i) = make_float4(swishf(v.x * a + b) + w.x, swishf(v.y * a + b) + w.y,
-                                                     swishf(v.z * a + b) + w.z, swishf(v.w * a + b) + w.w);
-  } else {
-    for (int j = i; j < L && j < i + 4; ++j) q[j] = swishf(p[j] * a + b) + ad[j];
+    *reinterpret_cast<float4 *>(q + i) = make_float4(swish_affine_add(v.x, a, b, w.x), swish_affine_add(v.y, a, b, w.y),
+                                                     swish_affine_add(v.z, a, b, w.z), swish_affine_add(v.w, a, b, w.w));
+  } else {
+    for (int j = i; j < L && j < i + 4; ++j) q[j] = swish_affine_add(p[j], a, b, ad[j]);
   }
 }
 
diff --git a/lion_amd/fused_ops.py b/lion_amd/fused_ops.py
--- a/lion_amd/fused_ops.py
+++ b/lion_amd/fused_ops.py
@@ -32,10 +32,17 @@
 
 class FoldSpec:
 
-    def __init__(self, gn: torch.nn.GroupNorm, fac, gbias, count, se=None):
+    def __init__(self, gn: torch.nn.GroupNorm, fac, gbias, count, se=None, partner=None):
         self.gn, self.fac, self.gbias, self.count, self.se = gn, fac, gbias, int(count), se
+        self.partner, self.partner_result = partner, None
 
     def apply(self, stats):
+        if self.partner is not None:
+            assert self.se is None and self.partner[0].se is None, "the paired fold has no SE form"
+            other, ostats = self.partner
+            (a, b_, _), (oa, ob, _) = groupnorm_fold_pair(stats, self, ostats, other)
+            self.partner_result = (oa, ob)
+            return a, b_
         if self.se is not None:
             merged = groupnorm_fold_se(stats, self.gn, self.fac, self.gbias, self.count, self.se)
             if merged is not None:
@@ -101,6 +108,23 @@
     return A, Bs, cm
 
 
+def groupnorm_fold_pair(stats0, spec0, stats1, spec1):
+    args, outs = [], []
+    for stats, s in ((stats0, spec0), (stats1, spec1)):
+        b, c, t, _ = stats.shape
+        A = torch.empty((b, c), device=stats.device, dtype=torch.float32)
+        Bs, cm = torch.empty_like(A), torch.empty_like(A)
+        fac, gbias = s.fac, s.gbias
+        if not (fac.stride(1) == 1 and gbias.stride(1) == 1 and fac.stride(0) == gbias.stride(0) and fac.stride(0) >= c):
+            fac, gbias = fac.contiguous(), gbias.contiguous()
+        args += [stats, c, t, s.gn.num_groups, s.count, s.gn.weight, s.gn.bias, fac, gbias, int(fac.stride(0)),
+                 float(s.gn.eps), A, Bs, cm]
+        outs.append((A, Bs, cm))
+    assert stats0.shape[0] == stats1.shape[0]
+    _lib.call("lion_groupnorm_fold_pair", stats0.shape[0], *args)
+    return outs[0], outs[1]
+
+
 def groupnorm_fold_se(stats, gn: torch.nn.GroupNorm, fac, gbias, voxels, se):
     b, c, t, _ = stats.shape
     w1, w2 = se.fc[0].weight.detach(), se.fc[2].weight.detach()
@@ -137,17 +161,26 @@
     return {"buf": buf, "coords": coords, "shape": (b, n, int(r))}
 
 
-def devoxelize_affine(grid, coords, r, scale, shift, plan=None):
+DEVOX_TAIL = os.environ.get("LION_DEVOX_TAIL", "0") != "0"
+
+
+def devoxelize_affine(grid, coords, r, scale, shift, plan=None, tail=None):
     b, c = grid.shape[:2]
     n = coords.shape[2]
     out = torch.empty((b, c, n), device=grid.device, dtype=torch.float32)
     co_c, gr_c, sc_c, sh_c = coords.contiguous(), grid.contiguous(), scale.contiguous(), shift.contiguous()
+    if tail is not None:
+        pw, ta, tb = tail[0].contiguous(), tail[1].contiguous(), tail[2].contiguous()
+        assert pw.shape == out.shape and pw.dtype == torch.float32
+        if DEVOX_TAIL and _lib.call("lion_trilinear_devoxelize_affine_tail_forward", co_c, gr_c, sc_c, sh_c, pw, ta, tb, b, c, n, int(r), out,
+                     unsupported_ok=True):
+            return out
     if plan is not None and plan["shape"] == (b, n, int(r)) and plan["coords"].data_ptr() == co_c.data_ptr():
         buf = plan["buf"]
         _lib.call("lion_trilinear_devoxelize_planned_forward", buf, buf.numel(), co_c, gr_c, sc_c, sh_c, b, c, n, int(r), out)
-        return out
-    _lib.call("lion_trilinear_devoxelize_affine_forward", co_c, gr_c, sc_c, sh_c, b, c, n, int(r), out)
-    return out
+    else:
+        _lib.call("lion_trilinear_devoxelize_affine_forward", co_c, gr_c, sc_c, sh_c, b, c, n, int(r), out)
+    return out if tail is None else affine_swish(pw, ta, tb, add=out)
 
 
 def fusable(conv1, conv2, r, x):
diff --git a/lion_amd/models/pvcnn2_ada.py b/lion_amd/models/pvcnn2_ada.py
--- a/lion_amd/models/pvcnn2_ada.py
+++ b/lion_amd/models/pvcnn2_ada.py
@@ -14,6 +14,7 @@
 FUSE_INFERENCE = True
 SPARSE_CONV1 = True
 OVERLAP_POINT_BRANCH = os.environ.get("LION_OVERLAP_POINT_BRANCH", "0") != "0"
+PVCONV_TAIL = os.environ.get("LION_PVCONV_TAIL", "1") != "0"
 _POINT_STREAMS = {}
 
 
@@ -376,7 +377,17 @@
         conv2 = self.voxel_layers[4]
         return 2 if (SKIP_UNREAD_LEVEL2 and conv_ops.use_split(None, conv2.in_channels, conv2.out_channels, self.resolution)) else 1
 
-    def _fused_voxel_branch(self, grid, geo, style, level):
+    def _point_conv(self, features):
+        mlp = self.point_features
+        if len(mlp.layers) != 3 or not mlp._fusable(features):
+            return None
+        conv, gn = mlp.layers[0], mlp.layers[1]
+        if not fused_ops.pw_supported(conv, features):
+            return None
+        pw, stats = fused_ops.pwconv_fused(features, conv, None)
+        return pw, stats, gn
+
+    def _fused_voxel_branch(self, grid, geo, style, level, point=None):
         conv1, gn1, conv2, gn2 = self.voxel_layers[0], self.voxel_layers[1], self.voxel_layers[4], self.voxel_layers[5]
         se = self.voxel_layers[6] if len(self.voxel_layers) > 6 else None
         r = self.resolution
@@ -384,12 +395,18 @@
         if SPARSE_CONV1 and r >= 16:
             occ1, occ2 = geo.occupancy(level, conv1.out_channels)
         f1, g1 = gn1.affine(style)
-        y1, (a1, b1) = fused_ops.conv3d_fused(grid, conv1, None, True, occ1,
-                                              fold=fused_ops.FoldSpec(gn1.norm, f1, g1, r ** 3))
+        partner = None
+        if point is not None:
+            pw, pw_stats, pgn = point
+            fp, gp = pgn.affine(style)
+            partner = (fused_ops.FoldSpec(pgn.norm, fp, gp, pw[0, 0].numel()), pw_stats)
+        fold1 = fused_ops.FoldSpec(gn1.norm, f1, g1, r ** 3, partner=partner)
+        y1, (a1, b1) = fused_ops.conv3d_fused(grid, conv1, None, True, occ1, fold=fold1)
         f2, g2 = gn2.affine(style)
         y2, (a2, b2) = fused_ops.conv3d_fused(y1, conv2, (a1, b1), True, occ2, prev_conv=conv1,
                                               fold=fused_ops.FoldSpec(gn2.norm, f2, g2, r ** 3, se))
-        return fused_ops.devoxelize_affine(y2, geo.norm, r, a2, b2, plan=geo.devox_plan())
+        tail = None if point is None else (point[0],) + fold1.partner_result
+        return fused_ops.devoxelize_affine(y2, geo.norm, r, a2, b2, plan=geo.devox_plan(), tail=tail)
 
     def forward(self, inputs):
         features, coords_input, time_emb, style = inputs
@@ -413,8 +430,13 @@
                 side.wait_stream(main)
                 with torch.cuda.stream(side):
                     pf = self.point_features(features, style)
-            fused = self._fused_voxel_branch(grid, geo, style, level)
-            if pf is not None:
+            point = None
+            if self.add_point_feat and pf is None and PVCONV_TAIL:
+                point = self._point_conv(features)
+            fused = self._fused_voxel_branch(grid, geo, style, level, point)
+            if point is not None:
+                pass
+            elif pf is not None:
                 main.wait_stream(side)
                 pf.record_stream(main)
                 fused = fused + pf
```

After: 5.942 (median of 6 runs). About the same (+0.4%).
